# heathsc/bs_call

Measured on AMD Instinct MI355X. Metric: genome positions called/sec, higher is better.
Workload: dtype f64

## Files before the change

bs_call_amd/csrc/accumulate.hip:

```cpp
#include <hip/hip_runtime.h>
#include <stdint.h>

#include "accdev.h"
#include "devtables.h"

#define IN_DW 26
#define SLOT_DW (64 * IN_DW)
#define ACC_WAVES 4
#define SUM_DW 12

struct bsc_template_dev {
  uint32_t pos[2];
  uint32_t len[2];
  uint64_t off[2];
  uint8_t mapq[2];
  uint8_t orientation;
  uint8_t bs_strand;
  uint32_t flags;
};
#define TPL_WALK_KNOWN 1u
#define TPL_WALKED0 2u

__device__ static __forceinline__ uint32_t leftmost(uint32_t p0, uint32_t p1) {
  return p0 == 0 ? p1 : (p1 > 0 && p1 < p0 ? p1 : p0);
}

__device__ static __forceinline__ uint32_t template_error(const bsc_template_dev &tp, uint32_t left, uint32_t x,
                                                          uint64_t seq_bytes) {
  if (left < x) return BSC_TERR_LEFT;
  if ((tp.len[0] && tp.pos[0] < x) || (tp.len[1] && tp.pos[1] < x)) return BSC_TERR_LEFT;
  if (tp.orientation > 1) return BSC_TERR_ORI;
  if (tp.bs_strand > 2) return BSC_TERR_STRAND;
  if (tp.len[0] && (tp.off[0] > seq_bytes || tp.len[0] > seq_bytes - tp.off[0])) return BSC_TERR_RANGE0;
  if (tp.len[1] && (tp.off[1] > seq_bytes || tp.len[1] > seq_bytes - tp.off[1])) return BSC_TERR_RANGE1;
  if (tp.flags & ~(TPL_WALK_KNOWN | TPL_WALKED0)) return BSC_TERR_FLAGS;
  return 0;
}

__device__ static __forceinline__ uint32_t template_reads(const bsc_template_dev &tp, uint32_t x, uint32_t y, uint64_t seq_bytes,
                                                          bool walked0, bsc_read_desc d[2]) {
  acc_dead(d[0]);
  acc_dead(d[1]);
  const uint32_t terr = template_error(tp, leftmost(tp.pos[0], tp.pos[1]), x, seq_bytes);
  if (terr) return terr;
  uint32_t ori = tp.orientation & 1u;
#pragma unroll
  for (int k = 0; k < 2; k++) {
    const uint32_t rl = tp.len[k];
    if (rl != 0 && (k == 1 || walked0)) {
      const uint64_t pa = (uint64_t)tp.pos[k], pb = (uint64_t)tp.pos[k] + rl - 1u;
      if (pa <= y) {
        d[k].a = (uint32_t)pa;
        d[k].b = pb > y ? y : (uint32_t)pb;
        d[k].base = (int64_t)tp.off[k] - (int64_t)tp.pos[k];
        d[k].meta = ACC_META(ori, tp.mapq[k]);
        d[k].lut = tp.bs_strand == 0 ? LUT4(0, 1, 2, 3) : (tp.bs_strand == 1 ? LUT4(0, 5, 2, 7) : LUT4(4, 1, 6, 3));
      }
    }
    if (k == 0 && walked0) ori ^= 1u;
  }
  return 0;
}

__device__ static __forceinline__ void template_block(const bsc_chain_mblock *__restrict__ blk, uint32_t n_blk, uint32_t t, uint32_t &x,
                                                      uint32_t &y, uint32_t &bin0) {
  bin0 = 0;
  if (!blk) return;
  uint32_t lo = 0, hi = n_blk - 1u;
  while (lo < hi) {
    const uint32_t mid = (lo + hi) >> 1;
    if (t < blk[mid].tpl_end) hi = mid;
    else lo = mid + 1u;
  }
  x = blk[lo].x;
  y = blk[lo].x + (blk[lo].n - 1u);
  bin0 = blk[lo].bin0;
}

#ifndef BIN_WG
#define BIN_WG 256
#endif
#ifndef BIN_TPT
#define BIN_TPT 4
#endif
#define BIN_TPW (BIN_WG * BIN_TPT)
#ifndef BIN_WIN
#define BIN_WIN 1024
#endif

__device__ static __forceinline__ uint32_t wg_min_bin(uint32_t m, uint32_t *s_min) {
  if (threadIdx.x == 0) *s_min = 0xffffffffu;
  __syncthreads();
  for (int o = 32; o > 0; o >>= 1) {
    const uint32_t v = __shfl_xor(m, o);
    m = v < m ? v : m;
  }
  if ((threadIdx.x & 63u) == 0 && m != 0xffffffffu) atomicMin(s_min, m);
  __syncthreads();
  return *s_min;
}

extern "C" __global__ __launch_bounds__(BIN_WG) void bsc_bin_count_kernel(const bsc_template_dev *__restrict__ tpl, uint32_t nr,
                                                                          const uint8_t *__restrict__ seq, uint64_t seq_bytes,
                                                                          uint32_t x, uint32_t y, uint8_t *__restrict__ tflag,
                                                                          uint32_t *__restrict__ bin_cnt,
                                                                          unsigned long long *__restrict__ counters,
                                                                          const bsc_chain_mblock *__restrict__ blk, uint32_t n_blk) {
  __shared__ uint32_t s_cnt[BIN_WIN];
  __shared__ uint32_t s_min;
  for (unsigned i = threadIdx.x; i < BIN_WIN; i += BIN_WG) s_cnt[i] = 0;
  uint32_t bin[BIN_TPT][2], span_max = 0, bin_lo = 0xffffffffu;
  bsc_template_dev tps[BIN_TPT];
#pragma unroll
  for (int j = 0; j < BIN_TPT; j++) {
    const uint32_t t = blockIdx.x * BIN_TPW + (uint32_t)j * BIN_WG + threadIdx.x;
    if (t < nr) tps[j] = tpl[t];
  }
#pragma unroll
  for (int j = 0; j < BIN_TPT; j++) {
    const uint32_t t = blockIdx.x * BIN_TPW + (uint32_t)j * BIN_WG + threadIdx.x;
    bin[j][0] = bin[j][1] = 0xffffffffu;
    if (t < nr) {
      const bsc_template_dev tp = tps[j];
      uint32_t bin0;
      template_block(blk, n_blk, t, x, y, bin0);
      bool walked0 = false;
      if (tp.flags & TPL_WALK_KNOWN) walked0 = (tp.flags & TPL_WALKED0) != 0;
      else if (template_error(tp, leftmost(tp.pos[0], tp.pos[1]), x, seq_bytes) == 0) {
        const uint32_t rl = tp.len[0];
        const uint8_t *sp = seq + tp.off[0];
        for (uint32_t q_ = 0; q_ < rl; q_++) {
          const uint32_t q = (uint32_t)sp[q_] >> 2;
          if (q > 0 && q != 63u) {
            walked0 = true;
            break;
          }
        }
      }
      tflag[t] = walked0 ? 1 : 0;
      bsc_read_desc d[2];
      const uint32_t terr = template_reads(tp, x, y, seq_bytes, walked0, d);
      if (terr) atomicMin(&counters[BSC_CNT_ERR], ((unsigned long long)t << 8) | terr);
#pragma unroll
      for (int k = 0; k < 2; k++)
        if (d[k].b >= d[k].a) {
          bin[j][k] = bin0 + ((d[k].a - x) >> ACC_BIN_SHIFT);
          if (bin[j][k] < bin_lo) bin_lo = bin[j][k];
          if (d[k].b - d[k].a > span_max) span_max = d[k].b - d[k].a;
        }
    }
  }
  const uint32_t base = wg_min_bin(bin_lo, &s_min);
#pragma unroll
  for (int j = 0; j < BIN_TPT; j++)
#pragma unroll
    for (int k = 0; k < 2; k++)
      if (bin[j][k] != 0xffffffffu) {
        if (bin[j][k] - base < BIN_WIN) atomicAdd(&s_cnt[bin[j][k] - base], 1u);
        else atomicAdd(&bin_cnt[bin[j][k]], 1u);
      }
  __syncthreads();
  for (unsigned i = threadIdx.x; i < BIN_WIN; i += BIN_WG)
    if (s_cnt[i]) atomicAdd(&bin_cnt[base + i], s_cnt[i]);
  for (int o = 32; o > 0; o >>= 1) {
    const uint32_t v = __shfl_xor(span_max, o);
    span_max = v > span_max ? v : span_max;
  }
  if ((threadIdx.x & 63u) == 0 && span_max &&
      __hip_atomic_load(&counters[BSC_CNT_SPAN], __ATOMIC_RELAXED, __HIP_MEMORY_SCOPE_AGENT) < span_max)
    atomicMax(&counters[BSC_CNT_SPAN], (unsigned long long)span_max);
}

extern "C" __global__ __launch_bounds__(BIN_WG) void bsc_bin_scatter_kernel(const bsc_template_dev *__restrict__ tpl, uint32_t nr,
                                                                            uint64_t seq_bytes, uint32_t x, uint32_t y,
                                                                            const uint8_t *__restrict__ tflag,
                                                                            uint32_t *__restrict__ bin_cur,
                                                                            bsc_read_desc *__restrict__ rd,
                                                                            const bsc_chain_mblock *__restrict__ blk, uint32_t n_blk) {
  __shared__ uint32_t s_cnt[BIN_WIN];
  __shared__ uint32_t s_min;
  for (unsigned i = threadIdx.x; i < BIN_WIN; i += BIN_WG) s_cnt[i] = 0;
  uint32_t bin[BIN_TPT][2], rank[BIN_TPT][2], bin_lo = 0xffffffffu;
  bsc_read_desc d[BIN_TPT][2];
  bsc_template_dev tps[BIN_TPT];
  uint8_t tf[BIN_TPT];
#pragma unroll
  for (int j = 0; j < BIN_TPT; j++) {
    const uint32_t t = blockIdx.x * BIN_TPW + (uint32_t)j * BIN_WG + threadIdx.x;
    tf[j] = 0;
    if (t < nr) {
      tps[j] = tpl[t];
      tf[j] = tflag[t];
    }
  }
#pragma unroll
  for (int j = 0; j < BIN_TPT; j++) {
    const uint32_t t = blockIdx.x * BIN_TPW + (uint32_t)j * BIN_WG + threadIdx.x;
    bin[j][0] = bin[j][1] = 0xffffffffu;
    rank[j][0] = rank[j][1] = 0;
    acc_dead(d[j][0]);
    acc_dead(d[j][1]);
    if (t < nr) {
      uint32_t bin0;
      template_block(blk, n_blk, t, x, y, bin0);
      (void)template_reads(tps[j], x, y, seq_bytes, tf[j] != 0, d[j]);
#pragma unroll
      for (int k = 0; k < 2; k++)
        if (d[j][k].b >= d[j][k].a) {
          bin[j][k] = bin0 + ((d[j][k].a - x) >> ACC_BIN_SHIFT);
          if (bin[j][k] < bin_lo) bin_lo = bin[j][k];
        }
    }
  }
  const uint32_t base = wg_min_bin(bin_lo, &s_min);
#pragma unroll
  for (int j = 0; j < BIN_TPT; j++)
#pragma unroll
    for (int k = 0; k < 2; k++)
      if (bin[j][k] != 0xffffffffu && bin[j][k] - base < BIN_WIN) rank[j][k] = atomicAdd(&s_cnt[bin[j][k] - base], 1u);
  __syncthreads();
  for (unsigned i = threadIdx.x; i < BIN_WIN; i += BIN_WG)
    if (s_cnt[i]) s_cnt[i] = atomicAdd(&bin_cur[base + i], s_cnt[i]);
  __syncthreads();
#pragma unroll
  for (int j = 0; j < BIN_TPT; j++)
#pragma unroll
    for (int k = 0; k < 2; k++)
      if (bin[j][k] != 0xffffffffu) {
        const uint32_t slot = bin[j][k] - base < BIN_WIN ? s_cnt[bin[j][k] - base] + rank[j][k] : atomicAdd(&bin_cur[bin[j][k]], 1u);
        rd[slot] = d[j][k];
      }
}

template <bool SUMM>
__global__ __launch_bounds__(64 * ACC_WAVES) void bsc_accumulate_kernel_t(
    const bsc_read_desc *__restrict__ rd, const uint32_t *__restrict__ bin_off, uint32_t n_bins, const uint8_t *__restrict__ seq,
    uint32_t x, uint32_t y, uint32_t min_qual, uint32_t *__restrict__ cts, unsigned long long *__restrict__ counters,
    const bsc_chain_mblock *__restrict__ blk, uint32_t n_blk) {
  __shared__ __attribute__((aligned(16))) uint32_t lds_slot[ACC_WAVES][SLOT_DW];
  const unsigned lane = threadIdx.x & 63u;
  const unsigned wid = __builtin_amdgcn_readfirstlane(threadIdx.x >> 6);
  uint32_t *slot = lds_slot[wid];
  uint32_t *row = slot + lane * IN_DW;
  const uint32_t n_sites = y - x + 1;
  const uint32_t n_wt = blk ? n_bins : (n_sites + 63u) / 64u;
  const uint32_t q_span = min_qual < 63u ? 63u - min_qual : 0u;
  unsigned inexact = 0;
  acc_reads R;
  R.rd = rd;
  R.bin_off = bin_off;
  R.seq = seq;
  R.n_bins = n_bins;
  R.x = x;
  uint32_t n_live = bin_off[n_bins];
  const uint32_t span = (uint32_t)counters[BSC_CNT_SPAN];
  const uint32_t wt_step = gridDim.x * ACC_WAVES;
#ifndef ACC_XCD_CHUNK
#define ACC_XCD_CHUNK 16
#endif
#ifndef ACC_NO_XCD_SWIZZLE
  const uint32_t per8 = 8u * ACC_XCD_CHUNK, full8 = gridDim.x / per8 * per8;
  const uint32_t lb = blockIdx.x >> 3;
  const uint32_t vb = blockIdx.x < full8 ? (lb / ACC_XCD_CHUNK) * per8 + (blockIdx.x & 7u) * ACC_XCD_CHUNK + lb % ACC_XCD_CHUNK : blockIdx.x;
#else
  const uint32_t vb = blockIdx.x;
#endif
  uint32_t wt = vb * ACC_WAVES + wid;
  uint32_t t0 = 0, kv = 0xffffffffu;
  bsc_read_desc d;
  acc_dead(d);
  uint32_t wl = wt, wl_n = 0;
#define ACC_BLOCK_OF(w, wlocal)                                    \
  do {                                                             \
    uint32_t lo_ = 0, hi_ = n_blk - 1u;                            \
    while (lo_ < hi_) {                                            \
      const uint32_t mid_ = (lo_ + hi_) >> 1;                      \
      if ((w) < blk[mid_].bin_end) hi_ = mid_;                     \
      else lo_ = mid_ + 1u;                                        \
    }                                                              \
    x = blk[lo_].x;                                                \
    y = blk[lo_].x + (blk[lo_].n - 1u);                            \
    R.x = x;                                                       \
    R.bin_off = bin_off + blk[lo_].bin0;                           \
    n_live = bin_off[blk[lo_].bin_end];                            \
    (wlocal) = (w)-blk[lo_].bin0;                                  \
  } while (0)
  if (wt < n_wt) {
    if (blk) ACC_BLOCK_OF(wt, wl);
    t0 = acc_tile_start(R, (int64_t)wl * 64, span);
    acc_fetch(R, n_live, t0, lane, kv, d);
  }
  for (; wt < n_wt; wt += wt_step) {
    const uint32_t p0 = x + wl * 64u;
    const uint32_t p_last = y - p0 < 63u ? y : p0 + 63u;
    const uint32_t r_last = p_last - x;
    const bool valid = lane <= p_last - p0;
    const acc_reads Rc = R;
    const uint32_t n_live_c = n_live;
    const uint32_t wt1 = wt + wt_step;
    const bool have1 = wt1 < n_wt && wt1 > wt;
    uint32_t kv_n = 0xffffffffu, t0_n = 0;
    bsc_read_desc dn;
    acc_dead(dn);
    wl_n = wt1;
    if (have1) {
      if (blk) ACC_BLOCK_OF(wt1, wl_n);
      t0_n = acc_tile_start(R, (int64_t)wl_n * 64, span);
      acc_fetch(R, n_live, t0_n, lane, kv_n, dn);
    }
    {
      uint32_t w[IN_DW];
      bool packed;
      inexact |= acc_tile(Rc, n_live_c, lane, lane, row, p0, p_last, r_last, min_qual, q_span, t0, kv, d, w, &packed) ? 1u : 0u;
      if (SUMM) {
        if (__builtin_expect(!packed, 0)) {
          uint32_t cmax = 0;
#pragma unroll
          for (int j = 0; j < 8; j++) cmax = max(cmax, w[j] + w[8 + j]);
          if (__any(cmax > 0xffffu) && lane == 0) atomicMax(&counters[BSC_CNT_DEEP], 1ull);
        }
        uint32_t o[SUM_DW];
        {
#include "call_summary.inc"
#pragma unroll
          for (int j = 0; j < 8; j++) o[j] = ((w[j] + w[8 + j]) & 0xffffu) | (w[j] << 16);
          o[8] = qpack0;
          o[9] = qpack1;
          o[10] = ((uint32_t)aq & 0xffffu) | ((uint32_t)mq << 16);
          o[11] = covered ? n_reads : 0u;
        }
        uint32_t *srow = slot + lane * SUM_DW;
#pragma unroll
        for (int i = 0; i < SUM_DW / 2; i++) reinterpret_cast<uint2 *>(srow)[i] = make_uint2(o[2 * i], o[2 * i + 1]);
      } else {
#pragma unroll
        for (int i = 0; i < IN_DW / 2; i++) reinterpret_cast<uint2 *>(row)[i] = make_uint2(w[2 * i], w[2 * i + 1]);
      }
    }
    const uint32_t nvalid = p_last - p0 + 1u;
    constexpr unsigned ROW = SUMM ? SUM_DW : IN_DW;
    uint32_t *dst = cts + (uint64_t)wt * (64u * ROW);
#ifdef ACC_EXPERIMENT_NOSTORE
    if (wt == 0xffffffffu)
#endif
    if (nvalid == 64u) {
      typedef unsigned int u32x4 __attribute__((ext_vector_type(4)));
      const u32x4 *s4 = reinterpret_cast<const u32x4 *>(slot);
      u32x4 *d4 = reinterpret_cast<u32x4 *>(dst);
#ifdef ACC_PLAIN_STORES
#define ACC_ST(p, v) *(p) = (v)
#else
#define ACC_ST(p, v) __builtin_nontemporal_store((v), (p))
#endif
      constexpr int full = (int)(64u * ROW * 4u / 1024u);
#pragma unroll
      for (int v = 0; v < full; v++) ACC_ST(d4 + v * 64 + lane, s4[v * 64 + lane]);
      constexpr unsigned rem = (64u * ROW * 4u % 1024u) / 16u;
      if (rem && lane < rem) ACC_ST(d4 + full * 64 + lane, s4[full * 64 + lane]);
#undef ACC_ST
    } else if (valid || blk) {
      const uint32_t *orow = slot + lane * ROW;
#pragma unroll
      for (int i = 0; i < (int)ROW; i++) dst[lane * ROW + i] = valid ? orow[i] : 0u;
    }
    t0 = t0_n;
    kv = kv_n;
    d = dn;
    wl = wl_n;
  }
  if (__any(inexact)) {
    const unsigned long long m = __ballot(inexact);
    if (lane == 0) atomicAdd(&counters[BSC_CNT_INEXACT], (unsigned long long)__popcll(m));
  }
}

extern "C" __global__ __launch_bounds__(256) void bsc_ref_pad_kernel(const uint8_t *__restrict__ packed, const bsc_chain_mblock *__restrict__ blk,
                                                                     uint32_t n_blk, uint8_t *__restrict__ padded, uint32_t n_pos) {
  for (uint32_t p = blockIdx.x * 256u + threadIdx.x; p < n_pos; p += gridDim.x * 256u) {
    uint32_t lo = 0, hi = n_blk;
    while (hi - lo > 1u) {
      const uint32_t mid = (lo + hi) >> 1;
      if (blk[mid].pos_off <= p) lo = mid;
      else hi = mid;
    }
    const uint32_t i = p - blk[lo].pos_off;
    padded[p] = i < blk[lo].n ? packed[(uint64_t)blk[lo].ref_in + i] : (uint8_t)0;
  }
}

extern "C" int bsc_dev_launch_ref_pad(const void *packed, const void *d_blk, uint32_t n_blk, void *padded, uint32_t n_pos, int num_cus,
                                      void *stream) {
  if (!n_pos) return 0;
  unsigned g = (n_pos + 255u) / 256u;
  if (g > (unsigned)num_cus * 8u) g = (unsigned)num_cus * 8u;
  hipLaunchKernelGGL(bsc_ref_pad_kernel, dim3(g), dim3(256), 0, (hipStream_t)stream, (const uint8_t *)packed, (const bsc_chain_mblock *)d_blk,
                     n_blk, (uint8_t *)padded, n_pos);
  return (int)hipGetLastError();
}

extern "C" int bsc_dev_scan_u32(const void *in, void *out, uint32_t n, void *tmp, size_t tmp_bytes, void *stream);

extern "C" uint32_t bsc_dev_n_bins(uint32_t n_sites) { return ((n_sites - 1u) >> ACC_BIN_SHIFT) + 1u; }

static int launch_bin_reads(const void *tpl, uint32_t nr, const void *seq, uint64_t seq_bytes, uint32_t x, uint32_t y, uint32_t nb,
                            const bsc_chain_mblock *blk, uint32_t n_blk, void *tflag, void *bin_cnt, void *bin_off, void *bin_cur,
                            void *scan_tmp, size_t scan_tmp_bytes, void *rd, void *counters, void *stream) {
  hipStream_t s = (hipStream_t)stream;
  const size_t bytes = ((size_t)nb + 1u) * sizeof(uint32_t);
  if (!nr) return (int)hipMemsetAsync(bin_off, 0, bytes, s);
  hipError_t e = hipMemsetAsync(bin_cnt, 0, bytes, s);
  if (e != hipSuccess) return (int)e;
  const unsigned g = (nr + BIN_TPW - 1u) / BIN_TPW;
  hipLaunchKernelGGL(bsc_bin_count_kernel, dim3(g), dim3(BIN_WG), 0, s, (const bsc_template_dev *)tpl, nr, (const uint8_t *)seq,
                     seq_bytes, x, y, (uint8_t *)tflag, (uint32_t *)bin_cnt, (unsigned long long *)counters, blk, n_blk);
  if ((e = hipGetLastError()) != hipSuccess) return (int)e;
  int rc = bsc_dev_scan_u32(bin_cnt, bin_off, nb + 1u, scan_tmp, scan_tmp_bytes, stream);
  if (rc) return rc;
  if ((e = hipMemcpyAsync(bin_cur, bin_off, bytes, hipMemcpyDeviceToDevice, s)) != hipSuccess) return (int)e;
  hipLaunchKernelGGL(bsc_bin_scatter_kernel, dim3(g), dim3(BIN_WG), 0, s, (const bsc_template_dev *)tpl, nr, seq_bytes, x, y,
                     (const uint8_t *)tflag, (uint32_t *)bin_cur, (bsc_read_desc *)rd, blk, n_blk);
  return (int)hipGetLastError();
}

extern "C" int bsc_dev_launch_bin_reads(const void *tpl, uint32_t nr, const void *seq, uint64_t seq_bytes, uint32_t x, uint32_t y,
                                        void *tflag, void *bin_cnt, void *bin_off, void *bin_cur, void *scan_tmp,
                                        size_t scan_tmp_bytes, void *rd, void *counters, void *stream) {
  return launch_bin_reads(tpl, nr, seq, seq_bytes, x, y, bsc_dev_n_bins(y - x + 1), NULL, 0, tflag, bin_cnt, bin_off, bin_cur, scan_tmp,
                          scan_tmp_bytes, rd, counters, stream);
}

extern "C" int bsc_dev_launch_bin_reads_multi(const void *tpl, uint32_t nr, const void *seq, uint64_t seq_bytes, const void *d_blk,
                                              uint32_t n_blk, uint32_t n_bins, void *tflag, void *bin_cnt, void *bin_off, void *bin_cur,
                                              void *scan_tmp, size_t scan_tmp_bytes, void *rd, void *counters, void *stream) {
  return launch_bin_reads(tpl, nr, seq, seq_bytes, 0, 0, n_bins, (const bsc_chain_mblock *)d_blk, n_blk, tflag, bin_cnt, bin_off, bin_cur,
                          scan_tmp, scan_tmp_bytes, rd, counters, stream);
}

static int launch_accumulate(const void *rd, const void *bin_off, const void *seq, uint32_t x, uint32_t y, uint32_t n_wt, uint32_t min_qual,
                             void *cts, void *counters, const bsc_chain_mblock *blk, uint32_t n_blk, int num_cus, void *stream,
                             bool summary = false) {
  unsigned g = (n_wt + ACC_WAVES - 1) / ACC_WAVES;
  const unsigned cap = (unsigned)num_cus * 6u * 8u;
  if (g > cap) g = cap;
  if (summary)
    hipLaunchKernelGGL(bsc_accumulate_kernel_t<true>, dim3(g), dim3(64 * ACC_WAVES), 0, (hipStream_t)stream, (const bsc_read_desc *)rd,
                       (const uint32_t *)bin_off, n_wt, (const uint8_t *)seq, x, y, min_qual, (uint32_t *)cts,
                       (unsigned long long *)counters, blk, n_blk);
  else
    hipLaunchKernelGGL(bsc_accumulate_kernel_t<false>, dim3(g), dim3(64 * ACC_WAVES), 0, (hipStream_t)stream, (const bsc_read_desc *)rd,
                       (const uint32_t *)bin_off, n_wt, (const uint8_t *)seq, x, y, min_qual, (uint32_t *)cts,
                       (unsigned long long *)counters, blk, n_blk);
  return (int)hipGetLastError();
}

extern "C" int bsc_dev_launch_accumulate_summary(const void *rd, const void *bin_off, const void *seq, uint32_t x, uint32_t y,
                                                 uint32_t min_qual, void *cts, void *counters, int num_cus, void *stream) {
  return launch_accumulate(rd, bin_off, seq, x, y, bsc_dev_n_bins(y - x + 1), min_qual, cts, counters, NULL, 0, num_cus, stream, true);
}
extern "C" size_t bsc_dev_summary_bytes(void) { return SUM_DW * 4u; }

extern "C" int bsc_dev_launch_accumulate(const void *rd, const void *bin_off, const void *seq, uint32_t x, uint32_t y, uint32_t min_qual,
                                         void *cts, void *counters, int num_cus, void *stream) {
  return launch_accumulate(rd, bin_off, seq, x, y, bsc_dev_n_bins(y - x + 1), min_qual, cts, counters, NULL, 0, num_cus, stream);
}

extern "C" int bsc_dev_launch_accumulate_multi(const void *rd, const void *bin_off, const void *seq, const void *d_blk, uint32_t n_blk,
                                               uint32_t n_bins, uint32_t min_qual, void *cts, void *counters, int num_cus, void *stream) {
  return launch_accumulate(rd, bin_off, seq, 0, 0, n_bins, min_qual, cts, counters, (const bsc_chain_mblock *)d_blk, n_blk, num_cus, stream);
}
```

bs_call_amd/csrc/bscall_api.c:

```c
#ifndef __HIP_PLATFORM_AMD__
#define __HIP_PLATFORM_AMD__ 1
#endif
#include <hip/hip_runtime_api.h>
#include <math.h>
#include <pthread.h>
#include <stdarg.h>
#include <stdio.h>
#include <stdlib.h>
#include <string.h>

#include "../../include/bscall_amd.h"
#include "devtables.h"
#include "bsmath.h"
#include "bsmath_tables.h"
#include "synth.h"

int bsc_dev_launch_call(const void *cts, const void *ref, uint64_t n, void *out, uint32_t out_dw, void *skip,
                        const void *tb, void *het_list, void *counters, int num_cus, void *stream, void *ev_start,
                        void *ev_mid, void *ev_stop);
int bsc_dev_launch_accumulate(const void *rd, const void *bin_off, const void *seq, uint32_t x, uint32_t y, uint32_t min_qual, void *cts,
                              void *counters, int num_cus, void *stream);
int bsc_dev_launch_bin_reads(const void *tpl, uint32_t nr, const void *seq, uint64_t seq_bytes, uint32_t x, uint32_t y, void *tflag,
                             void *bin_cnt, void *bin_off, void *bin_cur, void *scan_tmp, size_t scan_tmp_bytes, void *rd,
                             void *counters, void *stream);
uint32_t bsc_dev_n_bins(uint32_t n_sites);
int bsc_dev_launch_site_stats(const void *core, const void *gtm, uint32_t gtm_stride, const void *dbsnp, uint32_t n,
                              const void *tb, const void *logp, const void *carry_in, void *carry_out, void *stats,
                              void *pairs, int num_cus, void *stream);
int bsc_dev_launch_gc_cov_gtm(const void *core, const void *gtm, uint32_t gtm_stride, uint32_t n, const void *gc_bins, uint32_t n_bins,
                              uint32_t start_pos, void *table, int num_cus, void *stream);
int bsc_dev_launch_meth_eval(void *pairs, const void *tb, const void *logp, void *stats, const void *ovf_list,
                             const void *counters, int num_cus, void *stream);
int bsc_dev_scan_tmp_bytes(uint32_t n, size_t *bytes);
int bsc_dev_launch_stream_probe(const void *cts, const void *ref, uint64_t n, void *out, void *skip, int num_cus,
                                void *stream);
int bsc_dev_launch_compact(const void *core, const void *gtm, uint32_t gtm_stride, const void *dbsnp, uint32_t n,
                           void *tile_cnt, void *tile_off, void *scan_tmp, size_t scan_tmp_bytes, void *out,
                           uint64_t out_cap, void *total, const void *emit, void *emit_ws, int num_cus, void *stream);
#define BSC_PAIR_BYTES (4ull * 512u * 512u * 8u)
#define BSC_OVF_CAP (1u << 20)
int bsc_dev_launch_vcf(const void *gtm, uint32_t stride, const void *skip, const void *ref, const void *dbsnp, uint32_t n,
                       uint32_t x, int all_positions, uint32_t reg_start, uint32_t reg_stop, const void *tb, void *g,
                       void *out, int num_cus, void *stream);
int bsc_dev_launch_chain(const bsc_chain_launch *L);
unsigned bsc_dev_chain_quantum(int num_cus);
unsigned bsc_dev_chain_window(int num_cus, unsigned limit);
int bsc_dev_launch_synth(uint64_t seed, uint64_t first_site, uint64_t n, uint32_t coverage, uint32_t flags, void *cts,
                         void *ref, int num_cus, void *stream);
size_t bsc_dev_chain_het_bytes(uint32_t n, int num_cus, int with_depth, int reads);
size_t bsc_dev_chain_scratch_bytes(int num_cus);
size_t bsc_dev_chain_multi_table_bytes(uint32_t n_blocks);
int bsc_dev_launch_chain_multi(const bsc_chain_launch *L, const bsc_chain_mblock *blk, uint32_t b_first, uint32_t b_last, void *tab_h,
                               void *tab_d, size_t *cursor);
int bsc_dev_launch_accumulate_summary(const void *rd, const void *bin_off, const void *seq, uint32_t x, uint32_t y, uint32_t min_qual, void *cts,
                                      void *counters, int num_cus, void *stream);
size_t bsc_dev_summary_bytes(void);
int bsc_dev_launch_accumulate_multi(const void *rd, const void *bin_off, const void *seq, const void *d_blk, uint32_t n_blk, uint32_t n_bins,
                                    uint32_t min_qual, void *cts, void *counters, int num_cus, void *stream);
int bsc_dev_scan_tmp_bytes_u64(uint32_t n, size_t *bytes);
size_t bsc_dev_prep_plan_bytes(void);
int bsc_dev_launch_prep(const void *raw, uint32_t nr, const void *seq, uint64_t seq_bytes, const void *misms, uint64_t n_misms,
                        const bsc_prep_params *par, void *ms_work, void *plan, void *out_len, void *out_off, void *scan_tmp,
                        size_t scan_tmp_bytes, void *tpl_out, void *seq_out, uint64_t seq_out_cap, void *cnt, int num_cus, void *stream,
                        const void *prof_ref, uint32_t prof_x, uint32_t prof_n_ref, uint32_t prof_cap, uint32_t prof_used0, void *prof_table,
                        void *max_pos1, void *used_scan, void *prof_mask);
int bsc_dev_launch_bcf(const void *recs, const void *core, const void *aux, const void *n_recs, uint64_t max_recs, int32_t rid,
                       const bsc_bcf_ids *ids, const void *name_pos, const void *name_off, const void *name_bytes, uint32_t n_names,
                       void *tile_bytes, void *tile_off, void *scan_tmp, size_t scan_tmp_bytes, void *out, uint64_t out_cap, void *totals,
                       int num_cus, void *stream, const void *emit_len);
int bsc_dev_launch_vcf_text(const void *recs, const void *core, const void *aux, const void *n_recs, uint64_t max_recs, const char *contig,
                            uint32_t contig_len, const void *name_pos, const void *name_off, const void *name_bytes, uint32_t n_names,
                            void *tile_bytes, void *tile_off, void *line_len, void *scan_tmp, size_t scan_tmp_bytes, void *out, uint64_t out_cap,
                            void *totals, int num_cus, void *stream);
int bsc_dev_launch_fmt_g(const void *v, uint64_t n, void *out16, int num_cus, void *stream);
int bsc_dev_launch_ref_pad(const void *packed, const void *d_blk, uint32_t n_blk, void *padded, uint32_t n_pos, int num_cus, void *stream);
int bsc_dev_launch_bin_reads_multi(const void *tpl, uint32_t nr, const void *seq, uint64_t seq_bytes, const void *d_blk, uint32_t n_blk,
                                   uint32_t n_bins, void *tflag, void *bin_cnt, void *bin_off, void *bin_cur, void *scan_tmp,
                                   size_t scan_tmp_bytes, void *rd, void *counters, void *stream);
int bsc_dev_launch_bgzf(const void *src, uint64_t n, uint32_t n_members, void *slots, void *sizes, void *offs, void *scratch, uint32_t grid,
                        void *stream);
int bsc_dev_launch_bgzf_gather(const void *slots, const void *offs, const void *sizes, uint32_t n_members, void *out, void *stream);
#define BSC_PREP_CNT_SLOTS 64u
#define BSC_PREP_CNT_ALL (8u + 8u * BSC_PREP_CNT_SLOTS)
#define BSC_LN10 (2.30258509299404568402)
#define BSC_HOST_CHUNK (4u << 20)
#define BSC_MAX_LAUNCH (1ull << 31)

struct bsc_context {
  bsc_params params;
  int device;
  int num_cus;
  hipStream_t stream;
  double q_prob[44][5];
  bsc_dev_tables host_tables;
  void *d_tables;
  unsigned long long *d_counters;
  uint64_t sites;
  void *d_cts, *d_ref, *d_out, *d_skip;
  size_t cap_cts, cap_ref, cap_out, cap_skip;
  void *d_het;
  size_t cap_het;
  uint64_t max_launch;
  void *d_ovf;
  void *d_gc_table;
  void *d_gc_own;
  size_t cap_gc_own;
  const void *d_gc_bins;
  uint32_t gc_n_bins, gc_start_pos;
  hipEvent_t ev_chain[2];
  int ev_chain_valid;
  void *d_tpl, *d_seq, *d_rd;
  size_t cap_tpl, cap_seq, cap_rd;
  void *d_tflag, *d_bcnt, *d_boff, *d_bcur, *d_bscan;
  size_t cap_tflag, cap_bcnt, cap_boff, cap_bcur, cap_bscan;
  void *d_vg, *d_vout, *d_vdb;
  size_t cap_vg, cap_vout, cap_vdb;
  void *d_tcnt, *d_toff, *d_scantmp, *d_recs;
  size_t cap_tcnt, cap_toff, cap_scantmp, cap_recs;
  void *d_sstats, *d_pairs;
  uint32_t *d_carry;
  double *d_logp;
  unsigned carry_slot;
  void *h_stage;
  size_t cap_stage;
  uint64_t pending_sz;
  uint32_t pending_stride;
  int pending_copied;
  const bsc_template *blk_tpl;
  const void *blk_d_tpl;
  uint32_t blk_x;
  unsigned long long *h_cnt;
  bsc_vcf_rec *rec_out;
  uint64_t rec_cap, rec_copied;
  uint32_t rec_sz;
  int rec_pending;
  double rec_share;
  void *d_btb, *d_bto, *d_bscn, *d_bnm, *d_bcf, *d_btot;
  size_t cap_btb, cap_bto, cap_bscn, cap_bnm, cap_bcf, cap_btot;
  void *d_vtl;
  size_t cap_vtl;
  struct {
    void *p[4];
    size_t cap[4];
  } bcf_pool;
  pthread_mutex_t pool_mu;
  int pool_mu_made;
  void *det_ptr[4];
  hipStream_t s_det;
  void *h_names;
  size_t cap_hnm;
  const bsc_bcf_names *names_up;
  uint32_t names_up_n;
  uint64_t names_up_bytes;
  struct {
    int valid, have_names, inexact;
    uint32_t sz, n_names;
    uint64_t name_bytes;
    int32_t rid;
    bsc_bcf_ids ids;
    const void *emit;
    bsc_bcf_names names;
    int text;
    char contig[256];
  } again;
  int no_h2d_turns;
  void *d_emit;
  size_t cap_emit;
  hipEvent_t ev_h2d;
  const void *emit_hint;
  uint8_t *bcf_out;
  int stage_timing;
  int no_emit_bytes;
  int bcf_blk, bcf_keep;
  uint64_t bcf_cap, bcf_copied, bcf_bytes;
  double bcf_share;
  const bsc_chain_mblock *mb_tab;
  uint32_t mb_n;
  void *d_mblk, *d_mtab;
  size_t cap_mblk, cap_mtab;
  void *d_pplan, *d_plen, *d_poff, *d_pms, *d_pscan, *d_pcnt, *d_raw, *d_rseq, *d_rms;
  size_t cap_pplan, cap_plen, cap_poff, cap_pms, cap_pscan, cap_pcnt, cap_raw, cap_rseq, cap_rms;
  unsigned long long *h_prep;
  size_t cap_hprep;
  void *d_pmask;
  size_t cap_pmask;
  void *d_pprof, *d_pmax, *d_pused;
  size_t cap_pprof, cap_pmax, cap_pused;
  void *d_refp;
  size_t cap_refp;
  const uint32_t *mb_toff;
  int dbg_fail_summary;
  int reads_fused;
  void *d_fscr;
  size_t cap_fscr;
  hipEvent_t ev_rchain[2];
  int ev_rchain_valid;
  hipEvent_t ev_raw[2];
  int ev_raw_valid;
  int ref_resident;
  hipEvent_t ev_acc[2];
  int ev_acc_valid;
  hipStream_t s_in, s_out;
  hipEvent_t ev_in[2], ev_k[2], ev_out[2];
  void *p_cts[2], *p_ref[2], *p_out[2], *p_skip[2];
  size_t p_cap_cts[2], p_cap_ref[2], p_cap_out[2], p_cap_skip[2];
  int pipe_ready;
  int profiling;
#define BSC_EV_RING 32
  hipEvent_t ev[BSC_EV_RING][3];
  uint64_t ev_count;
};

static __thread char bsc_errbuf[512];

static int bsc_fail(int code, const char *fmt, ...) {
  va_list ap;
  va_start(ap, fmt);
  vsnprintf(bsc_errbuf, sizeof bsc_errbuf, fmt, ap);
  va_end(ap);
  return code;
}

typedef struct {
  int prev;
} bsc_devguard;
static void bsc_devguard_exit(bsc_devguard *g) {
  if (g->prev >= 0) (void)hipSetDevice(g->prev);
}
#define BSC_GUARD(g) bsc_devguard g __attribute__((cleanup(bsc_devguard_exit), unused)) = {-1}
#define BSC_ENTER_GUARD(ctx, g)  \
  do {                                                                               \
    int cur_ = -1;                                                                   \
    if (hipGetDevice(&cur_) != hipSuccess || cur_ != (ctx)->device) {                \
      HIP_TRY(hipSetDevice((ctx)->device));                                          \
      (g).prev = cur_;                                                               \
    }                                                                                \
  } while (0)
#define BSC_ENTER(ctx) \
  BSC_GUARD(guard_);   \
  BSC_ENTER_GUARD(ctx, guard_)

int bsc_set_error(int code, const char *fmt, ...) {
  va_list ap;
  va_start(ap, fmt);
  vsnprintf(bsc_errbuf, sizeof bsc_errbuf, fmt, ap);
  va_end(ap);
  return code;
}

#define HIP_TRY(call)                                                                                        \
  do {                                                                                                       \
    hipError_t e_ = (call);                                                                                  \
    if (e_ != hipSuccess) return bsc_fail(BSC_ERR_HIP, "%s failed: %s (%s:%d)", #call, hipGetErrorString(e_), \
                                          __FILE__, __LINE__);                                               \
  } while (0)

int bsc_ctx_device(const bsc_context *ctx) { return ctx->device; }
void *bsc_ctx_stream(const bsc_context *ctx) { return (void *)ctx->stream; }

int bsc_abi_version(void) { return BSC_ABI_VERSION; }
const char *bsc_last_error(void) { return bsc_errbuf; }

void bsc_params_default(bsc_params *p) {
  p->under_conv = 0.01;
  p->over_conv = 0.05;
  p->ref_bias = 2.0;
  p->min_qual = 20;
  p->device = -1;
}

static int bsc_phred_of_om(double om) {
  const double lg = bsm_log_t(om, bsm_log_tab);
  const double v = (-10.0 * lg) / BSC_LN10;
  const int p = (int)v;
  return p > 255 ? 255 : p;
}
static int bsc_build_phred_table(bsc_dev_tables *t) {
  double T[260];
  for (int k = 1; k <= 255; k++) {
    uint64_t lo = bsm_bits(0x1p-1000), hi = bsm_bits(1.0);
    if (bsc_phred_of_om(bsm_from_bits(lo)) < k || bsc_phred_of_om(bsm_from_bits(hi)) >= k) return -1;
    while (hi - lo > 1) {
      const uint64_t mid = lo + (hi - lo) / 2;
      if (bsc_phred_of_om(bsm_from_bits(mid)) >= k) lo = mid;
      else hi = mid;
    }
    T[k] = bsm_from_bits(lo);
    if (k > 1 && !(T[k] < T[k - 1])) return -1;
  }
  for (int k = 256; k < 260; k++) T[k] = -1.0;
  for (int e = 0; e < 64; e++) {
    const double top = e == 0 ? 1.0 : bsm_from_bits(bsm_bits(ldexp(1.0, 1 - e)) - 1);
    const int b = bsc_phred_of_om(top);
    if (bsc_phred_of_om(ldexp(1.0, -e)) - b > 4) return -1;
    t->phred_base[e] = (unsigned char)b;
    for (int j = 0; j < 4; j++) t->phred_thr[e][j] = T[b + 1 + j];
  }
  return 0;
}

int bsc_phred_table(double *thr_64x4, unsigned char *base_64) {
  if (!thr_64x4 || !base_64) return bsc_fail(BSC_ERR_ARG, "bsc_phred_table: NULL argument");
  bsc_dev_tables *t = malloc(sizeof *t);
  if (!t) return bsc_fail(BSC_ERR_NOMEM, "bsc_phred_table: out of memory");
  const int rc = bsc_build_phred_table(t);
  if (!rc) {
    memcpy(thr_64x4, t->phred_thr, sizeof t->phred_thr);
    memcpy(base_64, t->phred_base, sizeof t->phred_base);
  }
  free(t);
  return rc ? bsc_fail(BSC_ERR_ARG, "bsc_phred_table: the QUAL staircase of this build's log is not monotone") : BSC_OK;
}

static void bsc_build_tables(bsc_context *ctx) {
  bsc_dev_tables *t = &ctx->host_tables;
  for (int q = 0; q <= 43; q++) {
    double e = exp(-.1 * (double)q * BSC_LN10);
    if (e > .5) e = .5;
    double k = e / (3.0 - 4.0 * e);
    ctx->q_prob[q][0] = e;
    ctx->q_prob[q][1] = t->k[q] = k;
    ctx->q_prob[q][2] = t->ln_k[q] = log(k);
    ctx->q_prob[q][3] = t->ln_k_half[q] = log(0.5 + k);
    ctx->q_prob[q][4] = t->ln_k_one[q] = log(1.0 + k);
  }
  t->lfact[0] = t->lfact[1] = 0.0;
  double l = 0.0;
  for (int i = 2; i < 256; i++) {
    l += log((double)i);
    t->lfact[i] = l;
  }
  memcpy(t->log_tab, bsm_log_tab, sizeof t->log_tab);
  memcpy(t->exp_tab, bsm_exp_tab, sizeof t->exp_tab);
  t->under_conv = ctx->params.under_conv;
  t->over_conv = ctx->params.over_conv;
  t->lrb = log(ctx->params.ref_bias);
  t->lrb1 = log(0.5 * (1.0 + ctx->params.ref_bias));
}

int bsc_create(const bsc_params *params, bsc_context **out) {
  if (!out) return bsc_fail(BSC_ERR_ARG, "bsc_create: out is NULL");
  *out = NULL;
  bsc_params p;
  if (params) p = *params;
  else bsc_params_default(&p);
  if (!(p.under_conv >= 0.0 && p.under_conv < 1.0) || !(p.over_conv >= 0.0 && p.over_conv < 1.0) || !(p.ref_bias > 0.0))
    return bsc_fail(BSC_ERR_ARG, "bsc_create: conversion rates must be in [0,1) and ref_bias > 0");
  if (!((1.0 - p.under_conv) - p.over_conv >= 0x1p-20))
    return bsc_fail(BSC_ERR_ARG, "bsc_create: under_conv + over_conv must be < 1 (by at least 2^-20)");
  if (p.min_qual < 1) p.min_qual = 1;
  if (p.min_qual > 43) p.min_qual = 43;
// ... 209 lines not shown
    return bsc_fail(BSC_ERR_ARG, "out_stride must be 200 (gt_meth[]) or 208 (gt_vcf[]), got %u", out_stride);
  return BSC_OK;
}

int bsc_call_sites_device(bsc_context *ctx, const void *d_cts, const void *d_ref, uint64_t n, void *d_out,
                          uint32_t out_stride, void *d_skip, void *stream) {
  if (!ctx) return bsc_fail(BSC_ERR_ARG, "bsc_call_sites_device: ctx is NULL");
  int rc = bsc_check_stride(out_stride);
  if (rc) return rc;
  if (n == 0) return BSC_OK;
  if (!d_cts || !d_ref || !d_out || !d_skip) return bsc_fail(BSC_ERR_ARG, "bsc_call_sites_device: NULL buffer");
  if (((uintptr_t)d_cts & 15u) || ((uintptr_t)d_out & 15u))
    return bsc_fail(BSC_ERR_ARG, "bsc_call_sites_device: d_cts and d_out must be 16-byte aligned");
  BSC_ENTER(ctx);
  hipStream_t s = (hipStream_t)stream;
  uint64_t done = 0;
  while (done < n) {
    uint64_t m = n - done;
    if (m > ctx->max_launch) m = ctx->max_launch;
    rc = bsc_reserve(&ctx->d_het, &ctx->cap_het, (size_t)((m + 63u) / 64u) * 8u);
    if (rc) return rc;
    int e = bsc_dev_launch_call((const char *)d_cts + done * 104u, (const char *)d_ref + done, m,
                                (char *)d_out + done * out_stride, out_stride / 4u, (char *)d_skip + done,
                                ctx->d_tables, ctx->d_het, ctx->d_counters, ctx->num_cus, s,
                                ctx->profiling ? ctx->ev[ctx->ev_count % BSC_EV_RING][0] : NULL,
                                ctx->profiling ? ctx->ev[ctx->ev_count % BSC_EV_RING][1] : NULL,
                                ctx->profiling ? ctx->ev[ctx->ev_count % BSC_EV_RING][2] : NULL);
    if (ctx->profiling) ctx->ev_count++;
    if (e) return bsc_fail(BSC_ERR_HIP, "kernel launch failed: %s", hipGetErrorString((hipError_t)e));
    done += m;
  }
  ctx->sites += n;
  return BSC_OK;
}

#define BSC_PIPE_CHUNK (1u << 20)

static int bsc_pipe_init(bsc_context *ctx) {
  if (ctx->pipe_ready) return BSC_OK;
  HIP_TRY(hipStreamCreateWithFlags(&ctx->s_in, hipStreamNonBlocking));
  HIP_TRY(hipStreamCreateWithFlags(&ctx->s_out, hipStreamNonBlocking));
  for (int b = 0; b < 2; b++) {
    HIP_TRY(hipEventCreateWithFlags(&ctx->ev_in[b], hipEventDisableTiming));
    HIP_TRY(hipEventCreateWithFlags(&ctx->ev_k[b], hipEventDisableTiming));
    HIP_TRY(hipEventCreateWithFlags(&ctx->ev_out[b], hipEventDisableTiming));
  }
  ctx->pipe_ready = 1;
  return BSC_OK;
}

int bsc_call_sites(bsc_context *ctx, const bsc_pileup *cts, const uint8_t *ref, uint64_t n, void *out,
                   uint32_t out_stride, uint8_t *skip) {
  if (!ctx) return bsc_fail(BSC_ERR_ARG, "bsc_call_sites: ctx is NULL");
  int rc = bsc_check_stride(out_stride);
  if (rc) return rc;
  if (n == 0) return BSC_OK;
  if (!cts || !ref || !out || !skip) return bsc_fail(BSC_ERR_ARG, "bsc_call_sites: NULL buffer");
  BSC_ENTER(ctx);
  if ((rc = bsc_pipe_init(ctx))) return rc;
  const uint64_t chunk = n < BSC_PIPE_CHUNK ? n : BSC_PIPE_CHUNK;
  const int nbuf = n > chunk ? 2 : 1;
  for (int b = 0; b < nbuf; b++) {
    if ((rc = bsc_reserve(&ctx->p_cts[b], &ctx->p_cap_cts[b], (size_t)chunk * 104u))) return rc;
    if ((rc = bsc_reserve(&ctx->p_ref[b], &ctx->p_cap_ref[b], (size_t)chunk))) return rc;
    if ((rc = bsc_reserve(&ctx->p_out[b], &ctx->p_cap_out[b], (size_t)chunk * out_stride))) return rc;
    if ((rc = bsc_reserve(&ctx->p_skip[b], &ctx->p_cap_skip[b], (size_t)chunk))) return rc;
  }
  uint64_t k = 0;
  for (uint64_t done = 0; done < n; done += chunk, k++) {
    const int b = (int)(k & 1);
    const uint64_t m = (n - done) < chunk ? (n - done) : chunk;
    if (k >= 2) HIP_TRY(hipStreamWaitEvent(ctx->s_in, ctx->ev_k[b], 0));
    HIP_TRY(hipMemcpyAsync(ctx->p_cts[b], cts + done, (size_t)m * 104u, hipMemcpyHostToDevice, ctx->s_in));
    HIP_TRY(hipMemcpyAsync(ctx->p_ref[b], ref + done, (size_t)m, hipMemcpyHostToDevice, ctx->s_in));
    HIP_TRY(hipEventRecord(ctx->ev_in[b], ctx->s_in));
    HIP_TRY(hipStreamWaitEvent(ctx->stream, ctx->ev_in[b], 0));
    if (k >= 2) HIP_TRY(hipStreamWaitEvent(ctx->stream, ctx->ev_out[b], 0));
    rc = bsc_call_sites_device(ctx, ctx->p_cts[b], ctx->p_ref[b], m, ctx->p_out[b], out_stride, ctx->p_skip[b], ctx->stream);
    if (rc) return rc;
    HIP_TRY(hipEventRecord(ctx->ev_k[b], ctx->stream));
    HIP_TRY(hipStreamWaitEvent(ctx->s_out, ctx->ev_k[b], 0));
    HIP_TRY(hipMemcpyAsync((char *)out + done * out_stride, ctx->p_out[b], (size_t)m * out_stride, hipMemcpyDeviceToHost,
                           ctx->s_out));
    HIP_TRY(hipMemcpyAsync(skip + done, ctx->p_skip[b], (size_t)m, hipMemcpyDeviceToHost, ctx->s_out));
    HIP_TRY(hipEventRecord(ctx->ev_out[b], ctx->s_out));
  }
  HIP_TRY(hipStreamSynchronize(ctx->s_out));
  HIP_TRY(hipStreamSynchronize(ctx->stream));
  return BSC_OK;
}

void *bsc_alloc_host(uint64_t bytes) {
  void *p = NULL;
  if (hipHostMalloc(&p, (size_t)bytes, hipHostMallocDefault) != hipSuccess) {
    bsc_fail(BSC_ERR_NOMEM, "bsc_alloc_host(%llu) failed", (unsigned long long)bytes);
    return NULL;
  }
  return p;
}

void bsc_free_host(void *p) {
  if (p) hipHostFree(p);
}

static uint32_t bsc_leftmost(const bsc_template *t) {
  uint32_t x1 = t->pos[0];
  if (x1 == 0) x1 = t->pos[1];
  else if (t->pos[1] > 0 && t->pos[1] < x1) x1 = t->pos[1];
  return x1;
}

static int bsc_stage_reserve(bsc_context *ctx, size_t need) {
  if (need <= ctx->cap_stage) return BSC_OK;
  if (ctx->h_stage) hipHostFree(ctx->h_stage);
  ctx->h_stage = NULL;
  ctx->cap_stage = 0;
  size_t sz = need + need / 4;
  if (hipHostMalloc(&ctx->h_stage, sz, hipHostMallocDefault) != hipSuccess)
    return bsc_fail(BSC_ERR_NOMEM, "hipHostMalloc(%zu) failed", sz);
  ctx->cap_stage = sz;
  return BSC_OK;
}

static int bsc_accumulate_queue2(bsc_context *ctx, const bsc_template *tpl, uint32_t nr, const uint8_t *seq,
                                 uint64_t seq_bytes, uint32_t x, uint32_t y, const uint8_t *ref, int stage);

static int bsc_accumulate_queue(bsc_context *ctx, const bsc_template *tpl, uint32_t nr, const uint8_t *seq,
                                uint64_t seq_bytes, uint32_t x, uint32_t y) {
  return bsc_accumulate_queue2(ctx, tpl, nr, seq, seq_bytes, x, y, NULL, 0);
}

static int bsc_accumulate_reserve(bsc_context *ctx, uint32_t nr, uint32_t x, uint32_t y, size_t *scan_bytes) {
  const uint64_t sz = (uint64_t)y - x + 1;
  if (sz > 0xffffffffull) return bsc_fail(BSC_ERR_ARG, "accumulate: block longer than 2^32 - 1 positions");
  const size_t nb1 = (size_t)bsc_dev_n_bins((uint32_t)sz) + 1u;
  int rc;
  *scan_bytes = 0;
  if (nr > 0x7fffffffu) return bsc_fail(BSC_ERR_ARG, "accumulate: more than 2^31 - 1 templates in one block");
  if (bsc_dev_scan_tmp_bytes((uint32_t)nb1, scan_bytes)) return bsc_fail(BSC_ERR_HIP, "accumulate: scan size query failed");
  if ((rc = bsc_reserve(&ctx->d_rd, &ctx->cap_rd, (size_t)(nr ? nr : 1) * 48u))) return rc;
  if ((rc = bsc_reserve(&ctx->d_tflag, &ctx->cap_tflag, (size_t)(nr ? nr : 1)))) return rc;
  if ((rc = bsc_reserve(&ctx->d_bcnt, &ctx->cap_bcnt, nb1 * 4u))) return rc;
  if ((rc = bsc_reserve(&ctx->d_boff, &ctx->cap_boff, nb1 * 4u))) return rc;
  if ((rc = bsc_reserve(&ctx->d_bcur, &ctx->cap_bcur, nb1 * 4u))) return rc;
  if ((rc = bsc_reserve(&ctx->d_bscan, &ctx->cap_bscan, *scan_bytes ? *scan_bytes : 1))) return rc;
  return BSC_OK;
}

static int bsc_reads_prepare(bsc_context *ctx, const void *d_tpl, uint32_t nr, const void *d_seq, uint64_t seq_bytes, uint32_t x,
                             uint32_t y, size_t scan_bytes, hipStream_t s) {
  HIP_TRY(hipMemsetAsync(ctx->d_counters + BSC_CNT_SPAN, 0, 2 * sizeof(unsigned long long), s));
  HIP_TRY(hipMemsetAsync(ctx->d_counters + BSC_CNT_ERR, 0xff, sizeof(unsigned long long), s));
  HIP_TRY(hipMemsetAsync(ctx->d_counters + BSC_CNT_DEEP, 0, sizeof(unsigned long long), s));
  int e = bsc_dev_launch_bin_reads(d_tpl, nr, d_seq, seq_bytes, x, y, ctx->d_tflag, ctx->d_bcnt, ctx->d_boff, ctx->d_bcur,
                                   ctx->d_bscan, scan_bytes, ctx->d_rd, ctx->d_counters, s);
  if (e) return bsc_fail(BSC_ERR_HIP, "read grouping launch failed: %s", hipGetErrorString((hipError_t)e));
  return BSC_OK;
}

static int bsc_accumulate_launch(bsc_context *ctx, const void *d_tpl, uint32_t nr, const void *d_seq, uint64_t seq_bytes,
                                 uint32_t x, uint32_t y, void *d_cts, size_t scan_bytes, hipStream_t s) {
  if (ctx->profiling) {
    if (!ctx->ev_acc[0])
      for (int i = 0; i < 2; i++) HIP_TRY(hipEventCreate(&ctx->ev_acc[i]));
    HIP_TRY(hipEventRecord(ctx->ev_acc[0], s));
  }
  int rc = bsc_reads_prepare(ctx, d_tpl, nr, d_seq, seq_bytes, x, y, scan_bytes, s);
  if (rc) return rc;
  int e = bsc_dev_launch_accumulate(ctx->d_rd, ctx->d_boff, d_seq, x, y, (uint32_t)ctx->params.min_qual, d_cts, ctx->d_counters,
                                    ctx->num_cus, s);
  if (e) return bsc_fail(BSC_ERR_HIP, "accumulate launch failed: %s", hipGetErrorString((hipError_t)e));
  if (ctx->profiling) {
    HIP_TRY(hipEventRecord(ctx->ev_acc[1], s));
    ctx->ev_acc_valid = 1;
  }
  return BSC_OK;
}

static int bsc_accumulate_queue2(bsc_context *ctx, const bsc_template *tpl, uint32_t nr, const uint8_t *seq,
                                 uint64_t seq_bytes, uint32_t x, uint32_t y, const uint8_t *ref, int stage) {
  if (y < x) return bsc_fail(BSC_ERR_ARG, "accumulate: y (%u) < x (%u) (reference asserts y >= x)", y, x);
  if (nr && (!tpl || !seq)) return bsc_fail(BSC_ERR_ARG, "accumulate: NULL template or read buffer");
  if (ctx->pending_sz || ctx->rec_pending)
    return bsc_fail(BSC_ERR_ARG, "a submitted block has not been fetched (bsc_block_fetch / bsc_block_records_fetch first)");
  BSC_ENTER(ctx);
  const uint64_t sz = (uint64_t)y - x + 1;
  const uint64_t n_wt = (sz + 63) / 64;
  int rc;
  size_t scan_bytes = 0;
  if ((rc = bsc_reserve(&ctx->d_cts, &ctx->cap_cts, (size_t)n_wt * 64u * 104u))) return rc;
  if ((rc = bsc_reserve(&ctx->d_tpl, &ctx->cap_tpl, (size_t)(nr ? nr : 1) * sizeof(bsc_template)))) return rc;
  if ((rc = bsc_reserve(&ctx->d_seq, &ctx->cap_seq, (size_t)(seq_bytes ? seq_bytes : 1)))) return rc;
  if ((rc = bsc_accumulate_reserve(ctx, nr, x, y, &scan_bytes))) return rc;
  if (stage) {
    const size_t b_tpl = (size_t)nr * sizeof(bsc_template), b_seq = (size_t)seq_bytes, b_ref = ref ? (size_t)sz : 0;
    const size_t o_seq = (b_tpl + 63u) & ~(size_t)63u, o_ref = (o_seq + b_seq + 63u) & ~(size_t)63u;
    if ((rc = bsc_stage_reserve(ctx, o_ref + b_ref + 64u))) return rc;
    char *st = ctx->h_stage;
    if (nr) {
      memcpy(st, tpl, b_tpl);
      memcpy(st + o_seq, seq, b_seq);
      tpl = (const bsc_template *)st;
      seq = (const uint8_t *)(st + o_seq);
    }
    if (ref) {
      memcpy(st + o_ref, ref, b_ref);
      if ((rc = bsc_reserve(&ctx->d_ref, &ctx->cap_ref, (size_t)sz))) return rc;
      HIP_TRY(hipMemcpyAsync(ctx->d_ref, st + o_ref, b_ref, hipMemcpyHostToDevice, ctx->stream));
    }
  }
  ctx->blk_tpl = tpl;
  ctx->blk_d_tpl = ctx->d_tpl;
  ctx->blk_x = x;
  ctx->mb_n = 0;
  if (nr) {
    HIP_TRY(hipMemcpyAsync(ctx->d_tpl, tpl, (size_t)nr * sizeof(bsc_template), hipMemcpyHostToDevice, ctx->stream));
    HIP_TRY(hipMemcpyAsync(ctx->d_seq, seq, (size_t)seq_bytes, hipMemcpyHostToDevice, ctx->stream));
  }
  return bsc_accumulate_launch(ctx, ctx->d_tpl, nr, ctx->d_seq, seq_bytes, x, y, ctx->d_cts, scan_bytes, ctx->stream);
}

static int bsc_verdict(bsc_context *ctx, const unsigned long long f[2], int *inexact);

static int bsc_block_check_on(bsc_context *ctx, hipStream_t s, int *inexact) {
  unsigned long long f[2];
  HIP_TRY(hipMemcpyAsync(f, ctx->d_counters + BSC_CNT_INEXACT, sizeof f, hipMemcpyDeviceToHost, s));
  HIP_TRY(hipStreamSynchronize(s));
  return bsc_verdict(ctx, f, inexact);
}

static int bsc_block_check(bsc_context *ctx, int *inexact) { return bsc_block_check_on(ctx, ctx->stream, inexact); }

static int bsc_verdict(bsc_context *ctx, const unsigned long long f[2], int *inexact) {
  if (f[1] != ~0ull) {
    const uint32_t i = (uint32_t)(f[1] >> 8);
    bsc_template dt;
    const bsc_template *t = &dt;
    if (ctx->blk_tpl) t = ctx->blk_tpl + i;
    else HIP_TRY(hipMemcpy(&dt, (const char *)ctx->blk_d_tpl + (size_t)i * sizeof(bsc_template), sizeof dt, hipMemcpyDeviceToHost));
    uint32_t blk_x = ctx->blk_x;
    for (uint32_t b = 0; b < ctx->mb_n; b++)
      if (i < ctx->mb_tab[b].tpl_end) {
        blk_x = ctx->mb_tab[b].x;
        break;
      }
    switch ((int)(f[1] & 0xffu)) {
      case BSC_TERR_LEFT:
        return bsc_fail(BSC_ERR_ARG, "accumulate: template %u starts at %u, left of the block start %u", i,
                        bsc_leftmost(t), blk_x);
      case BSC_TERR_ORI:
        return bsc_fail(BSC_ERR_ARG, "accumulate: template %u has orientation %u (reference asserts ori < 2)", i,
                        t->orientation);
      case BSC_TERR_STRAND: return bsc_fail(BSC_ERR_ARG, "accumulate: template %u has bs_strand %u", i, t->bs_strand);
      case BSC_TERR_FLAGS:
        return bsc_fail(BSC_ERR_ARG, "accumulate: template %u has flags 0x%x (only BSC_TPL_WALK_KNOWN | BSC_TPL_WALKED0 are defined: ABI %d)", i, t->flags,
                        BSC_ABI_VERSION);
      default:
        return bsc_fail(BSC_ERR_ARG, "accumulate: read %d of template %u lies outside the read buffer",
                        (int)(f[1] & 0xffu) - BSC_TERR_RANGE0, i);
    }
  }
  if (inexact) *inexact = f[0] != 0;
  return BSC_OK;
}

static int bsc_inexact_status(int inexact) {
  if (inexact) {
    bsc_fail(BSC_WARN_INEXACT, "accumulate: position(s) with a quality or MAPQ^2 sum >= 2^24: the reference's float "
             "sums depend on read order there");
    return BSC_WARN_INEXACT;
  }
  return BSC_OK;
}

int bsc_accumulate(bsc_context *ctx, const bsc_template *tpl, uint32_t nr, const uint8_t *seq, uint64_t seq_bytes,
                   uint32_t x, uint32_t y, bsc_pileup *out) {
  if (!ctx || !out) return bsc_fail(BSC_ERR_ARG, "bsc_accumulate: NULL argument");
  int rc = bsc_accumulate_queue(ctx, tpl, nr, seq, seq_bytes, x, y), inexact = 0;
  if (rc) return rc;
  if ((rc = bsc_block_check(ctx, &inexact))) return rc;
  const uint64_t sz = (uint64_t)y - x + 1;
  HIP_TRY(hipMemcpyAsync(out, ctx->d_cts, (size_t)sz * 104u, hipMemcpyDeviceToHost, ctx->stream));
  HIP_TRY(hipStreamSynchronize(ctx->stream));
  return bsc_inexact_status(inexact);
}

int bsc_accumulate_device(bsc_context *ctx, const void *d_tpl, uint32_t nr, const void *d_seq, uint64_t seq_bytes, uint32_t x,
                          uint32_t y, void *d_cts, void *stream) {
  if (!ctx || !d_cts) return bsc_fail(BSC_ERR_ARG, "bsc_accumulate_device: NULL argument");
  if (y < x) return bsc_fail(BSC_ERR_ARG, "accumulate: y (%u) < x (%u) (reference asserts y >= x)", y, x);
  if (nr && (!d_tpl || !d_seq)) return bsc_fail(BSC_ERR_ARG, "accumulate: NULL template or read buffer");
  if (((uintptr_t)d_cts & 15u) || ((uintptr_t)d_tpl & 7u))
    return bsc_fail(BSC_ERR_ARG, "bsc_accumulate_device: d_cts must be 16-byte and d_tpl 8-byte aligned");
  BSC_ENTER(ctx);
  size_t scan_bytes = 0;
  int rc = bsc_accumulate_reserve(ctx, nr, x, y, &scan_bytes);
  if (rc) return rc;
  ctx->blk_tpl = NULL;
  ctx->blk_d_tpl = d_tpl;
  ctx->blk_x = x;
  ctx->mb_n = 0;
  return bsc_accumulate_launch(ctx, d_tpl, nr, d_seq, seq_bytes, x, y, d_cts, scan_bytes, (hipStream_t)stream);
}

int bsc_block_status(bsc_context *ctx, void *stream) {
  if (!ctx) return bsc_fail(BSC_ERR_ARG, "bsc_block_status: ctx is NULL");
  BSC_ENTER(ctx);
  int inexact = 0;
// ... 489 lines not shown
    L.run_if = 2;
    e = bsc_dev_launch_chain(&L);
    if (e) return bsc_fail(BSC_ERR_HIP, "reads chain launch failed: %s", hipGetErrorString((hipError_t)e));
    L = L2;
    L.run_if = 1;
    L.ev_start = NULL;
  }
  if (!two_kernels || L.run_if) {
    L.rd = ctx->d_rd;
    L.bin_off = ctx->d_boff;
    L.seq = d_seq;
    L.f_scratch = ctx->d_fscr;
    L.n_bins = bsc_dev_n_bins(w.n);
    L.min_qual = (uint32_t)ctx->params.min_qual;
  }
  e = bsc_dev_launch_chain(&L);
  if (e) return bsc_fail(BSC_ERR_HIP, "reads chain launch failed: %s", hipGetErrorString((hipError_t)e));
  if (ctx->profiling) {
    HIP_TRY(hipEventRecord(ctx->ev_rchain[1], s));
    ctx->ev_rchain_valid = 1;
  }
  if (with_stats) ctx->carry_slot ^= 1u;
  ctx->sites += w.n;
  return BSC_OK;
}

int bsc_reads_chain_device(bsc_context *ctx, const void *d_tpl, uint32_t nr, const void *d_seq, uint64_t seq_bytes, uint32_t x,
                           uint32_t y, const void *d_ref, const void *d_dbsnp, const bsc_vcf_params *params, int with_stats,
                           void *d_core, void *d_aux, void *stream) {
  if (!ctx || !params || !d_ref || !d_core) return bsc_fail(BSC_ERR_ARG, "bsc_reads_chain_device: NULL argument");
  if (y < x) return bsc_fail(BSC_ERR_ARG, "bsc_reads_chain_device: y (%u) < x (%u) (reference asserts y >= x)", y, x);
  if (nr && (!d_tpl || !d_seq)) return bsc_fail(BSC_ERR_ARG, "bsc_reads_chain_device: NULL template or read buffer");
  if (((uintptr_t)d_core & 15u) || ((uintptr_t)d_aux & 15u) || ((uintptr_t)d_tpl & 7u))
    return bsc_fail(BSC_ERR_ARG, "bsc_reads_chain_device: d_core / d_aux must be 16-byte and d_tpl 8-byte aligned");
  BSC_ENTER(ctx);
  ctx->blk_tpl = NULL;
  ctx->blk_d_tpl = d_tpl;
  ctx->blk_x = x;
  ctx->mb_n = 0;
  return bsc_reads_chain_queue(ctx, d_tpl, nr, d_seq, seq_bytes, x, y, d_ref, d_dbsnp, params, with_stats, d_core, d_aux, NULL,
                               (hipStream_t)stream);
}

int bsc_reads_chain_len_device(bsc_context *ctx, const void *d_tpl, uint32_t nr, const void *d_seq, uint64_t seq_bytes, uint32_t x, uint32_t y,
                               const void *d_ref, const void *d_dbsnp, const bsc_vcf_params *params, int with_stats, void *d_core, void *d_aux,
                               void *d_len, void *stream) {
  if (!ctx || !params || !d_ref || !d_core || !d_len) return bsc_fail(BSC_ERR_ARG, "bsc_reads_chain_len_device: NULL argument");
  if (y < x) return bsc_fail(BSC_ERR_ARG, "bsc_reads_chain_len_device: y (%u) < x (%u)", y, x);
  if (nr && (!d_tpl || !d_seq)) return bsc_fail(BSC_ERR_ARG, "bsc_reads_chain_len_device: NULL template or read buffer");
  if (((uintptr_t)d_core & 15u) || ((uintptr_t)d_aux & 15u) || ((uintptr_t)d_tpl & 7u))
    return bsc_fail(BSC_ERR_ARG, "bsc_reads_chain_len_device: d_core / d_aux must be 16-byte and d_tpl 8-byte aligned");
  BSC_ENTER(ctx);
  ctx->blk_tpl = NULL;
  ctx->blk_d_tpl = d_tpl;
  ctx->blk_x = x;
  ctx->mb_n = 0;
  HIP_TRY(hipMemsetAsync(d_len, 0, (size_t)y - x + 1u, (hipStream_t)stream));
  return bsc_reads_chain_queue(ctx, d_tpl, nr, d_seq, seq_bytes, x, y, d_ref, d_dbsnp, params, with_stats, d_core, d_aux, d_len, (hipStream_t)stream);
}

int bsc_last_reads_chain_ms(bsc_context *ctx, float *ms) {
  if (!ctx || !ms) return bsc_fail(BSC_ERR_ARG, "bsc_last_reads_chain_ms: NULL argument");
  if (!ctx->profiling || !ctx->ev_rchain_valid) return bsc_fail(BSC_ERR_ARG, "bsc_last_reads_chain_ms: no profiled launch yet");
  BSC_ENTER(ctx);
  HIP_TRY(hipEventSynchronize(ctx->ev_rchain[1]));
  HIP_TRY(hipEventElapsedTime(ms, ctx->ev_rchain[0], ctx->ev_rchain[1]));
  return BSC_OK;
}

int bsc_last_raw_block_ms(bsc_context *ctx, float *ms) {
  if (!ctx || !ms) return bsc_fail(BSC_ERR_ARG, "bsc_last_raw_block_ms: NULL argument");
  if (!ctx->profiling || !ctx->ev_raw_valid) return bsc_fail(BSC_ERR_ARG, "bsc_last_raw_block_ms: no profiled raw block yet");
  BSC_ENTER(ctx);
  HIP_TRY(hipEventSynchronize(ctx->ev_raw[1]));
  HIP_TRY(hipEventElapsedTime(ms, ctx->ev_raw[0], ctx->ev_raw[1]));
  return BSC_OK;
}

uint32_t bsc_chain_window_quantum(const bsc_context *ctx) { return ctx ? bsc_dev_chain_quantum(ctx->num_cus) : 0u; }
uint32_t bsc_chain_window_size(const bsc_context *ctx, uint32_t limit) { return ctx ? bsc_dev_chain_window(ctx->num_cus, limit) : 0u; }

int bsc_last_chain_ms(bsc_context *ctx, float *ms) {
  if (!ctx || !ms) return bsc_fail(BSC_ERR_ARG, "bsc_last_chain_ms: NULL argument");
  if (!ctx->profiling || !ctx->ev_chain_valid) return bsc_fail(BSC_ERR_ARG, "bsc_last_chain_ms: no profiled launch yet");
  BSC_ENTER(ctx);
  HIP_TRY(hipEventSynchronize(ctx->ev_chain[1]));
  HIP_TRY(hipEventElapsedTime(ms, ctx->ev_chain[0], ctx->ev_chain[1]));
  return BSC_OK;
}

static int bsc_prep_device_error(bsc_context *ctx, unsigned long long word, const void *d_raw, const void *d_seq, const void *d_misms,
                                 const bsc_prep_params *par) {
  (void)ctx;
  const uint32_t ti = (uint32_t)(word >> 8), code = (uint32_t)(word & 0xffu);
  if (code == 9u) return bsc_fail(BSC_ERR_ARG, "bsc_prepare_templates: seq_out too small (template %u)", ti);
  if (code == 10u) return bsc_fail(BSC_ERR_ARG, "bsc_prepare_templates: template %u: read position beyond the profile", ti);
  if (code == 11u) return bsc_fail(BSC_ERR_ARG, "bsc_prepare_templates: template %u lies outside the profile's reference", ti);
  bsc_raw_template t;
  HIP_TRY(hipMemcpy(&t, (const char *)d_raw + (size_t)ti * sizeof t, sizeof t, hipMemcpyDeviceToHost));
  if (code == 1u) return bsc_fail(BSC_ERR_ARG, "bsc_prepare_templates: template %u has orientation %u", ti, t.orientation);
  if (code == 2u || code == 3u) return bsc_fail(BSC_ERR_ARG, "bsc_prepare_templates: read %d of template %u lies outside the read buffer", (int)code - 2, ti);
  if (code == 4u || code == 5u)
    return bsc_fail(BSC_ERR_ARG, "bsc_prepare_templates: mismatch list %d of template %u lies outside the list buffer", (int)code - 4, ti);
  const size_t nb = (size_t)t.len[0] + t.len[1], nmm = (size_t)t.n_misms[0] + t.n_misms[1];
  uint8_t *rb = malloc(nb + 1);
  bsc_misms *mb = malloc((nmm + 1) * sizeof *mb);
  uint8_t *so = NULL;
  size_t so_cap = nb + 16;
  if (!rb || !mb) {
    free(rb);
    free(mb);
    return bsc_fail(BSC_ERR_NOMEM, "bsc_prepare_templates_device: out of memory");
  }
  bsc_raw_template l = t;
  size_t ob = 0, om = 0;
  for (int k = 0; k < 2; k++) {
    if (t.len[k]) (void)hipMemcpy(rb + ob, (const char *)d_seq + t.off[k], t.len[k], hipMemcpyDeviceToHost);
    if (t.n_misms[k])
      (void)hipMemcpy(mb + om, (const char *)d_misms + (size_t)t.misms_off[k] * sizeof *mb, (size_t)t.n_misms[k] * sizeof *mb, hipMemcpyDeviceToHost);
    l.off[k] = ob;
    l.misms_off[k] = om;
    ob += t.len[k];
    om += t.n_misms[k];
  }
  for (size_t z = 0; z < nmm; z++)
    if (mb[z].type == BSC_MISMS_INS && mb[z].size <= nb) so_cap += mb[z].size;
  so = malloc(so_cap);
  if (!so) {
    free(rb);
    free(mb);
    return bsc_fail(BSC_ERR_NOMEM, "bsc_prepare_templates_device: out of memory");
  }
  bsc_template o;
  uint64_t used = 0;
  const int rc = bsc_prepare_templates(&l, 1, rb, nb, mb, nmm, par, &o, so, so_cap, &used, NULL);
  free(rb);
  free(mb);
  free(so);
  if (rc >= 0 || strstr(bsc_errbuf, "seq_out too small"))
    return bsc_fail(BSC_ERR_ARG, "bsc_prepare_templates_device: template %u fails check %u on the device, none on the host", ti, code);
  char msg[sizeof bsc_errbuf];
  snprintf(msg, sizeof msg, "%s", bsc_errbuf);
  char *at = strstr(msg, "template 0 ");
  if (at) {
    char tail[sizeof bsc_errbuf];
    snprintf(tail, sizeof tail, "%s", at + 11);
    *at = 0;
    return bsc_fail(rc, "%stemplate %u %s", msg, ti, tail);
  }
  return bsc_fail(rc, "%s (template %u)", msg, ti);
}

static int bsc_prep_queue(bsc_context *ctx, const void *d_raw, uint32_t nr, const void *d_seq, uint64_t seq_bytes, const void *d_misms, uint64_t n_misms,
                          const bsc_prep_params *par, void *d_tpl_out, void *d_seq_out, uint64_t seq_out_cap, const bsc_read_profile *pf, hipStream_t s) {
  int rc;
  size_t scan_bytes = 0;
  const uint32_t n2 = 2u * nr + 1u;
  if (bsc_dev_scan_tmp_bytes_u64(n2, &scan_bytes)) return bsc_fail(BSC_ERR_HIP, "bsc_prepare_templates_device: scan size query failed");
  if ((rc = bsc_reserve(&ctx->d_pplan, &ctx->cap_pplan, (size_t)(nr ? nr : 1) * 2u * bsc_dev_prep_plan_bytes()))) return rc;
  if ((rc = bsc_reserve(&ctx->d_plen, &ctx->cap_plen, (size_t)n2 * 8u))) return rc;
  if ((rc = bsc_reserve(&ctx->d_poff, &ctx->cap_poff, (size_t)n2 * 8u))) return rc;
  if ((rc = bsc_reserve(&ctx->d_pms, &ctx->cap_pms, (size_t)(n_misms ? n_misms : 1) * sizeof(bsc_misms)))) return rc;
  if ((rc = bsc_reserve(&ctx->d_pscan, &ctx->cap_pscan, scan_bytes ? scan_bytes : 1))) return rc;
  if ((rc = bsc_reserve(&ctx->d_pcnt, &ctx->cap_pcnt, BSC_PREP_CNT_ALL * sizeof(unsigned long long)))) return rc;
  const size_t prof_bytes = pf && nr ? (size_t)pf->cap * 4u * sizeof(unsigned long long) : 0;
  const size_t h_need = (BSC_PREP_CNT_ALL + 2u) * sizeof(unsigned long long) + prof_bytes;
  if (h_need > ctx->cap_hprep) {
    if (ctx->h_prep) hipHostFree(ctx->h_prep);
    ctx->h_prep = NULL;
    ctx->cap_hprep = 0;
    if (hipHostMalloc((void **)&ctx->h_prep, h_need, hipHostMallocDefault) != hipSuccess)
      return bsc_fail(BSC_ERR_NOMEM, "bsc_prepare_templates_device: hipHostMalloc(%zu) failed", h_need);
    ctx->cap_hprep = h_need;
  }
  if (prof_bytes) {
    if ((rc = bsc_reserve(&ctx->d_pprof, &ctx->cap_pprof, prof_bytes))) return rc;
    if ((rc = bsc_reserve(&ctx->d_pmax, &ctx->cap_pmax, (size_t)nr * 4u))) return rc;
    if ((rc = bsc_reserve(&ctx->d_pused, &ctx->cap_pused, (size_t)nr * 4u))) return rc;
    if ((rc = bsc_reserve(&ctx->d_pmask, &ctx->cap_pmask, (size_t)pf->n_ref + 28u))) return rc;
    HIP_TRY(hipMemsetAsync(ctx->d_pprof, 0, prof_bytes, s));
  }
  HIP_TRY(hipMemsetAsync(ctx->d_pcnt, 0, BSC_PREP_CNT_ALL * sizeof(unsigned long long), s));
  HIP_TRY(hipMemsetAsync(ctx->d_pcnt, 0xff, sizeof(unsigned long long), s));
  int e = bsc_dev_launch_prep(d_raw, nr, d_seq, seq_bytes, d_misms, n_misms, par, ctx->d_pms, ctx->d_pplan, ctx->d_plen, ctx->d_poff,
                              ctx->d_pscan, scan_bytes, d_tpl_out, d_seq_out, seq_out_cap, ctx->d_pcnt, ctx->num_cus, s,
                              prof_bytes ? pf->ref : NULL, pf ? pf->x : 0u, pf ? pf->n_ref : 0u, pf ? pf->cap : 0u, pf ? pf->used : 0u,
                              ctx->d_pprof, ctx->d_pmax, ctx->d_pused, ctx->d_pmask);
  if (e) {
    (void)hipStreamSynchronize(s);
    return bsc_fail(BSC_ERR_HIP, "read pre-processing launch failed: %s", hipGetErrorString((hipError_t)e));
  }
  unsigned long long *h = ctx->h_prep;
  h[BSC_PREP_CNT_ALL + 1u] = 0;
  HIP_TRY(hipMemcpyAsync(h, ctx->d_pcnt, BSC_PREP_CNT_ALL * sizeof(unsigned long long), hipMemcpyDeviceToHost, s));
  HIP_TRY(hipMemcpyAsync(h + BSC_PREP_CNT_ALL, (const char *)ctx->d_poff + (size_t)(nr ? 2u * nr : 0u) * 8u, sizeof(unsigned long long), hipMemcpyDeviceToHost, s));
  if (prof_bytes) {
    HIP_TRY(hipMemcpyAsync(h + BSC_PREP_CNT_ALL + 2u, ctx->d_pprof, prof_bytes, hipMemcpyDeviceToHost, s));
    HIP_TRY(hipMemcpyAsync(h + BSC_PREP_CNT_ALL + 1u, (const char *)ctx->d_pused + (size_t)(nr - 1u) * 4u, 4, hipMemcpyDeviceToHost, s));
  }
  return BSC_OK;
}

static int bsc_prep_finish(bsc_context *ctx, const void *d_raw, uint32_t nr, const void *d_seq, const void *d_misms, const bsc_prep_params *par,
                           uint64_t *seq_out_used, bsc_prep_stats *stats, bsc_read_profile *pf) {
  const unsigned long long *hs = ctx->h_prep;
  unsigned long long h[8];
  memcpy(h, hs, sizeof h);
  for (unsigned k = 0; k < BSC_PREP_CNT_SLOTS; k++) {
    h[1] += hs[8u + 8u * k];
    h[2] += hs[8u + 8u * k + 1u];
  }
  if (h[0] != ~0ull) return bsc_prep_device_error(ctx, h[0], d_raw, d_seq, d_misms, par);
  if (pf && nr) {
    const uint32_t used_last = (uint32_t)hs[BSC_PREP_CNT_ALL + 1u];
    const unsigned long long *delta = hs + BSC_PREP_CNT_ALL + 2u;
    if (used_last > pf->used) {
      memset(pf->counts + (size_t)pf->used * 4u, 0, (size_t)(pf->cap - pf->used) * 4u * sizeof(uint64_t));
      pf->used = used_last;
    }
    for (size_t i = 0; i < (size_t)pf->cap * 4u; i++) pf->counts[i] += delta[i];
  }
  if (seq_out_used) *seq_out_used = hs[BSC_PREP_CNT_ALL];
  if (stats) {
    stats->base_clip = h[1];
    stats->base_overlap = h[2];
    stats->base_none = h[3];
    stats->base_trim = h[4];
    stats->base_lowqual = h[5];
    stats->reads = h[6];
    stats->read_bases = h[7];
  }
  return BSC_OK;
}

static int bsc_prep_args_check(bsc_context *ctx, const void *d_raw, uint32_t nr, const void *d_seq, uint64_t seq_bytes, const void *d_misms, uint64_t n_misms,
                               const bsc_prep_params *par, void *d_tpl_out, void *d_seq_out, uint64_t seq_out_cap, const bsc_read_profile *pf) {
  if (pf && (!pf->ref || !pf->counts || pf->used > pf->cap || !pf->cap)) return bsc_fail(BSC_ERR_ARG, "bsc_prepare_templates_device: bad read profile");
  if (!ctx || !par || (nr && (!d_raw || !d_tpl_out))) return bsc_fail(BSC_ERR_ARG, "bsc_prepare_templates_device: NULL argument");
  if ((seq_bytes && !d_seq) || (n_misms && !d_misms) || (seq_out_cap && !d_seq_out))
    return bsc_fail(BSC_ERR_ARG, "bsc_prepare_templates_device: NULL buffer");
  if (nr > 0x7fffffffu) return bsc_fail(BSC_ERR_ARG, "bsc_prepare_templates_device: more than 2^31 - 1 templates in one call");
  if (((uintptr_t)d_raw & 7u) || ((uintptr_t)d_tpl_out & 7u) || ((uintptr_t)d_misms & 3u))
    return bsc_fail(BSC_ERR_ARG, "bsc_prepare_templates_device: d_raw / d_tpl_out must be 8-byte, d_misms 4-byte aligned");
  return BSC_OK;
}

int bsc_prepare_templates_device(bsc_context *ctx, const void *d_raw, uint32_t nr, const void *d_seq, uint64_t seq_bytes, const void *d_misms,
                                 uint64_t n_misms, const bsc_prep_params *par, void *d_tpl_out, void *d_seq_out, uint64_t seq_out_cap,
                                 uint64_t *seq_out_used, bsc_prep_stats *stats, bsc_read_profile *pf, void *stream) {
  if (!seq_out_used) return bsc_fail(BSC_ERR_ARG, "bsc_prepare_templates_device: NULL argument");
  int rc = bsc_prep_args_check(ctx, d_raw, nr, d_seq, seq_bytes, d_misms, n_misms, par, d_tpl_out, d_seq_out, seq_out_cap, pf);
  if (rc) return rc;
  *seq_out_used = 0;
  if (stats) memset(stats, 0, sizeof *stats);
  BSC_ENTER(ctx);
  hipStream_t s = (hipStream_t)stream;
  if ((rc = bsc_prep_queue(ctx, d_raw, nr, d_seq, seq_bytes, d_misms, n_misms, par, d_tpl_out, d_seq_out, seq_out_cap, pf, s))) return rc;
  const hipError_t se = hipStreamSynchronize(s);
  if (se != hipSuccess) return bsc_fail(BSC_ERR_HIP, "bsc_prepare_templates_device: %s", hipGetErrorString(se));
  return bsc_prep_finish(ctx, d_raw, nr, d_seq, d_misms, par, seq_out_used, stats, pf);
}

int bsc_vcf_compact_device(bsc_context *ctx, const void *d_core, const void *d_gtm, uint32_t gtm_stride,
                           const void *d_dbsnp, uint32_t n, void *d_out, uint64_t out_cap, void *d_count, void *stream) {
  if (!ctx || !d_count) return bsc_fail(BSC_ERR_ARG, "bsc_vcf_compact_device: NULL argument");
  int rc = gtm_stride ? bsc_check_stride(gtm_stride) : BSC_OK;
  if (rc) return rc;
  BSC_ENTER(ctx);
  if (n == 0) {
    HIP_TRY(hipMemsetAsync(d_count, 0, sizeof(unsigned long long), (hipStream_t)stream));
    return BSC_OK;
  }
  if (!d_core || !d_gtm || (!d_out && out_cap)) return bsc_fail(BSC_ERR_ARG, "bsc_vcf_compact_device: NULL buffer");
  if (((uintptr_t)d_core & 15u) || ((uintptr_t)d_gtm & 7u) || ((uintptr_t)d_out & 15u))
    return bsc_fail(BSC_ERR_ARG, "bsc_vcf_compact_device: d_core / d_out must be 16-byte and d_gtm 8-byte aligned");
  const uint32_t n_tiles = (n + 63u) / 64u;
  size_t scan_bytes = 0;
  if (bsc_dev_scan_tmp_bytes(n_tiles, &scan_bytes)) return bsc_fail(BSC_ERR_HIP, "compact: scan size query failed");
  if ((rc = bsc_reserve(&ctx->d_tcnt, &ctx->cap_tcnt, (size_t)n_tiles * 4u))) return rc;
  if ((rc = bsc_reserve(&ctx->d_toff, &ctx->cap_toff, (size_t)n_tiles * 4u))) return rc;
  if ((rc = bsc_reserve(&ctx->d_scantmp, &ctx->cap_scantmp, scan_bytes ? scan_bytes : 1))) return rc;
  const void *emit = gtm_stride == 0 ? ctx->emit_hint : NULL;
  void *emit_ws = NULL;
  if (gtm_stride == 0 && !emit && !ctx->no_emit_bytes) {
    if ((rc = bsc_reserve(&ctx->d_emit, &ctx->cap_emit, (size_t)n + 64u))) return rc;
    emit_ws = ctx->d_emit;
  }
  int e = bsc_dev_launch_compact(d_core, d_gtm, gtm_stride, d_dbsnp, n, ctx->d_tcnt, ctx->d_toff, ctx->d_scantmp, scan_bytes,
                                 d_out, out_cap, d_count, emit, emit_ws, ctx->num_cus, stream);
  if (e) return bsc_fail(BSC_ERR_HIP, "compact launch failed: %s", hipGetErrorString((hipError_t)e));
  return BSC_OK;
}

static int bsc_names_check(const char *who, const bsc_bcf_names *names, uint32_t *n_names, uint64_t *name_bytes) {
  *n_names = 0;
  *name_bytes = 0;
  if (!names || !names->n) return BSC_OK;
  if (!names->pos || !names->off || (!names->bytes && names->off[names->n])) return bsc_fail(BSC_ERR_ARG, "%s: a names table with NULL arrays", who);
  for (uint32_t i = 0; i < names->n; i++) {
    if (names->off[i] > names->off[i + 1] || (i && names->pos[i] <= names->pos[i - 1]))
      return bsc_fail(BSC_ERR_ARG, "%s: names table entry %u: positions must ascend, offsets must not descend", who, i);
  }
  *n_names = names->n;
  *name_bytes = names->off[names->n];
  return BSC_OK;
}

static int bsc_names_upload(bsc_context *ctx, const char *who, const bsc_bcf_names *names, hipStream_t s) {
  ctx->names_up = NULL;
  uint32_t n = 0;
  uint64_t nb = 0;
  int rc;
  if ((rc = bsc_names_check(who, names, &n, &nb))) return rc;
  if (!n) return BSC_OK;
  const size_t o_off = (size_t)n * 4u, o_by = o_off + ((size_t)n + 1u) * 4u, total = o_by + (size_t)nb;
  if (total + 1u > ctx->cap_hnm) {
    if (ctx->h_names) hipHostFree(ctx->h_names);
    ctx->h_names = NULL;
    ctx->cap_hnm = 0;
    const size_t sz = total + total / 4 + 4096u;
    if (hipHostMalloc(&ctx->h_names, sz, hipHostMallocDefault) != hipSuccess) return bsc_fail(BSC_ERR_NOMEM, "%s: hipHostMalloc(%zu) failed", who, sz);
    ctx->cap_hnm = sz;
  }
  if ((rc = bsc_reserve(&ctx->d_bnm, &ctx->cap_bnm, total + 1u))) return rc;
  char *h = (char *)ctx->h_names;
  memcpy(h, names->pos, (size_t)n * 4u);
  memcpy(h + o_off, names->off, ((size_t)n + 1u) * 4u);
  if (nb) memcpy(h + o_by, names->bytes, (size_t)nb);
  HIP_TRY(hipMemcpyAsync(ctx->d_bnm, h, total, hipMemcpyHostToDevice, s));
  ctx->names_up = names;
  ctx->names_up_n = n;
  ctx->names_up_bytes = nb;
  return BSC_OK;
}

static int bsc_stream_args_check(const bsc_context *ctx, const char *who, const void *d_recs, const void *d_core, const void *d_aux, const void *d_n_recs,
                                 uint64_t max_recs, const void *d_out, uint64_t out_cap, const void *d_totals) {
  if (!ctx || !d_totals || (out_cap && !d_out)) return bsc_fail(BSC_ERR_ARG, "%s: NULL argument", who);
  if (d_recs ? !d_n_recs : (max_recs && (!d_core || !d_aux))) return bsc_fail(BSC_ERR_ARG, "%s: NULL argument", who);
  if (((uintptr_t)d_recs & 15u) || ((uintptr_t)d_core & 15u) || ((uintptr_t)d_aux & 15u) || ((uintptr_t)d_n_recs & 7u) || ((uintptr_t)d_totals & 7u))
    return bsc_fail(BSC_ERR_ARG, "%s: the records must be 16-byte, the count and the totals 8-byte aligned", who);
  if ((uintptr_t)d_out & 15u)
    return bsc_fail(BSC_ERR_ARG, "%s: d_out must be 16-byte aligned (append blocks at multiples of 16, or encode into a buffer of its own)", who);
  if (max_recs > 0x1fffffffc0ull) return bsc_fail(BSC_ERR_ARG, "%s: more than 2^37 records", who);
  return BSC_OK;
}

typedef struct {
  bsc_devguard guard;
  uint32_t n_tiles;
  size_t scan_bytes;
  const void *d_pos, *d_off, *d_nb;
  uint32_t n_names;
} bsc_stream_plan;
static void bsc_stream_plan_exit(bsc_stream_plan *p) { bsc_devguard_exit(&p->guard); }
#define BSC_STREAM_PLAN(p) bsc_stream_plan p __attribute__((cleanup(bsc_stream_plan_exit))) = {.guard = {-1}}

static int bsc_stream_encode_begin(bsc_context *ctx, const char *who, const void *d_recs, const void *d_core, const void *d_aux, const void *d_n_recs,
                                   uint64_t max_recs, const bsc_bcf_names *names, void *d_out, uint64_t out_cap, void *d_totals, void *stream,
                                   bsc_stream_plan *plan) {
  int rc;
  if ((rc = bsc_stream_args_check(ctx, who, d_recs, d_core, d_aux, d_n_recs, max_recs, d_out, out_cap, d_totals))) return rc;
  uint32_t n_names = 0;
  uint64_t name_bytes = 0;
  const int names_up = names && ctx->names_up == names;
  if (names_up) {
    n_names = ctx->names_up_n;
    name_bytes = ctx->names_up_bytes;
  } else if ((rc = bsc_names_check(who, names, &n_names, &name_bytes)))
    return rc;
  BSC_ENTER_GUARD(ctx, plan->guard);
  hipStream_t s = (hipStream_t)stream;
  const uint32_t n_tiles = (uint32_t)((max_recs + 63u) / 64u);
  size_t scan_bytes = 0;
  if (bsc_dev_scan_tmp_bytes_u64(n_tiles + 1u, &scan_bytes)) return bsc_fail(BSC_ERR_HIP, "%s: scan size query failed", who);
  if ((rc = bsc_reserve(&ctx->d_btb, &ctx->cap_btb, ((size_t)n_tiles + 1u) * 8u))) return rc;
  if ((rc = bsc_reserve(&ctx->d_bto, &ctx->cap_bto, ((size_t)n_tiles + 1u) * 8u))) return rc;
  if ((rc = bsc_reserve(&ctx->d_bscn, &ctx->cap_bscn, scan_bytes ? scan_bytes : 1))) return rc;
  plan->d_pos = plan->d_off = plan->d_nb = NULL;
  if (n_names) {
    const size_t o_off = (size_t)n_names * 4u, o_by = o_off + ((size_t)n_names + 1u) * 4u;
    if (!names_up) {
      if ((rc = bsc_reserve(&ctx->d_bnm, &ctx->cap_bnm, o_by + (size_t)name_bytes + 1u))) return rc;
      HIP_TRY(hipMemcpyAsync(ctx->d_bnm, names->pos, (size_t)n_names * 4u, hipMemcpyHostToDevice, s));
      HIP_TRY(hipMemcpyAsync((char *)ctx->d_bnm + o_off, names->off, ((size_t)n_names + 1u) * 4u, hipMemcpyHostToDevice, s));
      if (name_bytes) HIP_TRY(hipMemcpyAsync((char *)ctx->d_bnm + o_by, names->bytes, (size_t)name_bytes, hipMemcpyHostToDevice, s));
    }
    plan->d_pos = ctx->d_bnm;
    plan->d_off = (char *)ctx->d_bnm + o_off;
    plan->d_nb = (char *)ctx->d_bnm + o_by;
  }
  HIP_TRY(hipMemsetAsync(d_totals, 0, 3 * sizeof(unsigned long long), s));
  plan->n_tiles = n_tiles;
  plan->scan_bytes = scan_bytes;
  plan->n_names = n_names;
  return BSC_OK;
}

static int bsc_bcf_encode(bsc_context *ctx, const char *who, const void *d_recs, const void *d_core, const void *d_aux, const void *d_n_recs,
                          uint64_t max_recs, int32_t rid, const bsc_bcf_ids *ids, const bsc_bcf_names *names, void *d_out, uint64_t out_cap,
                          void *d_totals, void *stream) {
  if (!ids) return bsc_fail(BSC_ERR_ARG, "%s: NULL argument", who);
  BSC_STREAM_PLAN(plan);
  int rc;
  if ((rc = bsc_stream_encode_begin(ctx, who, d_recs, d_core, d_aux, d_n_recs, max_recs, names, d_out, out_cap, d_totals, stream, &plan))) return rc;
  const int e = bsc_dev_launch_bcf(d_recs, d_core, d_aux, d_n_recs, max_recs, rid, ids, plan.d_pos, plan.d_off, plan.d_nb, plan.n_names, ctx->d_btb,
                                   ctx->d_bto, ctx->d_bscn, plan.scan_bytes, d_out, out_cap, d_totals, ctx->num_cus, stream, d_recs ? NULL : ctx->emit_hint);
  if (e) return bsc_fail(BSC_ERR_HIP, "BCF encoder launch failed: %s", hipGetErrorString((hipError_t)e));
  return BSC_OK;
}
// ... 59 lines not shown
}

int bsc_fmt_g(const float *v, uint64_t n, uint8_t *out16) {
  if (n && (!v || !out16)) return bsc_fail(BSC_ERR_ARG, "bsc_fmt_g: NULL argument");
  for (uint64_t i = 0; i < n; i++) {
    char buf[32];
    const int l = snprintf(buf, sizeof buf, "%g", (double)v[i]);
    if (l < 0 || l > 15) return bsc_fail(BSC_ERR_RANGE, "bsc_fmt_g: a value printed in %d characters", l);
    memset(out16 + 16u * i, 0, 16);
    memcpy(out16 + 16u * i, buf, (size_t)l);
    out16[16u * i + 15u] = (uint8_t)l;
  }
  return BSC_OK;
}

int bsc_fmt_g_device(bsc_context *ctx, const void *d_v, uint64_t n, void *d_out16, void *stream) {
  if (!ctx || (n && (!d_v || !d_out16))) return bsc_fail(BSC_ERR_ARG, "bsc_fmt_g_device: NULL argument");
  if (((uintptr_t)d_v & 3u) || ((uintptr_t)d_out16 & 15u)) return bsc_fail(BSC_ERR_ARG, "bsc_fmt_g_device: the values must be 4-byte, the slots 16-byte aligned");
  BSC_ENTER(ctx);
  const int e = bsc_dev_launch_fmt_g(d_v, n, d_out16, ctx->num_cus, stream);
  if (e) return bsc_fail(BSC_ERR_HIP, "bsc_fmt_g_device: launch failed: %s", hipGetErrorString((hipError_t)e));
  return BSC_OK;
}

static void bsc_bcf_pool_take(bsc_context *ctx, size_t need);
typedef struct {
  int32_t rid;
  const bsc_bcf_ids *ids;
  const bsc_bcf_names *names;
  uint8_t *out;
  uint64_t out_cap;
  int text;
  const char *contig;
} bsc_bcf_req;

static pthread_mutex_t bsc_h2d_lock = PTHREAD_MUTEX_INITIALIZER;
static hipEvent_t bsc_h2d_last = NULL;
static int bsc_h2d_last_dev = -1;
static const bsc_context *bsc_h2d_last_ctx = NULL;

static void bsc_h2d_turn_begin(bsc_context *ctx, hipStream_t s) {
  if (ctx->no_h2d_turns) return;
  pthread_mutex_lock(&bsc_h2d_lock);
  if (bsc_h2d_last && bsc_h2d_last_ctx != ctx && bsc_h2d_last_dev == ctx->device) (void)hipStreamWaitEvent(s, bsc_h2d_last, 0);
  pthread_mutex_unlock(&bsc_h2d_lock);
}

static void bsc_h2d_turn_end(bsc_context *ctx, hipStream_t s) {
  if (ctx->no_h2d_turns) return;
  if (!ctx->ev_h2d && hipEventCreateWithFlags(&ctx->ev_h2d, hipEventDisableTiming) != hipSuccess) {
    ctx->ev_h2d = NULL;
    (void)hipGetLastError();
    return;
  }
  if (hipEventRecord(ctx->ev_h2d, s) != hipSuccess) return;
  pthread_mutex_lock(&bsc_h2d_lock);
  bsc_h2d_last = ctx->ev_h2d;
  bsc_h2d_last_dev = ctx->device;
  bsc_h2d_last_ctx = ctx;
  pthread_mutex_unlock(&bsc_h2d_lock);
}

static void bsc_h2d_turn_forget(bsc_context *ctx) {
  pthread_mutex_lock(&bsc_h2d_lock);
  if (bsc_h2d_last_ctx == ctx) {
    bsc_h2d_last = NULL;
    bsc_h2d_last_ctx = NULL;
    bsc_h2d_last_dev = -1;
  }
  pthread_mutex_unlock(&bsc_h2d_lock);
  if (ctx->ev_h2d) (void)hipEventDestroy(ctx->ev_h2d);
  ctx->ev_h2d = NULL;
}

static int bsc_records_queue(bsc_context *ctx, const bsc_template *tpl, uint32_t nr, const uint8_t *seq, uint64_t seq_bytes, uint32_t x,
                             uint32_t y, const uint8_t *ref, const uint8_t *dbsnp, const bsc_vcf_params *params, int with_stats,
                             bsc_vcf_rec *out, uint64_t out_cap, int stage, const bsc_bcf_req *bcf) {
  const int resident = stage == 2;
  if (resident) {
    stage = 0;
    tpl = NULL;
  }
  if (y < x) return bsc_fail(BSC_ERR_ARG, "accumulate: y (%u) < x (%u) (reference asserts y >= x)", y, x);
  if (nr && !resident && (!tpl || !seq)) return bsc_fail(BSC_ERR_ARG, "accumulate: NULL template or read buffer");
  if (ctx->pending_sz || ctx->rec_pending)
    return bsc_fail(BSC_ERR_ARG, "a submitted block has not been fetched (bsc_block_fetch / bsc_block_records_fetch first)");
  const uint64_t sz64 = (uint64_t)y - x + 1;
  if (sz64 > 0x0fffffffull) return bsc_fail(BSC_ERR_ARG, "bsc_block_records: block longer than 2^28 - 1 positions");
  const uint32_t sz = (uint32_t)sz64;
  BSC_ENTER(ctx);
  int rc;
  if (bcf) {
    out = NULL;
    out_cap = 0;
    bsc_bcf_pool_take(ctx, (size_t)(bcf->out_cap ? bcf->out_cap : 1));
    if ((rc = bsc_reserve(&ctx->d_bcf, &ctx->cap_bcf, (size_t)(bcf->out_cap ? bcf->out_cap : 1)))) return rc;
    if ((rc = bsc_reserve(&ctx->d_btot, &ctx->cap_btot, 3 * sizeof(unsigned long long)))) return rc;
  }
  if (!resident) {
    if ((rc = bsc_reserve(&ctx->d_tpl, &ctx->cap_tpl, (size_t)(nr ? nr : 1) * sizeof(bsc_template)))) return rc;
    if ((rc = bsc_reserve(&ctx->d_seq, &ctx->cap_seq, (size_t)(seq_bytes ? seq_bytes : 1)))) return rc;
  }
  if ((rc = bsc_reserve(&ctx->d_ref, &ctx->cap_ref, (size_t)sz + 2))) return rc;
  ctx->again.valid = 0;
  if ((rc = bsc_reserve(&ctx->d_out, &ctx->cap_out, (size_t)sz * 64u))) return rc;
  if ((rc = bsc_reserve(&ctx->d_vout, &ctx->cap_vout, (size_t)sz * sizeof(bsc_vcf_core)))) return rc;
  if ((rc = bsc_reserve(&ctx->d_recs, &ctx->cap_recs, (size_t)(out_cap ? out_cap : 1) * sizeof(bsc_vcf_rec)))) return rc;
  if (dbsnp && (rc = bsc_reserve(&ctx->d_vdb, &ctx->cap_vdb, (size_t)sz))) return rc;
  if (!ctx->h_cnt && hipHostMalloc((void **)&ctx->h_cnt, 8 * sizeof(unsigned long long), hipHostMallocDefault) != hipSuccess)
    return bsc_fail(BSC_ERR_NOMEM, "bsc_block_records: pinned counter block");
  if (stage) {
    const size_t b_tpl = resident ? 0 : (size_t)nr * sizeof(bsc_template), b_seq = resident ? 0 : (size_t)seq_bytes, b_ref = (size_t)sz + 2,
                 b_db = dbsnp ? (size_t)sz : 0;
    const size_t o_seq = (b_tpl + 63u) & ~(size_t)63u, o_ref = (o_seq + b_seq + 63u) & ~(size_t)63u, o_db = (o_ref + b_ref + 63u) & ~(size_t)63u;
    if ((rc = bsc_stage_reserve(ctx, o_db + b_db + 64u))) return rc;
    char *st = ctx->h_stage;
    if (nr && !resident) {
      memcpy(st, tpl, b_tpl);
      memcpy(st + o_seq, seq, b_seq);
      tpl = (const bsc_template *)st;
      seq = (const uint8_t *)(st + o_seq);
    }
    memcpy(st + o_ref, ref, b_ref);
    ref = (const uint8_t *)(st + o_ref);
    if (dbsnp) {
      memcpy(st + o_db, dbsnp, b_db);
      dbsnp = (const uint8_t *)(st + o_db);
    }
  }
  hipStream_t s = ctx->stream;
  ctx->blk_tpl = tpl;
  ctx->blk_d_tpl = ctx->d_tpl;
  ctx->blk_x = x;
  ctx->mb_n = 0;
  const int turns = bcf != NULL && !resident;
  if (turns) bsc_h2d_turn_begin(ctx, s);
  if (nr && !resident) {
    HIP_TRY(hipMemcpyAsync(ctx->d_tpl, tpl, (size_t)nr * sizeof(bsc_template), hipMemcpyHostToDevice, s));
    HIP_TRY(hipMemcpyAsync(ctx->d_seq, seq, (size_t)seq_bytes, hipMemcpyHostToDevice, s));
  }
  if (!(resident && ctx->ref_resident)) HIP_TRY(hipMemcpyAsync(ctx->d_ref, ref, (size_t)sz + 2, hipMemcpyHostToDevice, s));
  if (dbsnp) HIP_TRY(hipMemcpyAsync(ctx->d_vdb, dbsnp, (size_t)sz, hipMemcpyHostToDevice, s));
  if (bcf && (rc = bsc_names_upload(ctx, "bsc_block_bcf", bcf->names, s))) return rc;
  const bsc_bcf_names *const names_ready = ctx->names_up;
  ctx->names_up = NULL;
  if (turns) bsc_h2d_turn_end(ctx, s);
  void *d_db = dbsnp ? ctx->d_vdb : NULL;
  void *d_emit = NULL;
  if (!ctx->no_emit_bytes) {
    if ((rc = bsc_reserve(&ctx->d_emit, &ctx->cap_emit, (size_t)sz + 64u))) return rc;
    HIP_TRY(hipMemsetAsync(ctx->d_emit, 0, (size_t)sz + 64u, s));
    d_emit = ctx->d_emit;
  }
  if ((rc = bsc_reads_chain_queue(ctx, ctx->d_tpl, nr, ctx->d_seq, seq_bytes, x, y, ctx->d_ref, d_db, params, with_stats, ctx->d_vout,
                                  ctx->d_out, d_emit, s)))
    return rc;
  unsigned long long *d_total = ctx->d_counters + BSC_CNT_RECORDS;
  ctx->emit_hint = d_emit;
  rc = bcf ? BSC_OK : bsc_vcf_compact_device(ctx, ctx->d_vout, ctx->d_out, 0, d_db, sz, ctx->d_recs, out_cap, d_total, s);
  ctx->emit_hint = NULL;
  if (rc) return rc;
  HIP_TRY(hipMemcpyAsync(ctx->h_cnt, ctx->d_counters + BSC_CNT_INEXACT, 3 * sizeof(unsigned long long), hipMemcpyDeviceToHost, s));
  ctx->rec_out = out;
  ctx->rec_cap = out_cap;
  ctx->rec_sz = sz;
  ctx->bcf_out = NULL;
  if (bcf) {
    ctx->emit_hint = d_emit;
    ctx->again.sz = sz;
    ctx->again.rid = bcf->rid;
    ctx->again.text = bcf->text;
    if (bcf->text) {
      strncpy(ctx->again.contig, bcf->contig, sizeof ctx->again.contig - 1);
      ctx->again.contig[sizeof ctx->again.contig - 1] = 0;
    } else
      ctx->again.ids = *bcf->ids;
    ctx->again.emit = d_emit;
    ctx->again.have_names = names_ready != NULL;
    ctx->again.n_names = ctx->names_up_n;
    ctx->again.name_bytes = ctx->names_up_bytes;
    ctx->names_up = names_ready;
    rc = bcf->text ? bsc_vcf_text_sites_device(ctx, ctx->d_vout, ctx->d_out, sz, bcf->contig, bcf->names, ctx->d_bcf, bcf->out_cap, ctx->d_btot, s)
                   : bsc_bcf_sites_device(ctx, ctx->d_vout, ctx->d_out, sz, bcf->rid, bcf->ids, bcf->names, ctx->d_bcf, bcf->out_cap, ctx->d_btot, s);
    ctx->emit_hint = NULL;
    ctx->names_up = NULL;
    if (rc) return rc;
    HIP_TRY(hipMemcpyAsync(ctx->h_cnt + 4, ctx->d_btot, 3 * sizeof(unsigned long long), hipMemcpyDeviceToHost, s));
    uint64_t guess = ctx->bcf_share > 0.0 ? (uint64_t)((double)sz * ctx->bcf_share) + 65536u : 0u;
    if (guess > bcf->out_cap) guess = bcf->out_cap;
    if (!bcf->out) guess = 0;
    if (guess) HIP_TRY(hipMemcpyAsync(bcf->out, ctx->d_bcf, (size_t)guess, hipMemcpyDeviceToHost, s));
    ctx->bcf_blk = 1;
    ctx->bcf_keep = bcf->out == NULL;
    ctx->bcf_out = bcf->out;
    ctx->bcf_cap = bcf->out_cap;
    ctx->bcf_copied = guess;
    ctx->rec_copied = 0;
    return BSC_OK;
  }
  uint64_t guess = (uint64_t)((double)sz * ctx->rec_share) + 4096u;
  if (guess > out_cap) guess = out_cap;
  if (guess > sz) guess = sz;
  if (guess) HIP_TRY(hipMemcpyAsync(out, ctx->d_recs, (size_t)guess * sizeof(bsc_vcf_rec), hipMemcpyDeviceToHost, s));
  ctx->rec_copied = guess;
  return BSC_OK;
}

static int bsc_bcf_finish(bsc_context *ctx, uint8_t *out, int inexact) {
  const unsigned long long bytes = ctx->h_cnt[4], bad = ctx->h_cnt[5];
  ctx->bcf_bytes = bytes;
  ctx->bcf_copied = ctx->bcf_copied < bytes ? ctx->bcf_copied : bytes;
  const char *const who = ctx->again.text ? "bsc_block_vcf" : "bsc_block_bcf";
  if (bad) return bsc_fail(BSC_ERR_ARG, "%s: %llu records with a genotype beyond 9 or more than 6 likelihoods", who, bad);
  if (bytes > ctx->bcf_cap) {
    ctx->again.valid = 1;
    ctx->again.inexact = inexact;
    return bsc_fail(BSC_ERR_ARG, "%s: the block's stream has %llu bytes, out_cap is %llu", who, bytes, (unsigned long long)ctx->bcf_cap);
  }
  if (ctx->bcf_keep) return bsc_inexact_status(inexact);
  if (bytes > ctx->bcf_copied) {
    HIP_TRY(hipMemcpyAsync(out + ctx->bcf_copied, (const char *)ctx->d_bcf + ctx->bcf_copied, (size_t)(bytes - ctx->bcf_copied), hipMemcpyDeviceToHost,
                           ctx->stream));
    HIP_TRY(hipStreamSynchronize(ctx->stream));
  }
  if (ctx->rec_sz >= 4096u) ctx->bcf_share = (double)bytes / (double)ctx->rec_sz * 1.02;
  return bsc_inexact_status(inexact);
}

int bsc_block_bcf_again(bsc_context *ctx, uint8_t *out, uint64_t out_cap, uint64_t *n_bytes, uint64_t *n_records) {
  if (!ctx || !n_bytes || !n_records || !out_cap) return bsc_fail(BSC_ERR_ARG, "bsc_block_bcf_again: NULL argument");
  *n_bytes = *n_records = 0;
  if (!ctx->again.valid || ctx->rec_pending || ctx->pending_sz)
    return bsc_fail(BSC_ERR_ARG, "bsc_block_bcf_again: the last call on this context was not a BCF block refused for its out_cap");
  BSC_ENTER(ctx);
  hipStream_t s = ctx->stream;
  int rc;
  if ((rc = bsc_reserve(&ctx->d_bcf, &ctx->cap_bcf, (size_t)out_cap))) return rc;
  ctx->again.names.n = ctx->again.n_names;
  ctx->names_up = ctx->again.have_names ? &ctx->again.names : NULL;
  ctx->names_up_n = ctx->again.n_names;
  ctx->names_up_bytes = ctx->again.name_bytes;
  ctx->emit_hint = ctx->again.emit;
  rc = ctx->again.text
           ? bsc_vcf_text_sites_device(ctx, ctx->d_vout, ctx->d_out, ctx->again.sz, ctx->again.contig, ctx->names_up, ctx->d_bcf, out_cap, ctx->d_btot, s)
           : bsc_bcf_sites_device(ctx, ctx->d_vout, ctx->d_out, ctx->again.sz, ctx->again.rid, &ctx->again.ids, ctx->names_up, ctx->d_bcf, out_cap, ctx->d_btot, s);
  ctx->emit_hint = NULL;
  ctx->names_up = NULL;
  if (rc) return rc;
  HIP_TRY(hipMemcpyAsync(ctx->h_cnt + 4, ctx->d_btot, 3 * sizeof(unsigned long long), hipMemcpyDeviceToHost, s));
  HIP_TRY(hipStreamSynchronize(s));
  const unsigned long long bytes = ctx->h_cnt[4];
  *n_bytes = ctx->bcf_bytes = bytes;
  *n_records = ctx->h_cnt[6];
  if (bytes > out_cap)
    return bsc_fail(BSC_ERR_ARG, "%s: the block's stream has %llu bytes, out_cap is %llu", ctx->again.text ? "bsc_block_vcf" : "bsc_block_bcf", bytes,
                    (unsigned long long)out_cap);
  if (out && bytes) {
    HIP_TRY(hipMemcpyAsync(out, ctx->d_bcf, (size_t)bytes, hipMemcpyDeviceToHost, s));
    HIP_TRY(hipStreamSynchronize(s));
  }
  ctx->bcf_keep = out == NULL;
  ctx->again.valid = 0;
  return bsc_inexact_status(ctx->again.inexact);
}

static int bsc_records_finish(bsc_context *ctx, uint64_t *n_out) {
  *n_out = 0;
  uint8_t *const bcf_out = ctx->bcf_out;
  const int is_bcf = ctx->bcf_blk;
  ctx->bcf_out = NULL;
  ctx->bcf_blk = 0;
  HIP_TRY(hipStreamSynchronize(ctx->stream));
  int inexact = 0;
  int rc = bsc_verdict(ctx, ctx->h_cnt, &inexact);
  if (rc) return rc;
  const unsigned long long total = is_bcf ? ctx->h_cnt[6] : ctx->h_cnt[2];
  *n_out = total;
  if (is_bcf) return bsc_bcf_finish(ctx, bcf_out, inexact);
  if (total > ctx->rec_cap)
    return bsc_fail(BSC_ERR_ARG, "bsc_block_records: the block has %llu records, out_cap is %llu", total,
                    (unsigned long long)ctx->rec_cap);
  if (total > ctx->rec_copied) {
    HIP_TRY(hipMemcpyAsync((char *)ctx->rec_out + (size_t)ctx->rec_copied * sizeof(bsc_vcf_rec),
                           (const char *)ctx->d_recs + (size_t)ctx->rec_copied * sizeof(bsc_vcf_rec),
                           (size_t)(total - ctx->rec_copied) * sizeof(bsc_vcf_rec), hipMemcpyDeviceToHost, ctx->stream));
    HIP_TRY(hipStreamSynchronize(ctx->stream));
  }
  if (ctx->rec_sz >= 4096u) {
    const double share = (double)total / (double)ctx->rec_sz * 1.02;
    ctx->rec_share = share > 1.0 ? 1.0 : share;
  }
  return bsc_inexact_status(inexact);
}

static int bsc_block_records_(bsc_context *ctx, const bsc_template *tpl, uint32_t nr, const uint8_t *seq, uint64_t seq_bytes,
                              uint32_t x, uint32_t y, const uint8_t *ref, const uint8_t *dbsnp, const bsc_vcf_params *params,
                              int with_stats, bsc_vcf_rec *out, uint64_t out_cap, uint64_t *n_out, const bsc_bcf_req *bcf) {
  if (!ctx || !ref || !params || !n_out || (!out && out_cap)) return bsc_fail(BSC_ERR_ARG, "bsc_block_records: NULL argument");
  *n_out = 0;
  if (ctx->rec_pending) return bsc_fail(BSC_ERR_ARG, "bsc_block_records: a submitted block has not been fetched");
  int rc = bsc_records_queue(ctx, tpl, nr, seq, seq_bytes, x, y, ref, dbsnp, params, with_stats, out, out_cap, 0, bcf);
  if (rc) {
    (void)hipStreamSynchronize(ctx->stream);
    return rc;
  }
  BSC_ENTER(ctx);
  return bsc_records_finish(ctx, n_out);
}

int bsc_block_records(bsc_context *ctx, const bsc_template *tpl, uint32_t nr, const uint8_t *seq, uint64_t seq_bytes,
                      uint32_t x, uint32_t y, const uint8_t *ref, const uint8_t *dbsnp, const bsc_vcf_params *params,
                      int with_stats, bsc_vcf_rec *out, uint64_t out_cap, uint64_t *n_out) {
  return bsc_block_records_(ctx, tpl, nr, seq, seq_bytes, x, y, ref, dbsnp, params, with_stats, out, out_cap, n_out, NULL);
}

static int bsc_bcf_req_check(const char *who, const bsc_bcf_ids *ids, uint8_t *out, uint64_t out_cap, uint64_t *n_bytes, uint64_t *n_records) {
  if (!ids || !n_bytes || !n_records || (!out && out_cap)) return bsc_fail(BSC_ERR_ARG, "%s: NULL argument", who);
  *n_bytes = 0;
  *n_records = 0;
  return BSC_OK;
}

int bsc_block_bcf(bsc_context *ctx, const bsc_template *tpl, uint32_t nr, const uint8_t *seq, uint64_t seq_bytes, uint32_t x, uint32_t y,
                  const uint8_t *ref, const uint8_t *dbsnp, const bsc_vcf_params *params, int with_stats, int32_t rid, const bsc_bcf_ids *ids,
                  const bsc_bcf_names *names, uint8_t *out, uint64_t out_cap, uint64_t *n_bytes, uint64_t *n_records) {
  int rc = bsc_bcf_req_check("bsc_block_bcf", ids, out, out_cap, n_bytes, n_records);
  if (rc) return rc;
  const bsc_bcf_req req = {rid, ids, names, out, out_cap};
  if (ctx) ctx->bcf_bytes = 0;
  rc = bsc_block_records_(ctx, tpl, nr, seq, seq_bytes, x, y, ref, dbsnp, params, with_stats, NULL, 0, n_records, &req);
  if (ctx) *n_bytes = ctx->bcf_bytes;
  return rc;
}

static double bsc_now_s(void) {
  struct timespec t;
  clock_gettime(CLOCK_MONOTONIC, &t);
  return (double)t.tv_sec + 1e-9 * (double)t.tv_nsec;
}
static int bsc_block_records_rawdev_(bsc_context *ctx, const void *d_raw, uint32_t nr, const void *d_rseq, uint64_t seq_bytes, const void *d_rms,
                                     uint64_t n_misms, uint64_t cap, const bsc_prep_params *prep, uint32_t x, uint32_t y, const uint8_t *ref,
                                     const uint8_t *dbsnp, const bsc_vcf_params *params, int with_stats, bsc_vcf_rec *out, uint64_t out_cap,
                                     uint64_t *n_out, bsc_prep_stats *prep_stats, bsc_read_profile *profile, const bsc_bcf_req *bcf) {
  int rc;
  const int timing = ctx->stage_timing;
  double t0 = timing ? bsc_now_s() : 0.0, t1;
  if ((rc = bsc_reserve(&ctx->d_tpl, &ctx->cap_tpl, (size_t)nr * sizeof(bsc_template)))) return rc;
  if ((rc = bsc_reserve(&ctx->d_seq, &ctx->cap_seq, (size_t)cap))) return rc;
  hipStream_t s = ctx->stream;
  bsc_read_profile dp;
  ctx->ref_resident = 0;
  if (profile) {
    const uint64_t n_ref = (uint64_t)y - x + 3;
    if ((rc = bsc_reserve(&ctx->d_ref, &ctx->cap_ref, (size_t)n_ref))) return rc;
    HIP_TRY(hipMemcpyAsync(ctx->d_ref, ref, (size_t)n_ref, hipMemcpyHostToDevice, s));
    ctx->ref_resident = 1;
    dp = *profile;
    dp.ref = ctx->d_ref;
    dp.x = x;
    dp.n_ref = (uint32_t)n_ref;
  }
  if (ctx->profiling) {
    if (!ctx->ev_raw[0])
      for (int i = 0; i < 2; i++) HIP_TRY(hipEventCreate(&ctx->ev_raw[i]));
    HIP_TRY(hipEventRecord(ctx->ev_raw[0], s));
    ctx->ev_raw_valid = 0;
  }
  if (timing) {
    t1 = bsc_now_s();
    fprintf(stderr, "bsc stage: reserve + reference upload queued %.1f us\n", (t1 - t0) * 1e6);
    t0 = t1;
  }
  if ((rc = bsc_prep_args_check(ctx, d_raw, nr, d_rseq, seq_bytes, d_rms, n_misms, prep, ctx->d_tpl, ctx->d_seq, cap, profile ? &dp : NULL))) return rc;
  if (prep_stats) memset(prep_stats, 0, sizeof *prep_stats);
  if ((rc = bsc_prep_queue(ctx, d_raw, nr, d_rseq, seq_bytes, d_rms, n_misms, prep, ctx->d_tpl, ctx->d_seq, cap, profile ? &dp : NULL, s))) {
    (void)hipStreamSynchronize(s);
    return rc;
  }
  if (timing) {
    t1 = bsc_now_s();
    fprintf(stderr, "bsc stage: pre-processing queued %.1f us\n", (t1 - t0) * 1e6);
    t0 = t1;
  }
  rc = bsc_records_queue(ctx, NULL, nr, NULL, cap, x, y, ref, dbsnp, params, with_stats, out, out_cap, 2, bcf);
  ctx->ref_resident = 0;
  if (rc) {
    (void)hipStreamSynchronize(ctx->stream);
    return rc;
  }
  if (ctx->profiling && hipEventRecord(ctx->ev_raw[1], s) == hipSuccess) ctx->ev_raw_valid = 1;
  if (timing) {
    t1 = bsc_now_s();
    fprintf(stderr, "bsc stage: bsc_records_queue (reserves, uploads, launches) %.1f us\n", (t1 - t0) * 1e6);
    t0 = t1;
  }
  const hipError_t se = hipStreamSynchronize(s);
  if (se != hipSuccess) return bsc_fail(BSC_ERR_HIP, "bsc_block_records_raw: %s", hipGetErrorString(se));
  if (timing) {
    t1 = bsc_now_s();
    fprintf(stderr, "bsc stage: the wait %.1f us\n", (t1 - t0) * 1e6);
    t0 = t1;
  }
  rc = bsc_prep_finish(ctx, d_raw, nr, d_rseq, d_rms, prep, NULL, prep_stats, profile ? &dp : NULL);
  if (profile) profile->used = dp.used;
  if (rc) {
    ctx->bcf_out = NULL;
    ctx->bcf_blk = 0;
    return rc;
  }
  rc = bsc_records_finish(ctx, n_out);
  if (timing) {
    t1 = bsc_now_s();
    fprintf(stderr, "bsc stage: bsc_records_finish %.1f us\n", (t1 - t0) * 1e6);
  }
  return rc;
}

static int bsc_block_records_raw_(bsc_context *ctx, const bsc_raw_template *raw, uint32_t nr, const uint8_t *seq, uint64_t seq_bytes,
                                  const bsc_misms *misms, uint64_t n_misms, const bsc_prep_params *prep, uint32_t x, uint32_t y, const uint8_t *ref,
                                  const uint8_t *dbsnp, const bsc_vcf_params *params, int with_stats, bsc_vcf_rec *out, uint64_t out_cap,
                                  uint64_t *n_out, bsc_prep_stats *prep_stats, bsc_read_profile *profile, const bsc_bcf_req *bcf) {
  if (!ctx || !ref || !params || !prep || !n_out || (!out && out_cap)) return bsc_fail(BSC_ERR_ARG, "bsc_block_records_raw: NULL argument");
  if (y < x) return bsc_fail(BSC_ERR_ARG, "bsc_block_records_raw: y (%u) < x (%u)", y, x);
  *n_out = 0;
  if (prep_stats) memset(prep_stats, 0, sizeof *prep_stats);
  if (ctx->rec_pending || ctx->pending_sz) return bsc_fail(BSC_ERR_ARG, "bsc_block_records_raw: a submitted block has not been fetched");
  if (nr && (!raw || (seq_bytes && !seq) || (n_misms && !misms))) return bsc_fail(BSC_ERR_ARG, "bsc_block_records_raw: NULL input buffer");
  if (!nr) return bsc_block_records_(ctx, NULL, 0, NULL, 0, x, y, ref, dbsnp, params, with_stats, out, out_cap, n_out, bcf);
  if (y - x > 0x0ffffffeu) return bsc_fail(BSC_ERR_ARG, "bsc_block_records_raw: block longer than 2^28 - 1 positions");
  BSC_ENTER(ctx);
  uint64_t cap = seq_bytes + 16;
  for (uint64_t z = 0; z < n_misms; z++)
    if (misms[z].type == BSC_MISMS_INS && misms[z].size <= seq_bytes) cap += misms[z].size;
  int rc;
  if ((rc = bsc_reserve(&ctx->d_raw, &ctx->cap_raw, (size_t)nr * sizeof *raw))) return rc;
  if ((rc = bsc_reserve(&ctx->d_rseq, &ctx->cap_rseq, (size_t)(seq_bytes ? seq_bytes : 1)))) return rc;
  if ((rc = bsc_reserve(&ctx->d_rms, &ctx->cap_rms, (size_t)(n_misms ? n_misms : 1) * sizeof *misms))) return rc;
  hipStream_t s = ctx->stream;
  HIP_TRY(hipMemcpyAsync(ctx->d_raw, raw, (size_t)nr * sizeof *raw, hipMemcpyHostToDevice, s));
  if (seq_bytes) HIP_TRY(hipMemcpyAsync(ctx->d_rseq, seq, (size_t)seq_bytes, hipMemcpyHostToDevice, s));
  if (n_misms) HIP_TRY(hipMemcpyAsync(ctx->d_rms, misms, (size_t)n_misms * sizeof *misms, hipMemcpyHostToDevice, s));
  return bsc_block_records_rawdev_(ctx, ctx->d_raw, nr, ctx->d_rseq, seq_bytes, ctx->d_rms, n_misms, cap, prep, x, y, ref, dbsnp, params, with_stats, out,
                                   out_cap, n_out, prep_stats, profile, bcf);
}

static int bsc_block_rawdev_check(bsc_context *ctx, const void *d_raw, uint32_t nr, const void *d_seq, uint64_t seq_bytes, const void *d_misms,
                                  uint64_t n_misms, const bsc_prep_params *prep, uint32_t x, uint32_t y, const uint8_t *ref, const bsc_vcf_params *params,
                                  uint64_t *n_out, const void *out, uint64_t out_cap) {
  if (!ctx || !ref || !params || !prep || !n_out || (!out && out_cap)) return bsc_fail(BSC_ERR_ARG, "bsc_block_records_rawdev: NULL argument");
  if (y < x) return bsc_fail(BSC_ERR_ARG, "bsc_block_records_rawdev: y (%u) < x (%u)", y, x);
  if (ctx->rec_pending || ctx->pending_sz) return bsc_fail(BSC_ERR_ARG, "bsc_block_records_rawdev: a submitted block has not been fetched");
  if (nr && (!d_raw || (seq_bytes && !d_seq) || (n_misms && !d_misms))) return bsc_fail(BSC_ERR_ARG, "bsc_block_records_rawdev: NULL input buffer");
  if (nr && y - x > 0x0ffffffeu) return bsc_fail(BSC_ERR_ARG, "bsc_block_records_rawdev: block longer than 2^28 - 1 positions");
  return BSC_OK;
}

int bsc_block_records_rawdev(bsc_context *ctx, const void *d_raw, uint32_t nr, const void *d_seq, uint64_t seq_bytes, const void *d_misms, uint64_t n_misms,
                             uint64_t ins_pad, const bsc_prep_params *prep, uint32_t x, uint32_t y, const uint8_t *ref, const uint8_t *dbsnp,
                             const bsc_vcf_params *params, int with_stats, bsc_vcf_rec *out, uint64_t out_cap, uint64_t *n_out, bsc_prep_stats *prep_stats,
                             bsc_read_profile *profile) {
  int rc = bsc_block_rawdev_check(ctx, d_raw, nr, d_seq, seq_bytes, d_misms, n_misms, prep, x, y, ref, params, n_out, out, out_cap);
  if (rc) return rc;
  *n_out = 0;
  if (prep_stats) memset(prep_stats, 0, sizeof *prep_stats);
  if (!nr) return bsc_block_records_(ctx, NULL, 0, NULL, 0, x, y, ref, dbsnp, params, with_stats, out, out_cap, n_out, NULL);
  BSC_ENTER(ctx);
  return bsc_block_records_rawdev_(ctx, d_raw, nr, d_seq, seq_bytes, d_misms, n_misms, seq_bytes + ins_pad + 16, prep, x, y, ref, dbsnp, params, with_stats,
                                   out, out_cap, n_out, prep_stats, profile, NULL);
}

int bsc_block_bcf_rawdev(bsc_context *ctx, const void *d_raw, uint32_t nr, const void *d_seq, uint64_t seq_bytes, const void *d_misms, uint64_t n_misms,
                         uint64_t ins_pad, const bsc_prep_params *prep, uint32_t x, uint32_t y, const uint8_t *ref, const uint8_t *dbsnp,
                         const bsc_vcf_params *params, int with_stats, int32_t rid, const bsc_bcf_ids *ids, const bsc_bcf_names *names, uint8_t *out,
                         uint64_t out_cap, uint64_t *n_bytes, uint64_t *n_records, bsc_prep_stats *prep_stats, bsc_read_profile *profile) {
  int rc = bsc_bcf_req_check("bsc_block_bcf_rawdev", ids, out, out_cap, n_bytes, n_records);
  if (rc) return rc;
  if ((rc = bsc_block_rawdev_check(ctx, d_raw, nr, d_seq, seq_bytes, d_misms, n_misms, prep, x, y, ref, params, n_records, NULL, 0))) return rc;
  if (prep_stats) memset(prep_stats, 0, sizeof *prep_stats);
  const bsc_bcf_req req = {rid, ids, names, out, out_cap};
  ctx->bcf_bytes = 0;
  if (!nr) rc = bsc_block_records_(ctx, NULL, 0, NULL, 0, x, y, ref, dbsnp, params, with_stats, NULL, 0, n_records, &req);
  else {
    BSC_ENTER(ctx);
    rc = bsc_block_records_rawdev_(ctx, d_raw, nr, d_seq, seq_bytes, d_misms, n_misms, seq_bytes + ins_pad + 16, prep, x, y, ref, dbsnp, params, with_stats,
                                   NULL, 0, n_records, prep_stats, profile, &req);
  }
  *n_bytes = ctx->bcf_bytes;
  return rc;
}

int bsc_block_records_raw(bsc_context *ctx, const bsc_raw_template *raw, uint32_t nr, const uint8_t *seq, uint64_t seq_bytes,
                          const bsc_misms *misms, uint64_t n_misms, const bsc_prep_params *prep, uint32_t x, uint32_t y, const uint8_t *ref,
                          const uint8_t *dbsnp, const bsc_vcf_params *params, int with_stats, bsc_vcf_rec *out, uint64_t out_cap,
                          uint64_t *n_out, bsc_prep_stats *prep_stats, bsc_read_profile *profile) {
  return bsc_block_records_raw_(ctx, raw, nr, seq, seq_bytes, misms, n_misms, prep, x, y, ref, dbsnp, params, with_stats, out, out_cap, n_out, prep_stats,
                                profile, NULL);
}

int bsc_block_bcf_raw(bsc_context *ctx, const bsc_raw_template *raw, uint32_t nr, const uint8_t *seq, uint64_t seq_bytes, const bsc_misms *misms,
                      uint64_t n_misms, const bsc_prep_params *prep, uint32_t x, uint32_t y, const uint8_t *ref, const uint8_t *dbsnp,
                      const bsc_vcf_params *params, int with_stats, int32_t rid, const bsc_bcf_ids *ids, const bsc_bcf_names *names, uint8_t *out,
                      uint64_t out_cap, uint64_t *n_bytes, uint64_t *n_records, bsc_prep_stats *prep_stats, bsc_read_profile *profile) {
  int rc = bsc_bcf_req_check("bsc_block_bcf_raw", ids, out, out_cap, n_bytes, n_records);
  if (rc) return rc;
  const bsc_bcf_req req = {rid, ids, names, out, out_cap};
  if (ctx) ctx->bcf_bytes = 0;
  rc = bsc_block_records_raw_(ctx, raw, nr, seq, seq_bytes, misms, n_misms, prep, x, y, ref, dbsnp, params, with_stats, NULL, 0, n_records, prep_stats,
                              profile, &req);
  if (ctx) *n_bytes = ctx->bcf_bytes;
  return rc;
}

int bsc_block_bcf_rawdev_keep(bsc_context *ctx, const void *d_raw, uint32_t nr, const void *d_seq, uint64_t seq_bytes, const void *d_misms, uint64_t n_misms,
                              uint64_t ins_pad, const bsc_prep_params *prep, uint32_t x, uint32_t y, const uint8_t *ref, const uint8_t *dbsnp,
                              const bsc_vcf_params *params, int with_stats, int32_t rid, const bsc_bcf_ids *ids, const bsc_bcf_names *names, uint64_t dev_cap,
                              uint64_t *n_bytes, uint64_t *n_records, bsc_prep_stats *prep_stats, bsc_read_profile *profile) {
  if (!ids || !n_bytes || !n_records) return bsc_fail(BSC_ERR_ARG, "bsc_block_bcf_rawdev_keep: NULL argument");
  *n_bytes = 0;
  *n_records = 0;
  int rc;
  if ((rc = bsc_block_rawdev_check(ctx, d_raw, nr, d_seq, seq_bytes, d_misms, n_misms, prep, x, y, ref, params, n_records, NULL, 0))) return rc;
  if (prep_stats) memset(prep_stats, 0, sizeof *prep_stats);
  const bsc_bcf_req req = {rid, ids, names, NULL, dev_cap};
  ctx->bcf_bytes = 0;
  if (!nr) rc = bsc_block_records_(ctx, NULL, 0, NULL, 0, x, y, ref, dbsnp, params, with_stats, NULL, 0, n_records, &req);
  else {
    BSC_ENTER(ctx);
    rc = bsc_block_records_rawdev_(ctx, d_raw, nr, d_seq, seq_bytes, d_misms, n_misms, seq_bytes + ins_pad + 16, prep, x, y, ref, dbsnp, params, with_stats,
                                   NULL, 0, n_records, prep_stats, profile, &req);
  }
  *n_bytes = ctx->bcf_bytes;
  return rc;
}

int bsc_block_vcf_rawdev_keep(bsc_context *ctx, const void *d_raw, uint32_t nr, const void *d_seq, uint64_t seq_bytes, const void *d_misms, uint64_t n_misms,
                              uint64_t ins_pad, const bsc_prep_params *prep, uint32_t x, uint32_t y, const uint8_t *ref, const uint8_t *dbsnp,
                              const bsc_vcf_params *params, int with_stats, const char *contig, const bsc_bcf_names *names, uint64_t dev_cap,
// ... 948 lines not shown
```

bs_call_amd/csrc/prepdev.hip:

```cpp
#include <hip/hip_runtime.h>
#include <stdint.h>

#include "../../include/bscall_amd.h"

#define FLT_QUAL 63u

struct bsc_prep_plan {
  uint64_t src;
  uint64_t ms;
  uint32_t rl0;
  uint32_t w0, wl;
  uint32_t nm;
  uint32_t mark_l, mark_r;
  uint32_t out_len;
  uint32_t present;
  uint32_t trim_l, trim_r;
};

struct bsc_prep_desc {
  uint64_t srcw;
  uint32_t pk;
  int32_t pc;
};
#define PD_PRESENT 1u
#define PD_EDITED 2u
#define PD_SLOW 8u

#define PREP_CNT_WORDS 8u
#define PREP_CNT_SLOTS 64u
#define PE_ORI 1u
#define PE_READ 2u
#define PE_LIST 4u
#define PE_SOFT_POS 6u
#define PE_SOFT_ILL 7u
#define PE_INDEL 8u
#define PE_CAP 9u
#define PE_PROF_CAP 10u
#define PE_PROF_RANGE 11u

struct prep_rd {
  uint32_t w0, wl;
};
__device__ static __forceinline__ void d_left_trim(prep_rd &r, uint32_t l) {
  if (l > 0) {
    if (l >= r.wl) r.wl = 0;
    else {
      r.w0 += l;
      r.wl -= l;
    }
  }
}
__device__ static __forceinline__ void d_right_trim(prep_rd &r, uint32_t l) {
  if (l > 0) {
    if (l >= r.wl) r.wl = 0;
    else r.wl -= l;
  }
}

__device__ static __forceinline__ uint32_t d_qual(const uint8_t *sp, uint32_t i, uint32_t rl0, uint32_t mark_l, uint32_t mark_r) {
  return (i < mark_l || i >= rl0 - mark_r) ? FLT_QUAL : (uint32_t)sp[i] >> 2;
}

__device__ static __forceinline__ uint32_t d_ld32(const uint8_t *p);
__device__ static uint32_t d_mean_qual(const uint8_t *sp, const prep_rd &r, uint32_t rl0, uint32_t mark_l, uint32_t mark_r) {
  const uint32_t lo = r.w0 > mark_l ? r.w0 : mark_l;
  const uint32_t e0 = r.w0 + r.wl, e1 = rl0 - mark_r;
  const uint32_t hi = e0 < e1 ? e0 : e1;
  uint32_t tot = 0, n = 0, i = lo;
#define MQ_DWORD(w_)                                                                                                                   \
  {                                                                                                                                    \
    const uint32_t q = ((w_) >> 2) & 0x3f3f3f3fu;                                                                                      \
    const uint32_t nz = ((q ^ 0x3f3f3f3fu) + 0x7f7f7f7fu) & 0x80808080u;  \
    n += (uint32_t)__popc(nz);                                                                                                         \
    tot = __builtin_amdgcn_sad_u8(q & ((nz >> 7) * 0xffu), 0u, tot);                                       \
  }
  for (; i + 16u <= hi; i += 16u) {
    uint4 v;
    __builtin_memcpy(&v, sp + i, 16);
    MQ_DWORD(v.x) MQ_DWORD(v.y) MQ_DWORD(v.z) MQ_DWORD(v.w)
  }
  for (; i + 4u <= hi; i += 4u) MQ_DWORD(d_ld32(sp + i))
#undef MQ_DWORD
  for (; i < hi; i++) {
    const uint32_t q = (uint32_t)sp[i] >> 2;
    if (q != FLT_QUAL) {
      tot += q;
      n++;
    }
  }
  return n > 0 ? tot / n : 0;
}

__global__ __launch_bounds__(256) void bsc_prep_plan_kernel(const bsc_raw_template *__restrict__ raw, uint32_t nr, const uint8_t *__restrict__ seq,
                                                            uint64_t seq_bytes, const bsc_misms *__restrict__ misms_in, uint64_t n_misms_in,
                                                            bsc_prep_params par, bsc_misms *__restrict__ ms_work,
                                                            bsc_prep_plan *__restrict__ plan, bsc_prep_desc *__restrict__ desc,
                                                            unsigned long long *__restrict__ out_len,
                                                            bsc_template *__restrict__ tpl_out, unsigned long long *__restrict__ cnt,
                                                            uint32_t *__restrict__ max_pos1) {
  const uint32_t ti = blockIdx.x * 256u + threadIdx.x;
  unsigned long long n_clip = 0, n_overlap = 0;
  uint32_t err = 0;
  if (ti < nr) {
    const bsc_raw_template t = raw[ti];
    bsc_prep_plan P[2];
    prep_rd rd[2];
    uint32_t nm[2];
    bsc_misms *ms[2];
    bool edited[2] = {false, false};
    uint32_t pos[2] = {t.pos[0], t.pos[1]};
    if (t.orientation > 1) err = PE_ORI;
#pragma unroll
    for (int k = 0; k < 2 && !err; k++) {
      if (t.len[k] && (t.off[k] > seq_bytes || t.len[k] > seq_bytes - t.off[k])) err = PE_READ + (uint32_t)k;
      else if (t.n_misms[k] && (t.misms_off[k] > n_misms_in || t.n_misms[k] > n_misms_in - t.misms_off[k])) err = PE_LIST + (uint32_t)k;
    }
    if (!err) {
      const int msk = t.orientation == 0 ? 0 : 1;
#pragma unroll
      for (int k = 0; k < 2; k++) {
        const int side = k ^ msk;
        const uint32_t rl = t.len[k];
        const int32_t lt = side ? par.left_trim[1] : par.left_trim[0], rt = side ? par.right_trim[1] : par.right_trim[0];
        P[k].src = t.off[k];
        P[k].ms = t.misms_off[k];
        P[k].rl0 = rl;
        P[k].mark_l = lt > 0 ? ((uint32_t)lt < rl ? (uint32_t)lt : rl) : 0u;
        P[k].mark_r = rt > 0 ? ((uint32_t)rt < rl ? (uint32_t)rt : rl) : 0u;
        P[k].present = rl != 0;
        P[k].trim_l = P[k].trim_r = 0;
        rd[k].w0 = 0;
        rd[k].wl = rl;
        nm[k] = t.n_misms[k];
        ms[k] = ms_work + t.misms_off[k];
        for (uint32_t z = 0; z < nm[k]; z++) ms[k][z] = misms_in[t.misms_off[k] + z];
      }
#pragma unroll
      for (int k = 0; k < 2 && !err; k++) {
        const uint32_t rl = rd[k].wl;
        if (rl == 0) continue;
        int nclip = 0;
        uint32_t adj = 0;
        const uint32_t n0 = nm[k];
        for (uint32_t z = 0; z < n0; z++) {
          bsc_misms *m = ms[k] + z;
          if (m->type == BSC_MISMS_SOFT) {
            if (z && z != n0 - 1) { err = PE_SOFT_POS; break; }
            nclip++;
            if (!m->position) {
              if (m->size >= rl) { err = PE_SOFT_ILL; break; }
              adj = m->size;
              n_clip += adj;
              P[k].trim_l = adj;
              d_left_trim(rd[k], adj);
            } else {
              if (m->position + m->size != rl) { err = PE_SOFT_ILL; break; }
              d_right_trim(rd[k], m->size);
              P[k].trim_r = m->size;
              n_clip += m->size;
            }
          } else if (nclip) {
            m->position -= adj;
            ms[k][z - (uint32_t)nclip] = *m;
          }
        }
        if (nclip) nm[k] -= (uint32_t)nclip;
      }
    }
    if (!err) {
      const uint32_t rdl[2] = {rd[0].wl, rd[1].wl};
      if (rdl[0] > 0 && rdl[1] > 0) {
        int rev;
        int32_t overlap;
        if (pos[0] <= pos[1]) {
          overlap = (int32_t)(t.reference_span[0] - pos[1] + pos[0]);
          rev = 0;
        } else {
          overlap = (int32_t)(t.reference_span[1] + pos[1] - pos[0]);
          rev = 1;
        }
        if (pos[0] + t.reference_span[0] >= pos[1]) {
          int tr;
          if (t.reference_span[0] > t.reference_span[1]) tr = 1;
          else if (t.reference_span[0] < t.reference_span[1]) tr = 0;
          else
            tr = d_mean_qual(seq + P[0].src, rd[0], P[0].rl0, P[0].mark_l, P[0].mark_r) <=
                         d_mean_qual(seq + P[1].src, rd[1], P[1].rl0, P[1].mark_l, P[1].mark_r)
                     ? 0
                     : 1;
          const int right = (rev && tr) || !(rev || tr);
          if (!right) {
            if (tr) pos[1] += (uint32_t)overlap;
            else pos[0] += (uint32_t)overlap;
          }
          bsc_misms *mm = tr ? ms[1] : ms[0];
          prep_rd rdt = tr ? rd[1] : rd[0];
          const uint32_t rdl_t = tr ? rdl[1] : rdl[0], span_t = tr ? t.reference_span[1] : t.reference_span[0];
          uint32_t num = tr ? nm[1] : nm[0];
          if (!num) {
            if (right) d_right_trim(rdt, (uint32_t)overlap);
            else d_left_trim(rdt, (uint32_t)overlap);
          } else {
            int trimmed = 0;
            if (right) {
              const uint32_t xx = span_t - (uint32_t)overlap;
              int64_t adj = 0;
              for (uint32_t z = 0; z < num; z++) {
                bsc_misms *m = mm + z;
                if ((int64_t)m->position + adj >= (int64_t)xx) {
                  const int64_t trim = (int64_t)rdl_t - xx + adj;
                  d_right_trim(rdt, (uint32_t)trim);
                  num = z;
                  trimmed = 1;
                  break;
                }
                if (m->type == BSC_MISMS_INS) {
                  if ((int64_t)m->position + adj + m->size >= (int64_t)xx) {
                    const int64_t trim = (int64_t)rdl_t - m->position;
                    m->size = (uint32_t)((int64_t)xx - ((int64_t)m->position + adj));
                    d_right_trim(rdt, (uint32_t)trim);
                    num = z + 1;
                    trimmed = 1;
                  }
                  adj += m->size;
                } else if (m->type == BSC_MISMS_DEL) adj -= m->size;
              }
              if (!trimmed) d_right_trim(rdt, (uint32_t)overlap);
            } else {
              const uint32_t xx = (uint32_t)overlap;
              int64_t adj = 0;
              uint32_t z;
              for (z = 0; z < num; z++) {
                bsc_misms *m = mm + z;
                if ((int64_t)m->position + adj >= (int64_t)xx) {
                  const uint32_t trim = (uint32_t)((int64_t)overlap - adj);
                  d_left_trim(rdt, trim);
                  trimmed = 1;
                  if (z) {
                    for (uint32_t z1 = z; z1 < num; z1++) {
                      mm[z1].position -= trim;
                      const bsc_misms a = mm[z1], b = mm[z1 - z];
                      mm[z1 - z] = a;
                      mm[z1] = b;
                    }
                    num -= z;
                  } else {
                    for (uint32_t z1 = 0; z1 < num; z1++) mm[z1].position -= trim;
                  }
                  break;
                }
                if (m->type == BSC_MISMS_INS) {
                  if ((int64_t)m->position + adj + m->size >= (int64_t)xx) {
                    m->size = (uint32_t)((int64_t)m->position + m->size + adj - xx);
                    const uint32_t trim = m->position;
                    d_left_trim(rdt, trim);
                    trimmed = 1;
                    const uint32_t z2 = m->size ? z : z + 1;
                    for (uint32_t z1 = z2; z1 < num; z1++) {
                      mm[z1].position -= trim;
                      if (z2) {
                        const bsc_misms a = mm[z1], b = mm[z1 - z2];
                        mm[z1 - z2] = a;
                        mm[z1] = b;
                      }
                    }
                    num -= z2;
                    break;
                  }
                  adj += m->size;
                } else if (m->type == BSC_MISMS_DEL) adj -= m->size;
              }
              if (!trimmed) {
                d_left_trim(rdt, (uint32_t)((int64_t)overlap - adj));
                num = 0;
              }
            }
          }
          if (tr) {
            nm[1] = num;
            rd[1] = rdt;
          } else {
            nm[0] = num;
            rd[0] = rdt;
          }
          n_overlap += (rdl[0] - rd[0].wl) + (rdl[1] - rd[1].wl);
          const uint32_t cut = tr ? rdl[1] - rd[1].wl : rdl[0] - rd[0].wl;
          if (right) {
            if (tr) P[1].trim_r += cut;
            else P[0].trim_r += cut;
          } else {
            if (tr) P[1].trim_l += cut;
            else P[0].trim_l += cut;
          }
        }
      }
#pragma unroll
      for (int k = 0; k < 2 && !err; k++) {
        const uint32_t rl = rd[k].wl;
        uint32_t adj = 0;
        for (uint32_t z = 0; z < nm[k]; z++) {
          bsc_misms *m = ms[k] + z;
          const uint32_t ix1 = m->position + adj;
          edited[k] |= m->type == BSC_MISMS_INS || m->type == BSC_MISMS_DEL;
          if (m->type == BSC_MISMS_INS) {
            if (ix1 > rl + adj) { err = PE_INDEL; break; }
            adj += m->size;
          } else if (m->type == BSC_MISMS_DEL) {
            if ((uint64_t)ix1 + m->size > (uint64_t)rl + adj) { err = PE_INDEL; break; }
            adj -= m->size;
          }
          m->position = ix1;
        }
        P[k].w0 = rd[k].w0;
        P[k].wl = rl;
        P[k].nm = nm[k];
        P[k].out_len = rl + adj;
      }
    }
    if (err) {
#pragma unroll
      for (int k = 0; k < 2; k++) {
        P[k].src = P[k].ms = 0;
        P[k].rl0 = P[k].w0 = P[k].wl = P[k].nm = P[k].mark_l = P[k].mark_r = P[k].out_len = P[k].present = P[k].trim_l = P[k].trim_r = 0;
      }
      atomicMin(&cnt[0], ((unsigned long long)ti << 8) | err);
      n_clip = n_overlap = 0;
    }
#pragma unroll
    for (int k = 0; k < 2; k++) {
      bsc_prep_desc d;
      const uint32_t ol = P[k].out_len;
      d.srcw = P[k].src + P[k].w0;
      const uint32_t ml = P[k].mark_l > P[k].w0 ? (P[k].mark_l - P[k].w0 < ol ? P[k].mark_l - P[k].w0 : ol) : 0u;
      const uint32_t keep = P[k].rl0 - P[k].mark_r;
      const uint32_t hr = keep > P[k].w0 ? (keep - P[k].w0 < ol ? keep - P[k].w0 : ol) : 0u;
      const bool ed = edited[k] && !err;
      const bool slow = ol != 0 && (ed || hr < ol || ol < 4u || ol >= 0xfffffu || ml >= 256u);
      d.pk = (ol < 0xfffffu ? ol : 0xfffffu) | ((ml & 0xffu) << 20) |
             (((P[k].present ? PD_PRESENT : 0u) | (ed ? PD_EDITED : 0u) | (slow ? PD_SLOW : 0u)) << 28);
      d.pc = k ? (int32_t)(P[k].wl + P[k].trim_r) - 1 : (int32_t)P[k].trim_l;
      desc[2u * ti + (uint32_t)k] = d;
      if (slow) plan[2u * ti + (uint32_t)k] = P[k];
    }
    if (max_pos1) {
      int32_t max_pos = 0;
#pragma unroll
      for (int k = 0; k < 2; k++)
        if (P[k].present) {
          const int32_t mpos = k ? (int32_t)(P[k].wl + P[k].trim_r) - 1 : (int32_t)(P[k].trim_l + P[k].wl);
          if (mpos > max_pos) max_pos = mpos;
        }
      max_pos1[ti] = err ? 0u : (uint32_t)max_pos + 1u;
    }
    out_len[2u * ti] = P[0].out_len;
    out_len[2u * ti + 1u] = P[1].out_len;
    bsc_template o;
    o.pos[0] = pos[0];
    o.pos[1] = pos[1];
    o.len[0] = P[0].out_len;
    o.len[1] = P[1].out_len;
    o.off[0] = o.off[1] = 0;
    o.mapq[0] = t.mapq[0];
    o.mapq[1] = t.mapq[1];
    o.orientation = t.orientation;
    o.bs_strand = t.bs_strand;
    o.flags = 0;
    tpl_out[ti] = o;
  }
  for (int o = 32; o > 0; o >>= 1) {
    n_clip += __shfl_xor(n_clip, o);
    n_overlap += __shfl_xor(n_overlap, o);
  }
  if ((threadIdx.x & 63u) == 0) {
    unsigned long long *slot = cnt + PREP_CNT_WORDS + (blockIdx.x & (PREP_CNT_SLOTS - 1u)) * 8u;
    if (n_clip) atomicAdd(&slot[0], n_clip);
    if (n_overlap) atomicAdd(&slot[1], n_overlap);
  }
}

__device__ static __forceinline__ uint32_t d_marked(const uint8_t *sp, uint32_t i, uint32_t rl0, uint32_t mark_l, uint32_t mark_r) {
  const bool in_r = i >= rl0 - mark_r;
  const uint32_t b = sp[(in_r && 2u * i > rl0 - 1u) ? rl0 - 1u - i : i];
  return (i < mark_l || in_r) ? (b & 3u) | (FLT_QUAL << 2) : (uint32_t)sp[i];
}

struct bsc_prep_prof {
  const uint8_t *ref;
  uint32_t x, n_ref, cap, used0;
  const uint32_t *used_scan;
  unsigned long long *table;
};
__device__ static const uint8_t PROF_REF[64] = {
    0, 0, 0, 0, 0, 0, 0, 0, 0, 0, 0, 8, 0, 0, 0, 0, 0, 4, 4, 0, 4, 0, 0, 0, 0, 0, 0, 8, 0, 0, 0, 0,
    0, 0, 0, 8, 0, 0, 0, 0, 0, 0, 0, 0, 0, 0, 0, 0, 0, 0, 0, 0, 0, 0, 0, 0, 0, 0, 0, 0, 0, 0, 0, 0};
__device__ static __forceinline__ uint32_t d_profile_base(uint32_t bs_strand, uint32_t c) {
  const uint32_t q = c >> 2;
  if (q < 20u  || q >= FLT_QUAL || bs_strand > 2u) return 0u;
  return ((bs_strand == 0 ? 0x7A6Bu : (bs_strand == 1 ? 0x5A4Bu : 0x7869u)) >> (4u * (c & 3u))) & 15u;
}

#define PREP_WAVES 4
#define PREP_BATCH 4u
#define PROF_LDS 512u

__device__ static __forceinline__ void d_prof_base(const bsc_prep_prof &F, uint32_t *s_prof, uint32_t strand, uint32_t used_t, int64_t v,
                                                   int32_t orig, uint32_t byte) {
  const uint32_t xx = d_profile_base(strand, byte);
  if (xx && v + 1 < (int64_t)F.n_ref) {
    const uint32_t ra = v >= 1 ? F.ref[v - 1] : 0u, rb = v >= 0 ? F.ref[v] : 0u, rc = F.ref[v + 1];
    const uint32_t m_before = PROF_REF[((ra << 3) | rb) & 63u], m_after = PROF_REF[((rb << 3) | rc) & 63u];
    if ((((xx & m_after) | ((xx & m_before) >> 1)) >> 2) & 1u) {
      const uint32_t ix = (uint32_t)(orig + 1);
      if (ix < used_t && ix < F.cap) {
        if (ix < PROF_LDS) atomicAdd(&s_prof[(xx & 3u) * PROF_LDS + ix], 1u);
        else atomicAdd(&F.table[(uint64_t)ix * 4u + (xx & 3u)], 1ull);
      }
    }
  }
}

__device__ static __forceinline__ uint32_t d_bcast(uint32_t v, uint32_t l) { return (uint32_t)__builtin_amdgcn_readlane((int)v, (int)l); }
__device__ static __forceinline__ unsigned long long d_bcast64(unsigned long long v, uint32_t l) {
  return (unsigned long long)d_bcast((uint32_t)v, l) | ((unsigned long long)d_bcast((uint32_t)(v >> 32), l) << 32);
}
__device__ static __forceinline__ uint32_t d_ld32(const uint8_t *p) {
  uint32_t v;
  __builtin_memcpy(&v, p, 4);
  return v;
}
__device__ static __forceinline__ void d_st32(uint8_t *p, uint32_t v) { __builtin_memcpy(p, &v, 4); }

struct prep_slow_ret {
  uint32_t c63, cge;
  uint32_t walked;
};

__device__ static __forceinline__ uint32_t prep_slow_src(const bsc_prep_plan &P, const bsc_misms *__restrict__ ms, bool edited, uint32_t j, bool &pad) {
  uint32_t s = j;
  pad = false;
  if (edited) {
    for (uint32_t z = P.nm; z-- > 0;) {
      const bsc_misms m = ms[z];
      if (m.type == BSC_MISMS_INS) {
        if (s >= m.position) {
          if (s - m.position < m.size) {
            pad = true;
            break;
          }
          s -= m.size;
        }
      } else if (m.type == BSC_MISMS_DEL) {
        if (s >= m.position) s += m.size;
      }
    }
  }
  return s;
}

__device__ __noinline__ static prep_slow_ret prep_slow_read(const bsc_prep_plan *__restrict__ plan_r, uint32_t flags, uint8_t *__restrict__ dp,
                                                            const uint8_t *__restrict__ seq, const bsc_misms *__restrict__ ms_work, uint32_t mq) {
  const unsigned lane = threadIdx.x & 63u;
  prep_slow_ret r = {0u, 0u, 0u};
  const bsc_prep_plan P = *plan_r;
  const uint8_t *const sp = seq + P.src;
  const bool edited = (flags & PD_EDITED) != 0;
  if (edited) {
    for (uint32_t s0 = 0; s0 < P.wl; s0 += 64u) {
      const uint32_t s = s0 + lane;
      if (s < P.wl) {
        const uint32_t q = d_marked(sp, P.w0 + s, P.rl0, P.mark_l, P.mark_r) >> 2;
        r.c63 += q == FLT_QUAL;
        r.cge += q >= mq;
      }
    }
  }
  const bsc_misms *const ms = ms_work + P.ms;
  bool walked = false;
  for (uint32_t j0 = 0; j0 < P.out_len; j0 += 64u) {
    const uint32_t j = j0 + lane;
    if (j < P.out_len) {
      bool pad;
      const uint32_t s = prep_slow_src(P, ms, edited, j, pad);
      const uint32_t byte = pad ? 0u : d_marked(sp, P.w0 + s, P.rl0, P.mark_l, P.mark_r);
      const uint32_t q = byte >> 2;
      if (!edited) {
        r.c63 += q == FLT_QUAL;
        r.cge += q >= mq;
      }
      walked |= q != 0 && q != FLT_QUAL;
      dp[j] = (uint8_t)byte;
    }
  }
  r.walked = __any(walked) ? 1u : 0u;
  return r;
}

__global__ __launch_bounds__(64 * PREP_WAVES) void bsc_prep_copy_kernel(const bsc_prep_plan *__restrict__ plan,
                                                                        const bsc_prep_desc *__restrict__ desc, uint32_t nr,
                                                                        const uint8_t *__restrict__ seq, const bsc_misms *__restrict__ ms_work,
                                                                        const unsigned long long *__restrict__ out_off, int32_t min_qual,
                                                                        bsc_template *__restrict__ tpl_out, uint8_t *__restrict__ seq_out,
                                                                        uint64_t seq_out_cap, unsigned long long *__restrict__ cnt) {
  const unsigned lane = threadIdx.x & 63u, lane4 = lane * 4u;
  const uint32_t wave = (uint32_t)__builtin_amdgcn_readfirstlane((int)(blockIdx.x * PREP_WAVES + (threadIdx.x >> 6)));
  const uint32_t n_waves = gridDim.x * PREP_WAVES;
  const uint32_t mq = min_qual < 0 ? 0u : (min_qual > 64 ? 64u : (uint32_t)min_qual), mq4 = mq * 0x01010101u;
  unsigned long long l_total = 0, l_bases = 0;
  uint32_t c63 = 0, cge = 0, l_reads = 0;
  const uint32_t n_reads2 = 2u * nr, n_groups = (n_reads2 + 63u) / 64u;
  for (uint32_t g = wave; g < n_groups; g += n_waves) {
    const uint32_t g0 = g * 64u, n = n_reads2 - g0 < 64u ? n_reads2 - g0 : 64u;
    const uint32_t ri = g0 + (lane < n ? lane : 0u), my_ti = ri >> 1, my_k = ri & 1u;
    bsc_prep_desc L = desc[ri];
    const unsigned long long l_off = out_off[ri];
    if (lane >= n) L.pk = 0;
    if (lane < n) {
      const uint32_t fl = L.pk >> 28;
      uint32_t ol = L.pk & 0xfffffu, wl = ol;
      if (fl & PD_SLOW) {
        ol = plan[ri].out_len;
        wl = plan[ri].wl;
      }
      tpl_out[my_ti].off[my_k] = l_off;
      if (l_off > seq_out_cap || seq_out_cap - l_off < ol) {
        atomicMin(&cnt[0], ((unsigned long long)my_ti << 8) | PE_CAP);
        L.pk &= 0xf0000000u;
      }
      l_total += (fl & PD_EDITED) ? wl : ol;
      if (fl & PD_PRESENT) {
        l_reads++;
        l_bases += wl;
      }
    }
    enum : uint32_t { KIND_LEAN = 1u, KIND_FAST = 2u, KIND_SLOW = 3u };
    const uint32_t my_len = L.pk & 0xfffffu, my_ml = (L.pk >> 20) & 0xffu;
    const uint32_t my_kind = my_len == 0 ? 0u : ((L.pk >> 28) & PD_SLOW ? KIND_SLOW : ((my_len <= 256u && my_ml == 0) ? KIND_LEAN : KIND_FAST));
    const uint32_t l_ctl = (L.pk & 0x0fffffffu) | (my_kind << 28) | (((L.pk >> 28) & PD_EDITED) ? 1u << 30 : 0u);
    const bool my_fetch = my_kind == KIND_LEAN || my_kind == KIND_FAST;
    const unsigned long long l_src = my_fetch ? (unsigned long long)(seq + L.srcw) - (unsigned long long)desc : 0ull;
    unsigned long long walked_mask = 0;
    const unsigned long long obase = d_bcast64(l_off, 0);
    const unsigned long long m_w0 = __ballot(my_kind == KIND_LEAN && my_len >= 16u && my_len <= 128u);
    const unsigned long long sbase = m_w0 ? d_bcast64(L.srcw, (uint32_t)__builtin_ctzll(m_w0)) : 0ull;
    const unsigned long long orel = l_off - obase, srel = L.srcw - sbase;
    const bool my_wide = my_kind == KIND_LEAN && my_len >= 16u && my_len <= 128u && orel < (1ull << 24) && srel < (1ull << 31);
    const uint32_t w_a = my_wide ? my_len | ((uint32_t)orel << 8) : 0u, w_s = my_wide ? (uint32_t)srel : 0u;
    const uint32_t l16 = (lane & 7u) * 16u, sub = lane & 56u;
    const uint8_t *const sp_w = seq + sbase;
    uint8_t *const dp_w = seq_out + obase;
    uint32_t walk_bits = 0;
    constexpr uint32_t RW = 2u;
    auto fetch8 = [&](uint32_t i0, uint4(&vv)[RW]) {
#pragma unroll
      for (uint32_t i = 0; i < RW; i++) {
        const int src = (int)(sub | ((i0 + i) & 7u));
        const uint32_t len = (uint32_t)__shfl((int)w_a, src) & 0xffu, so = (uint32_t)__shfl((int)w_s, src);
        const uint32_t last = len ? len - 16u : 0u;
        __builtin_memcpy(&vv[i], sp_w + (so + (l16 < last ? l16 : last)), 16);
      }
    };
    auto process8 = [&](const uint32_t i0, const uint4(&v)[RW]) {
#pragma unroll
      for (uint32_t i = 0; i < RW; i++) {
        const uint32_t l = i0 + i;
        const int src = (int)(sub | l);
        const uint32_t a_ = (uint32_t)__shfl((int)w_a, src), len = a_ & 0xffu;
        const bool act = l16 < len;
        const uint32_t o = l16 < len - 16u ? l16 : len - 16u, dup = act ? l16 - o : 16u;
        const uint32_t w4[4] = {v[i].x, v[i].y, v[i].z, v[i].w};
        uint32_t any = 0;
#pragma unroll
        for (uint32_t d = 0; d < 4u; d++) {
          const uint32_t ge = (((0x83828180u + 0x04040404u * d) - dup * 0x01010101u) >> 7) & 0x01010101u;
          const uint32_t wc = w4[d] & (ge * 0xffu);
          const uint32_t qh = ((wc >> 2) & 0x3f3f3f3fu) | 0x80808080u;
          const uint32_t q1 = qh + 0x01010101u;
          c63 += (uint32_t)__popc(q1 & 0x40404040u);
          cge += (uint32_t)__popc((qh - mq4) & 0x80808080u);
          any |= q1 & 0x3e3e3e3eu;
        }
        if (any) walk_bits |= 1u << l;
        if (act) __builtin_memcpy(dp_w + ((a_ >> 8) + o), &v[i], 16);
      }
    };
    auto one = [&](const uint32_t l) {
      const uint32_t k = l & 1u;
      const uint32_t ctl = d_bcast(l_ctl, l), kind = (ctl >> 28) & 3u, len = ctl & 0xfffffu;
      uint8_t *const dp = seq_out + d_bcast64(l_off, l);
      if (kind == KIND_SLOW) {
        const prep_slow_ret r = prep_slow_read(plan + g0 + l, (ctl >> 30) & 1u ? PD_EDITED : 0u, dp, seq, ms_work, mq);
        c63 += r.c63;
        cge += r.cge;
        if (k == 0 && r.walked) walked_mask |= 1ull << l;
        return;
      }
      const uint32_t ml = (ctl >> 20) & 0xffu;
      bool walked = false;
      for (uint32_t base = 0; base < len; base += 256u) {
        const uint32_t nominal = base + lane4;
        const bool act = nominal < len;
        const uint32_t o = nominal < len - 4u ? nominal : len - 4u;
        uint32_t w = act ? d_ld32((const uint8_t *)desc + d_bcast64(l_src, l) + o) : 0u;
        if (ml + 3u > base) {
          const uint32_t nmk = act && ml > o ? (ml - o < 4u ? ml - o : 4u) : 0u;
          const uint32_t mm = nmk >= 4u ? 0xffffffffu : (1u << (8u * nmk)) - 1u;
          w = (w & ~mm) | (((w & 0x03030303u) | 0xfcfcfcfcu) & mm);
        }
        const uint32_t wc = act ? w >> (8u * (nominal - o)) : 0u;
        const uint32_t qh = ((wc >> 2) & 0x3f3f3f3fu) | 0x80808080u;
        const uint32_t q1 = qh + 0x01010101u;
        c63 += (uint32_t)__popc(q1 & 0x40404040u);
        cge += (uint32_t)__popc((qh - mq4) & 0x80808080u);
        if (k == 0) walked |= __any((q1 & 0x3e3e3e3eu) != 0u) != 0;
        if (act) d_st32(dp + o, w);
      }
      if (k == 0 && walked) walked_mask |= 1ull << l;
    };
    if (__ballot(my_wide)) {
      uint4 va[RW], vb[RW];
      fetch8(0, va);
#pragma unroll
      for (uint32_t i0 = 0; i0 < 8u; i0 += 2u * RW) {
        fetch8(i0 + RW, vb);
        process8(i0, va);
        fetch8(i0 + 2u * RW, va);
        process8(i0 + RW, vb);
      }
      walk_bits |= (uint32_t)__shfl_xor((int)walk_bits, 1);
      walk_bits |= (uint32_t)__shfl_xor((int)walk_bits, 2);
      walk_bits |= (uint32_t)__shfl_xor((int)walk_bits, 4);
      walked_mask |= __ballot((walk_bits >> (lane & 7u)) & 1u);
    }
    for (unsigned long long rest = __ballot(my_kind != 0u && !my_wide); rest; rest &= rest - 1ull) one((uint32_t)__builtin_ctzll(rest));
    if (lane < n && my_k == 0) tpl_out[my_ti].flags = BSC_TPL_WALK_KNOWN | (((walked_mask >> lane) & 1ull) ? BSC_TPL_WALKED0 : 0u);
  }
  unsigned long long w[5] = {l_total, c63, cge, l_reads, l_bases};
  for (int i = 0; i < 5; i++)
    for (int o = 32; o > 0; o >>= 1) w[i] += __shfl_xor(w[i], o);
  if (mq == 0) w[2] = w[0];
  if (lane == 0) {
    const unsigned long long low = w[0] - w[2] - (mq > FLT_QUAL ? w[1] : 0ull), none = w[0] - w[1] - low;
    if (none) atomicAdd(&cnt[3], none);
    if (w[1]) atomicAdd(&cnt[4], w[1]);
    if (low) atomicAdd(&cnt[5], low);
    if (w[3]) atomicAdd(&cnt[6], w[3]);
    if (w[4]) atomicAdd(&cnt[7], w[4]);
  }
}

__global__ __launch_bounds__(256) void bsc_prep_refmask_kernel(const uint8_t *__restrict__ ref, uint32_t n_ref, uint8_t *__restrict__ mask) {
  const uint64_t i = ((uint64_t)blockIdx.x * 256u + threadIdx.x) * 4u;
  if (i >= (uint64_t)n_ref + 24u) return;
  uint32_t m = 0;
  if (i >= 12u && i - 8u + 7u <= n_ref) {
    const uint64_t v = i - 8u;
    const uint32_t lo = d_ld32(ref + v - 1u) & 0x07070707u, hi = d_ld32(ref + v + 3u) & 0x07070707u;
    const uint32_t r_at = __builtin_amdgcn_alignbyte(hi, lo, 1u), r_next = __builtin_amdgcn_alignbyte(hi, lo, 2u);
#define PROF_NE(x, c) ((((x) ^ ((c) * 0x01010101u)) + 0x7f7f7f7fu) & 0x80808080u)
    const uint32_t over_c = ~PROF_NE(r_at, 2u) & PROF_NE(r_next, 0u) & PROF_NE(r_next, 3u) & 0x80808080u;
    const uint32_t over_g = ~PROF_NE(r_at, 3u) & PROF_NE(lo, 0u) & PROF_NE(lo, 2u) & 0x80808080u;
#undef PROF_NE
    m = (over_c >> 5) | (over_g >> 4);
  } else {
    for (uint32_t t = 0; t < 4u; t++) {
      const uint64_t it = i + t;
      if (it >= 8u && it - 8u + 1u < n_ref) {
        const uint64_t v = it - 8u;
        const uint32_t ra = v >= 1 ? ref[v - 1] : 0u, rb = ref[v], rc = ref[v + 1];
        m |= ((PROF_REF[((rb << 3) | rc) & 63u] & 4u) | (PROF_REF[((ra << 3) | rb) & 63u] & 8u)) << (8u * t);
      }
    }
  }
  __builtin_memcpy(mask + i, &m, 4);
}

__global__ __launch_bounds__(64 * PREP_WAVES) void bsc_prep_profile_kernel(const bsc_prep_plan *__restrict__ plan, const bsc_prep_desc *__restrict__ desc,
                                                                           uint32_t nr, const bsc_misms *__restrict__ ms_work,
                                                                           const unsigned long long *__restrict__ out_off,
                                                                           const bsc_template *__restrict__ tpl_out, const uint8_t *__restrict__ seq_out,
                                                                           uint64_t seq_out_cap, unsigned long long *__restrict__ cnt,
                                                                           const uint8_t *__restrict__ mask, const bsc_prep_prof F) {
  __shared__ uint32_t s_prof[PROF_LDS * 4u];
  for (unsigned i = threadIdx.x; i < PROF_LDS * 4u; i += 64 * PREP_WAVES) s_prof[i] = 0;
  __syncthreads();
  const unsigned lane = threadIdx.x & 63u;
  const uint32_t wave = (uint32_t)__builtin_amdgcn_readfirstlane((int)(blockIdx.x * PREP_WAVES + (threadIdx.x >> 6)));
  const uint32_t n_waves = gridDim.x * PREP_WAVES;
  const uint32_t n_reads2 = 2u * nr, n_groups = (n_reads2 + 63u) / 64u;
  uint32_t acc[4][2] = {{0u, 0u}, {0u, 0u}, {0u, 0u}, {0u, 0u}};
  uint32_t acc_n = 0;
  bool acc_quarter = true;
  auto flush = [&]() {
    const uint32_t p0 = 8u * (acc_quarter ? (lane & 15u) : (lane & 31u));
#pragma unroll
    for (uint32_t b = 0; b < 4u; b++) {
      const uint32_t col = (0x63u >> (2u * b)) & 3u;
#pragma unroll
      for (uint32_t t = 0; t < 8u; t++) {
        const uint32_t c = (acc[b][t >> 2] >> (8u * (t & 3u))) & 0xffu;
        if (c) atomicAdd(&s_prof[col * PROF_LDS + p0 + t + 1u], c);
      }
      acc[b][0] = acc[b][1] = 0u;
    }
    acc_n = 0;
  };
  for (uint32_t g = wave; g < n_groups; g += n_waves) {
    const uint32_t g0 = g * 64u, n = n_reads2 - g0 < 64u ? n_reads2 - g0 : 64u;
    const uint32_t ri = g0 + (lane < n ? lane : 0u), my_ti = ri >> 1, my_k = ri & 1u;
    const bsc_prep_desc L = desc[ri];
    const unsigned long long l_off = out_off[ri];
    const uint32_t us_prev = my_ti ? F.used_scan[my_ti - 1u] : 0u, us_mine = F.used_scan[my_ti];
    const uint32_t t_strand = tpl_out[my_ti].bs_strand, t_pos = tpl_out[my_ti].pos[my_k];
    uint32_t c1 = 0, kind = 0, l_used = 0, l_strand = 0, l_ol = 0, top = 0;
    if (lane < n) {
      const uint32_t fl = L.pk >> 28;
      uint32_t ol = L.pk & 0xfffffu;
      if (fl & PD_SLOW) ol = plan[ri].out_len;
      const bool fits = !(l_off > seq_out_cap || seq_out_cap - l_off < ol);
      if ((fl & PD_PRESENT) && ol != 0 && fits) {
        const uint32_t before = my_ti ? (us_prev > F.used0 ? us_prev : F.used0) : F.used0;
        l_used = us_mine > before ? us_mine : before;
        if (l_used > before && (unsigned long long)l_used + 1ull > F.cap) atomicMin(&cnt[0], ((unsigned long long)my_ti << 8) | PE_PROF_CAP);
        l_strand = t_strand;
        const uint32_t pos = t_pos;
        l_ol = ol;
        const bool in_ref = pos >= F.x && (uint64_t)pos - F.x + ol + 1u <= F.n_ref;
        if (!in_ref) atomicMin(&cnt[0], ((unsigned long long)my_ti << 8) | PE_PROF_RANGE);
        if (in_ref && l_strand <= 2u) {
          const uint32_t lim = l_used < F.cap ? l_used : F.cap;
          const int32_t pc = L.pc;
          top = my_k ? (uint32_t)(pc < 0 ? 0 : pc) : (uint32_t)pc + ol - 1u;
          const bool regs = !(fl & PD_SLOW) && l_strand != 0u && ol <= 256u && pc >= 0 && pc < 512 && top < 256u && top + 1u < lim && l_off >= 8u &&
                            seq_out_cap - l_off - ol >= 8u;
          kind = regs ? 1u : 2u;
          c1 = pos > F.x ? pos - F.x + 1u : 0u;
        }
      }
    }
    unsigned long long m_regs = __ballot(kind == 1u);
    if (m_regs) {
      const uint32_t first = (uint32_t)__builtin_ctzll(m_regs);
      const unsigned long long obase = d_bcast64(l_off, first);
      const unsigned long long orel = l_off - obase;
      if (kind == 1u && orel >= (1ull << 15)) kind = 2u;
      const uint32_t A1 = kind == 1u ? (c1 + 7u) | (l_strand == 2u ? 1u << 29 : 0u) | (1u << 31) : 0u;
      const uint32_t A2 = kind == 1u ? (l_ol - 1u) | ((uint32_t)L.pc << 8) | ((uint32_t)orel << 17) : 0u;
      const bool quarter = __ballot(kind == 1u && top >= 128u) == 0ull;
      if (quarter != acc_quarter) {
        flush();
        acc_quarter = quarter;
      }
      const uint8_t *const sb = seq_out + obase - 8u;
      const uint32_t h = quarter ? (lane & 15u) : (lane & 31u);
      const int32_t p0 = (int32_t)(8u * h);
      const uint32_t hsel = quarter ? (lane & 48u) : (lane & 32u), rounds = quarter ? 16u : 32u;
      constexpr uint32_t B = 2u;
      struct rnd {
        uint32_t a1;
        unsigned long long w, mw;
        int32_t jc, len8;
      };
      auto ask = [&](uint32_t i, rnd &r) {
        const int src = (int)(hsel | (i & (rounds - 1u)));
        r.a1 = (uint32_t)__shfl((int)A1, src);
        const uint32_t a2 = (uint32_t)__shfl((int)A2, src);
        const int32_t len = (int32_t)(a2 & 0xffu) + 1;
        r.len8 = 8 - len;
        const int32_t pc = (int32_t)((a2 >> 8) & 0x1ffu);
        const int32_t j0 = (i & 1u) ? pc - p0 - 7 : p0 - pc;
        const bool some = (int32_t)r.a1 < 0 && (uint32_t)(j0 + 7) < (uint32_t)(len + 7);
        r.jc = some ? j0 : 0;
        __builtin_memcpy(&r.w, sb + ((a2 >> 17) + (uint32_t)(r.jc + 8)), 8);
        __builtin_memcpy(&r.mw, mask + (some ? (r.a1 & 0x1fffffffu) + (uint32_t)j0 : 0u), 8);
      };
      auto count = [&](uint32_t i, const rnd &r) {
        const int32_t lo = r.jc < 0 ? -r.jc : 0, hi = r.jc + r.len8 > 0 ? r.jc + r.len8 : 0;
        unsigned long long w8 = r.w & (~0ull << (8 * lo)) & (~0ull >> (8 * hi));
        unsigned long long m8 = r.mw;
        if (i & 1u) {
          w8 = __builtin_bswap64(w8);
          m8 = __builtin_bswap64(m8);
        }
        const uint32_t sx = (r.a1 >> 29) & 1u ? 0xffffffffu : 0u;
#pragma unroll
        for (int d = 0; d < 2; d++) {
          const uint32_t w = (uint32_t)(w8 >> (32 * d)), mw = (uint32_t)(m8 >> (32 * d));
          const uint32_t odd = w << 7;
          const uint32_t qf = ((w >> 2) & 0x3f3f3f3fu) | 0x80808080u;
          const uint32_t q_ok = (qf - 20u * 0x01010101u) & ~((qf + 0x01010101u) << 1) & 0x80808080u;
          const uint32_t hb = (((odd & (mw << 5)) | (~odd & (mw << 4))) & q_ok) >> 7;
          const uint32_t wb = w ^ sx;
          const uint32_t t1 = hb & (wb >> 1), t0 = hb ^ t1, t3 = t1 & wb, t2 = t0 & wb;
          acc[3][d] += t3;
          acc[2][d] += t1 ^ t3;
          acc[1][d] += t2;
          acc[0][d] += t0 ^ t2;
        }
      };
      rnd ra[B], rb[B];
#pragma unroll
      for (uint32_t u = 0; u < B; u++) ask(u, ra[u]);
      for (uint32_t i0 = 0; i0 < rounds; i0 += 2u * B) {
        if (acc_n + 2u * B > 255u) flush();
#pragma unroll
        for (uint32_t u = 0; u < B; u++) ask(i0 + B + u, rb[u]);
#pragma unroll
        for (uint32_t u = 0; u < B; u++) count(u, ra[u]);
#pragma unroll
        for (uint32_t u = 0; u < B; u++) ask(i0 + 2u * B + u, ra[u]);
#pragma unroll
        for (uint32_t u = 0; u < B; u++) count(B + u, rb[u]);
        acc_n += 2u * B;
      }
    }
    unsigned long long m_long = __ballot(kind == 2u);
    while (m_long) {
      const uint32_t l = (uint32_t)__builtin_ctzll(m_long);
      m_long &= m_long - 1ull;
      const uint32_t ol = d_bcast(l_ol, l), k = l & 1u, strand = d_bcast(l_strand, l), used_t = d_bcast(l_used, l);
      const int32_t pc = (int32_t)d_bcast((uint32_t)L.pc, l);
      const int64_t v0 = (int64_t)d_bcast(c1, l) - 1;
      const uint8_t *const dp = seq_out + d_bcast64(l_off, l);
      const bool slow = (d_bcast(L.pk, l) >> 28) & PD_SLOW;
      bsc_prep_plan P;
      bool edited = false;
      if (slow) {
        P = plan[g0 + l];
        edited = (d_bcast(L.pk, l) >> 28) & PD_EDITED;
      }
      for (uint32_t jb = 0; jb < ol; jb += 64u) {
        const uint32_t j = jb + lane;
        if (j < ol) {
          bool pad = false;
          const uint32_t s = slow ? prep_slow_src(P, ms_work + P.ms, edited, j, pad) : j;
          if (!pad) d_prof_base(F, s_prof, strand, used_t, v0 + j, k ? pc - (int32_t)s : pc + (int32_t)s, dp[j]);
        }
      }
    }
  }
  flush();
  __syncthreads();
  for (unsigned i = threadIdx.x; i < PROF_LDS * 4u; i += 64 * PREP_WAVES)
    if (s_prof[i] && i % PROF_LDS < F.cap) atomicAdd(&F.table[(uint64_t)(i % PROF_LDS) * 4u + i / PROF_LDS], (unsigned long long)s_prof[i]);
}

extern "C" int bsc_dev_scan_u64(const void *in, void *out, uint32_t n, void *tmp, size_t tmp_bytes, void *stream);

extern "C" size_t bsc_dev_prep_plan_bytes(void) { return sizeof(bsc_prep_plan) + sizeof(bsc_prep_desc); }

extern "C" int bsc_dev_scan_max_u32(const void *in, void *out, uint32_t n, void *tmp, size_t tmp_bytes, void *stream);

extern "C" int bsc_dev_launch_prep(const void *raw, uint32_t nr, const void *seq, uint64_t seq_bytes, const void *misms, uint64_t n_misms,
                                   const bsc_prep_params *par, void *ms_work, void *plan, void *out_len, void *out_off, void *scan_tmp,
                                   size_t scan_tmp_bytes, void *tpl_out, void *seq_out, uint64_t seq_out_cap, void *cnt, int num_cus,
                                   void *stream, const void *prof_ref, uint32_t prof_x, uint32_t prof_n_ref, uint32_t prof_cap,
                                   uint32_t prof_used0, void *prof_table, void *max_pos1, void *used_scan, void *prof_mask) {
  hipStream_t s = (hipStream_t)stream;
  bsc_prep_desc *const desc = (bsc_prep_desc *)((bsc_prep_plan *)plan + 2ull * nr);
  if (!nr) return (int)hipMemsetAsync(out_off, 0, sizeof(unsigned long long), s);
  hipError_t e = hipMemsetAsync((unsigned long long *)out_len + 2ull * nr, 0, sizeof(unsigned long long), s);
  if (e != hipSuccess) return (int)e;
  hipLaunchKernelGGL(bsc_prep_plan_kernel, dim3((nr + 255u) / 256u), dim3(256), 0, s, (const bsc_raw_template *)raw, nr, (const uint8_t *)seq,
                     seq_bytes, (const bsc_misms *)misms, n_misms, *par, (bsc_misms *)ms_work, (bsc_prep_plan *)plan, desc,
                     (unsigned long long *)out_len, (bsc_template *)tpl_out, (unsigned long long *)cnt, prof_ref ? (uint32_t *)max_pos1 : nullptr);
  if ((e = hipGetLastError()) != hipSuccess) return (int)e;
  int rc = bsc_dev_scan_u64(out_len, out_off, 2u * nr + 1u, scan_tmp, scan_tmp_bytes, stream);
  if (rc) return rc;
  bsc_prep_prof F = {nullptr, 0u, 0u, 0u, 0u, nullptr, nullptr};
  if (prof_ref) {
    if ((rc = bsc_dev_scan_max_u32(max_pos1, used_scan, nr, scan_tmp, scan_tmp_bytes, stream))) return rc;
    F.ref = (const uint8_t *)prof_ref;
    F.x = prof_x;
    F.n_ref = prof_n_ref;
    F.cap = prof_cap;
    F.used0 = prof_used0;
    F.used_scan = (const uint32_t *)used_scan;
    F.table = (unsigned long long *)prof_table;
  }
  unsigned g = ((nr + 31u) / 32u + PREP_WAVES - 1u) / PREP_WAVES;
  static int per_cu[2] = {0, 0};
  for (int pv = 0; pv < (prof_ref ? 2 : 1); pv++)
    if (!per_cu[pv]) {
      int nb = 0;
      const hipError_t eo = pv ? hipOccupancyMaxActiveBlocksPerMultiprocessor(&nb, bsc_prep_profile_kernel, 64 * PREP_WAVES, 0)
                               : hipOccupancyMaxActiveBlocksPerMultiprocessor(&nb, bsc_prep_copy_kernel, 64 * PREP_WAVES, 0);
      per_cu[pv] = (eo == hipSuccess && nb > 0) ? nb : 4;
      (void)hipGetLastError();
    }
  unsigned gc = g, gp = g;
  if (gc > (unsigned)num_cus * (unsigned)per_cu[0]) gc = (unsigned)num_cus * (unsigned)per_cu[0];
  hipLaunchKernelGGL(bsc_prep_copy_kernel, dim3(gc), dim3(64 * PREP_WAVES), 0, s, (const bsc_prep_plan *)plan, (const bsc_prep_desc *)desc, nr,
                     (const uint8_t *)seq, (const bsc_misms *)ms_work, (const unsigned long long *)out_off, par->min_qual, (bsc_template *)tpl_out,
                     (uint8_t *)seq_out, seq_out_cap, (unsigned long long *)cnt);
  if ((e = hipGetLastError()) != hipSuccess) return (int)e;
  if (prof_ref) {
    hipLaunchKernelGGL(bsc_prep_refmask_kernel, dim3((unsigned)(((uint64_t)prof_n_ref + 24u + 1023u) / 1024u)), dim3(256), 0, s, (const uint8_t *)prof_ref,
                       prof_n_ref, (uint8_t *)prof_mask);
    if ((e = hipGetLastError()) != hipSuccess) return (int)e;
    if (gp > (unsigned)num_cus * (unsigned)per_cu[1]) gp = (unsigned)num_cus * (unsigned)per_cu[1];
    hipLaunchKernelGGL(bsc_prep_profile_kernel, dim3(gp), dim3(64 * PREP_WAVES), 0, s, (const bsc_prep_plan *)plan, (const bsc_prep_desc *)desc, nr,
                       (const bsc_misms *)ms_work, (const unsigned long long *)out_off, (const bsc_template *)tpl_out, (const uint8_t *)seq_out,
                       seq_out_cap, (unsigned long long *)cnt, (const uint8_t *)prof_mask, F);
  }
  return (int)hipGetLastError();
}
```

Before: 18.00 billion.

## Reference unedited reads in place instead of copying them to output buffer

When preprocessing from a device-resident raw sequence buffer, reads that need no edits (not slow, no mismatches) get zero output length. Their template offset then points back into the original input sequence instead of a copy in the compacted output. The copy, profile and binning kernels become templated on in-place mode and accept a second bounds window for offsets relative to the side buffer. This removes the byte copy and output-buffer traffic for most reads. In exchange it adds address arithmetic across two buffers and extra branching in the hot profile and accumulate paths.

```diff
diff --git a/bs_call_amd/csrc/accumulate.hip b/bs_call_amd/csrc/accumulate.hip
--- a/bs_call_amd/csrc/accumulate.hip
+++ b/bs_call_amd/csrc/accumulate.hip
@@ -25,19 +25,28 @@
   return p0 == 0 ? p1 : (p1 > 0 && p1 < p0 ? p1 : p0);
 }
 
+struct acc_seq_bounds {
+  uint64_t bytes, side_off, side_bytes;
+};
+__device__ static __forceinline__ bool read_in_bounds(const acc_seq_bounds &sb, uint64_t off, uint32_t len) {
+  if (off <= sb.bytes && len <= sb.bytes - off) return true;
+  const uint64_t rel = off - sb.side_off;
+  return rel <= sb.side_bytes && len <= sb.side_bytes - rel;
+}
+
 __device__ static __forceinline__ uint32_t template_error(const bsc_template_dev &tp, uint32_t left, uint32_t x,
-                                                          uint64_t seq_bytes) {
+                                                          const acc_seq_bounds &seq_bytes) {
   if (left < x) return BSC_TERR_LEFT;
   if ((tp.len[0] && tp.pos[0] < x) || (tp.len[1] && tp.pos[1] < x)) return BSC_TERR_LEFT;
   if (tp.orientation > 1) return BSC_TERR_ORI;
   if (tp.bs_strand > 2) return BSC_TERR_STRAND;
-  if (tp.len[0] && (tp.off[0] > seq_bytes || tp.len[0] > seq_bytes - tp.off[0])) return BSC_TERR_RANGE0;
-  if (tp.len[1] && (tp.off[1] > seq_bytes || tp.len[1] > seq_bytes - tp.off[1])) return BSC_TERR_RANGE1;
+  if (tp.len[0] && !read_in_bounds(seq_bytes, tp.off[0], tp.len[0])) return BSC_TERR_RANGE0;
+  if (tp.len[1] && !read_in_bounds(seq_bytes, tp.off[1], tp.len[1])) return BSC_TERR_RANGE1;
   if (tp.flags & ~(TPL_WALK_KNOWN | TPL_WALKED0)) return BSC_TERR_FLAGS;
   return 0;
 }
 
-__device__ static __forceinline__ uint32_t template_reads(const bsc_template_dev &tp, uint32_t x, uint32_t y, uint64_t seq_bytes,
+__device__ static __forceinline__ uint32_t template_reads(const bsc_template_dev &tp, uint32_t x, uint32_t y, const acc_seq_bounds &seq_bytes,
                                                           bool walked0, bsc_read_desc d[2]) {
   acc_dead(d[0]);
   acc_dead(d[1]);
@@ -101,7 +110,7 @@
 }
 
 extern "C" __global__ __launch_bounds__(BIN_WG) void bsc_bin_count_kernel(const bsc_template_dev *__restrict__ tpl, uint32_t nr,
-                                                                          const uint8_t *__restrict__ seq, uint64_t seq_bytes,
+                                                                          const uint8_t *__restrict__ seq, const acc_seq_bounds seq_bytes,
                                                                           uint32_t x, uint32_t y, uint8_t *__restrict__ tflag,
                                                                           uint32_t *__restrict__ bin_cnt,
                                                                           unsigned long long *__restrict__ counters,
@@ -172,7 +181,7 @@
 }
 
 extern "C" __global__ __launch_bounds__(BIN_WG) void bsc_bin_scatter_kernel(const bsc_template_dev *__restrict__ tpl, uint32_t nr,
-                                                                            uint64_t seq_bytes, uint32_t x, uint32_t y,
+                                                                            const acc_seq_bounds seq_bytes, uint32_t x, uint32_t y,
                                                                             const uint8_t *__restrict__ tflag,
                                                                             uint32_t *__restrict__ bin_cur,
                                                                             bsc_read_desc *__restrict__ rd,
@@ -402,7 +411,7 @@
 
 extern "C" uint32_t bsc_dev_n_bins(uint32_t n_sites) { return ((n_sites - 1u) >> ACC_BIN_SHIFT) + 1u; }
 
-static int launch_bin_reads(const void *tpl, uint32_t nr, const void *seq, uint64_t seq_bytes, uint32_t x, uint32_t y, uint32_t nb,
+static int launch_bin_reads(const void *tpl, uint32_t nr, const void *seq, const acc_seq_bounds seq_bytes, uint32_t x, uint32_t y, uint32_t nb,
                             const bsc_chain_mblock *blk, uint32_t n_blk, void *tflag, void *bin_cnt, void *bin_off, void *bin_cur,
                             void *scan_tmp, size_t scan_tmp_bytes, void *rd, void *counters, void *stream) {
   hipStream_t s = (hipStream_t)stream;
@@ -425,14 +434,24 @@
 extern "C" int bsc_dev_launch_bin_reads(const void *tpl, uint32_t nr, const void *seq, uint64_t seq_bytes, uint32_t x, uint32_t y,
                                         void *tflag, void *bin_cnt, void *bin_off, void *bin_cur, void *scan_tmp,
                                         size_t scan_tmp_bytes, void *rd, void *counters, void *stream) {
-  return launch_bin_reads(tpl, nr, seq, seq_bytes, x, y, bsc_dev_n_bins(y - x + 1), NULL, 0, tflag, bin_cnt, bin_off, bin_cur, scan_tmp,
+  const acc_seq_bounds sb = {seq_bytes, 0u, 0u};
+  return launch_bin_reads(tpl, nr, seq, sb, x, y, bsc_dev_n_bins(y - x + 1), NULL, 0, tflag, bin_cnt, bin_off, bin_cur, scan_tmp,
+                          scan_tmp_bytes, rd, counters, stream);
+}
+
+extern "C" int bsc_dev_launch_bin_reads_side(const void *tpl, uint32_t nr, const void *seq, uint64_t seq_bytes, uint64_t side_off,
+                                             uint64_t side_bytes, uint32_t x, uint32_t y, void *tflag, void *bin_cnt, void *bin_off,
+                                             void *bin_cur, void *scan_tmp, size_t scan_tmp_bytes, void *rd, void *counters, void *stream) {
+  const acc_seq_bounds sb = {seq_bytes, side_off, side_bytes};
+  return launch_bin_reads(tpl, nr, seq, sb, x, y, bsc_dev_n_bins(y - x + 1), NULL, 0, tflag, bin_cnt, bin_off, bin_cur, scan_tmp,
                           scan_tmp_bytes, rd, counters, stream);
 }
 
 extern "C" int bsc_dev_launch_bin_reads_multi(const void *tpl, uint32_t nr, const void *seq, uint64_t seq_bytes, const void *d_blk,
                                               uint32_t n_blk, uint32_t n_bins, void *tflag, void *bin_cnt, void *bin_off, void *bin_cur,
                                               void *scan_tmp, size_t scan_tmp_bytes, void *rd, void *counters, void *stream) {
-  return launch_bin_reads(tpl, nr, seq, seq_bytes, 0, 0, n_bins, (const bsc_chain_mblock *)d_blk, n_blk, tflag, bin_cnt, bin_off, bin_cur,
+  const acc_seq_bounds sb = {seq_bytes, 0u, 0u};
+  return launch_bin_reads(tpl, nr, seq, sb, 0, 0, n_bins, (const bsc_chain_mblock *)d_blk, n_blk, tflag, bin_cnt, bin_off, bin_cur,
                           scan_tmp, scan_tmp_bytes, rd, counters, stream);
 }
 
diff --git a/bs_call_amd/csrc/bscall_api.c b/bs_call_amd/csrc/bscall_api.c
--- a/bs_call_amd/csrc/bscall_api.c
+++ b/bs_call_amd/csrc/bscall_api.c
@@ -63,7 +63,7 @@
                         const bsc_prep_params *par, void *ms_work, void *plan, void *out_len, void *out_off, void *scan_tmp,
                         size_t scan_tmp_bytes, void *tpl_out, void *seq_out, uint64_t seq_out_cap, void *cnt, int num_cus, void *stream,
                         const void *prof_ref, uint32_t prof_x, uint32_t prof_n_ref, uint32_t prof_cap, uint32_t prof_used0, void *prof_table,
-                        void *max_pos1, void *used_scan, void *prof_mask);
+                        void *max_pos1, void *used_scan, void *prof_mask, int inplace);
 int bsc_dev_launch_bcf(const void *recs, const void *core, const void *aux, const void *n_recs, uint64_t max_recs, int32_t rid,
                        const bsc_bcf_ids *ids, const void *name_pos, const void *name_off, const void *name_bytes, uint32_t n_names,
                        void *tile_bytes, void *tile_off, void *scan_tmp, size_t scan_tmp_bytes, void *out, uint64_t out_cap, void *totals,
@@ -74,6 +74,9 @@
                             void *totals, int num_cus, void *stream);
 int bsc_dev_launch_fmt_g(const void *v, uint64_t n, void *out16, int num_cus, void *stream);
 int bsc_dev_launch_ref_pad(const void *packed, const void *d_blk, uint32_t n_blk, void *padded, uint32_t n_pos, int num_cus, void *stream);
+int bsc_dev_launch_bin_reads_side(const void *tpl, uint32_t nr, const void *seq, uint64_t seq_bytes, uint64_t side_off, uint64_t side_bytes,
+                                  uint32_t x, uint32_t y, void *tflag, void *bin_cnt, void *bin_off, void *bin_cur, void *scan_tmp,
+                                  size_t scan_tmp_bytes, void *rd, void *counters, void *stream);
 int bsc_dev_launch_bin_reads_multi(const void *tpl, uint32_t nr, const void *seq, uint64_t seq_bytes, const void *d_blk, uint32_t n_blk,
                                    uint32_t n_bins, void *tflag, void *bin_cnt, void *bin_off, void *bin_cur, void *scan_tmp,
                                    size_t scan_tmp_bytes, void *rd, void *counters, void *stream);
@@ -197,6 +200,8 @@
   int ev_rchain_valid;
   hipEvent_t ev_raw[2];
   int ev_raw_valid;
+  const void *win_seq;
+  uint64_t win_bytes, side_bytes;
   int ref_resident;
   hipEvent_t ev_acc[2];
   int ev_acc_valid;
@@ -712,8 +717,11 @@
   HIP_TRY(hipMemsetAsync(ctx->d_counters + BSC_CNT_SPAN, 0, 2 * sizeof(unsigned long long), s));
   HIP_TRY(hipMemsetAsync(ctx->d_counters + BSC_CNT_ERR, 0xff, sizeof(unsigned long long), s));
   HIP_TRY(hipMemsetAsync(ctx->d_counters + BSC_CNT_DEEP, 0, sizeof(unsigned long long), s));
-  int e = bsc_dev_launch_bin_reads(d_tpl, nr, d_seq, seq_bytes, x, y, ctx->d_tflag, ctx->d_bcnt, ctx->d_boff, ctx->d_bcur,
-                                   ctx->d_bscan, scan_bytes, ctx->d_rd, ctx->d_counters, s);
+  int e = ctx->win_seq ? bsc_dev_launch_bin_reads_side(d_tpl, nr, d_seq, seq_bytes, (uint64_t)(uintptr_t)ctx->d_seq - (uint64_t)(uintptr_t)d_seq,
+                                                       ctx->side_bytes, x, y, ctx->d_tflag, ctx->d_bcnt, ctx->d_boff, ctx->d_bcur, ctx->d_bscan,
+                                                       scan_bytes, ctx->d_rd, ctx->d_counters, s)
+                       : bsc_dev_launch_bin_reads(d_tpl, nr, d_seq, seq_bytes, x, y, ctx->d_tflag, ctx->d_bcnt, ctx->d_boff, ctx->d_bcur,
+                                                  ctx->d_bscan, scan_bytes, ctx->d_rd, ctx->d_counters, s);
   if (e) return bsc_fail(BSC_ERR_HIP, "read grouping launch failed: %s", hipGetErrorString((hipError_t)e));
   return BSC_OK;
 }
@@ -1509,7 +1517,8 @@
 }
 
 static int bsc_prep_queue(bsc_context *ctx, const void *d_raw, uint32_t nr, const void *d_seq, uint64_t seq_bytes, const void *d_misms, uint64_t n_misms,
-                          const bsc_prep_params *par, void *d_tpl_out, void *d_seq_out, uint64_t seq_out_cap, const bsc_read_profile *pf, hipStream_t s) {
+                          const bsc_prep_params *par, void *d_tpl_out, void *d_seq_out, uint64_t seq_out_cap, const bsc_read_profile *pf, hipStream_t s,
+                          int inplace) {
   int rc;
   size_t scan_bytes = 0;
   const uint32_t n2 = 2u * nr + 1u;
@@ -1542,7 +1551,7 @@
   int e = bsc_dev_launch_prep(d_raw, nr, d_seq, seq_bytes, d_misms, n_misms, par, ctx->d_pms, ctx->d_pplan, ctx->d_plen, ctx->d_poff,
                               ctx->d_pscan, scan_bytes, d_tpl_out, d_seq_out, seq_out_cap, ctx->d_pcnt, ctx->num_cus, s,
                               prof_bytes ? pf->ref : NULL, pf ? pf->x : 0u, pf ? pf->n_ref : 0u, pf ? pf->cap : 0u, pf ? pf->used : 0u,
-                              ctx->d_pprof, ctx->d_pmax, ctx->d_pused, ctx->d_pmask);
+                              ctx->d_pprof, ctx->d_pmax, ctx->d_pused, ctx->d_pmask, inplace);
   if (e) {
     (void)hipStreamSynchronize(s);
     return bsc_fail(BSC_ERR_HIP, "read pre-processing launch failed: %s", hipGetErrorString((hipError_t)e));
@@ -1612,7 +1621,7 @@
   if (stats) memset(stats, 0, sizeof *stats);
   BSC_ENTER(ctx);
   hipStream_t s = (hipStream_t)stream;
-  if ((rc = bsc_prep_queue(ctx, d_raw, nr, d_seq, seq_bytes, d_misms, n_misms, par, d_tpl_out, d_seq_out, seq_out_cap, pf, s))) return rc;
+  if ((rc = bsc_prep_queue(ctx, d_raw, nr, d_seq, seq_bytes, d_misms, n_misms, par, d_tpl_out, d_seq_out, seq_out_cap, pf, s, 0))) return rc;
   const hipError_t se = hipStreamSynchronize(s);
   if (se != hipSuccess) return bsc_fail(BSC_ERR_HIP, "bsc_prepare_templates_device: %s", hipGetErrorString(se));
   return bsc_prep_finish(ctx, d_raw, nr, d_seq, d_misms, par, seq_out_used, stats, pf);
@@ -1978,8 +1987,9 @@
     HIP_TRY(hipMemsetAsync(ctx->d_emit, 0, (size_t)sz + 64u, s));
     d_emit = ctx->d_emit;
   }
-  if ((rc = bsc_reads_chain_queue(ctx, ctx->d_tpl, nr, ctx->d_seq, seq_bytes, x, y, ctx->d_ref, d_db, params, with_stats, ctx->d_vout,
-                                  ctx->d_out, d_emit, s)))
+  const int windows = resident && ctx->win_seq;
+  if ((rc = bsc_reads_chain_queue(ctx, ctx->d_tpl, nr, windows ? ctx->win_seq : ctx->d_seq, windows ? ctx->win_bytes : seq_bytes, x, y, ctx->d_ref,
+                                  d_db, params, with_stats, ctx->d_vout, ctx->d_out, d_emit, s)))
     return rc;
   unsigned long long *d_total = ctx->d_counters + BSC_CNT_RECORDS;
   ctx->emit_hint = d_emit;
@@ -2199,7 +2209,7 @@
   }
   if ((rc = bsc_prep_args_check(ctx, d_raw, nr, d_rseq, seq_bytes, d_rms, n_misms, prep, ctx->d_tpl, ctx->d_seq, cap, profile ? &dp : NULL))) return rc;
   if (prep_stats) memset(prep_stats, 0, sizeof *prep_stats);
-  if ((rc = bsc_prep_queue(ctx, d_raw, nr, d_rseq, seq_bytes, d_rms, n_misms, prep, ctx->d_tpl, ctx->d_seq, cap, profile ? &dp : NULL, s))) {
+  if ((rc = bsc_prep_queue(ctx, d_raw, nr, d_rseq, seq_bytes, d_rms, n_misms, prep, ctx->d_tpl, ctx->d_seq, cap, profile ? &dp : NULL, s, d_rseq != NULL))) {
     (void)hipStreamSynchronize(s);
     return rc;
   }
@@ -2208,7 +2218,11 @@
     fprintf(stderr, "bsc stage: pre-processing queued %.1f us\n", (t1 - t0) * 1e6);
     t0 = t1;
   }
+  ctx->win_seq = d_rseq;
+  ctx->win_bytes = seq_bytes;
+  ctx->side_bytes = cap;
   rc = bsc_records_queue(ctx, NULL, nr, NULL, cap, x, y, ref, dbsnp, params, with_stats, out, out_cap, 2, bcf);
+  ctx->win_seq = NULL;
   ctx->ref_resident = 0;
   if (rc) {
     (void)hipStreamSynchronize(ctx->stream);
diff --git a/bs_call_amd/csrc/prepdev.hip b/bs_call_amd/csrc/prepdev.hip
--- a/bs_call_amd/csrc/prepdev.hip
+++ b/bs_call_amd/csrc/prepdev.hip
@@ -97,7 +97,7 @@
                                                             bsc_prep_plan *__restrict__ plan, bsc_prep_desc *__restrict__ desc,
                                                             unsigned long long *__restrict__ out_len,
                                                             bsc_template *__restrict__ tpl_out, unsigned long long *__restrict__ cnt,
-                                                            uint32_t *__restrict__ max_pos1) {
+                                                            uint32_t *__restrict__ max_pos1, uint32_t inplace) {
   const uint32_t ti = blockIdx.x * 256u + threadIdx.x;
   unsigned long long n_clip = 0, n_overlap = 0;
   uint32_t err = 0;
@@ -341,6 +341,7 @@
       d.pc = k ? (int32_t)(P[k].wl + P[k].trim_r) - 1 : (int32_t)P[k].trim_l;
       desc[2u * ti + (uint32_t)k] = d;
       if (slow) plan[2u * ti + (uint32_t)k] = P[k];
+      out_len[2u * ti + (uint32_t)k] = (inplace && !slow && ml == 0u) ? 0u : ol;
     }
     if (max_pos1) {
       int32_t max_pos = 0;
@@ -352,8 +353,6 @@
         }
       max_pos1[ti] = err ? 0u : (uint32_t)max_pos + 1u;
     }
-    out_len[2u * ti] = P[0].out_len;
-    out_len[2u * ti + 1u] = P[1].out_len;
     bsc_template o;
     o.pos[0] = pos[0];
     o.pos[1] = pos[1];
@@ -495,12 +494,15 @@
   return r;
 }
 
+#define PD_IN_PLACE(pk_) (!(((pk_) >> 28) & PD_SLOW) && (((pk_) >> 20) & 0xffu) == 0u)
+template <bool INPLACE>
 __global__ __launch_bounds__(64 * PREP_WAVES) void bsc_prep_copy_kernel(const bsc_prep_plan *__restrict__ plan,
                                                                         const bsc_prep_desc *__restrict__ desc, uint32_t nr,
                                                                         const uint8_t *__restrict__ seq, const bsc_misms *__restrict__ ms_work,
                                                                         const unsigned long long *__restrict__ out_off, int32_t min_qual,
                                                                         bsc_template *__restrict__ tpl_out, uint8_t *__restrict__ seq_out,
-                                                                        uint64_t seq_out_cap, unsigned long long *__restrict__ cnt) {
+                                                                        uint64_t seq_out_cap, unsigned long long *__restrict__ cnt,
+                                                                        uint64_t side_off) {
   const unsigned lane = threadIdx.x & 63u, lane4 = lane * 4u;
   const uint32_t wave = (uint32_t)__builtin_amdgcn_readfirstlane((int)(blockIdx.x * PREP_WAVES + (threadIdx.x >> 6)));
   const uint32_t n_waves = gridDim.x * PREP_WAVES;
@@ -521,8 +523,9 @@
         ol = plan[ri].out_len;
         wl = plan[ri].wl;
       }
-      tpl_out[my_ti].off[my_k] = l_off;
-      if (l_off > seq_out_cap || seq_out_cap - l_off < ol) {
+      const bool in_place = INPLACE && PD_IN_PLACE(L.pk);
+      tpl_out[my_ti].off[my_k] = INPLACE ? (in_place ? L.srcw : side_off + l_off) : l_off;
+      if (!in_place && (l_off > seq_out_cap || seq_out_cap - l_off < ol)) {
         atomicMin(&cnt[0], ((unsigned long long)my_ti << 8) | PE_CAP);
         L.pk &= 0xf0000000u;
       }
@@ -580,7 +583,7 @@
           any |= q1 & 0x3e3e3e3eu;
         }
         if (any) walk_bits |= 1u << l;
-        if (act) __builtin_memcpy(dp_w + ((a_ >> 8) + o), &v[i], 16);
+        if (!INPLACE && act) __builtin_memcpy(dp_w + ((a_ >> 8) + o), &v[i], 16);
       }
     };
     auto one = [&](const uint32_t l) {
@@ -612,7 +615,7 @@
         c63 += (uint32_t)__popc(q1 & 0x40404040u);
         cge += (uint32_t)__popc((qh - mq4) & 0x80808080u);
         if (k == 0) walked |= __any((q1 & 0x3e3e3e3eu) != 0u) != 0;
-        if (act) d_st32(dp + o, w);
+        if (act && (!INPLACE || ml != 0u)) d_st32(dp + o, w);
       }
       if (k == 0 && walked) walked_mask |= 1ull << l;
     };
@@ -674,12 +677,14 @@
   __builtin_memcpy(mask + i, &m, 4);
 }
 
+template <bool INPLACE>
 __global__ __launch_bounds__(64 * PREP_WAVES) void bsc_prep_profile_kernel(const bsc_prep_plan *__restrict__ plan, const bsc_prep_desc *__restrict__ desc,
                                                                            uint32_t nr, const bsc_misms *__restrict__ ms_work,
                                                                            const unsigned long long *__restrict__ out_off,
                                                                            const bsc_template *__restrict__ tpl_out, const uint8_t *__restrict__ seq_out,
                                                                            uint64_t seq_out_cap, unsigned long long *__restrict__ cnt,
-                                                                           const uint8_t *__restrict__ mask, const bsc_prep_prof F) {
+                                                                           const uint8_t *__restrict__ mask, const bsc_prep_prof F,
+                                                                           const uint8_t *__restrict__ seq, uint64_t seq_bytes) {
   __shared__ uint32_t s_prof[PROF_LDS * 4u];
   for (unsigned i = threadIdx.x; i < PROF_LDS * 4u; i += 64 * PREP_WAVES) s_prof[i] = 0;
   __syncthreads();
@@ -712,11 +717,13 @@
     const uint32_t us_prev = my_ti ? F.used_scan[my_ti - 1u] : 0u, us_mine = F.used_scan[my_ti];
     const uint32_t t_strand = tpl_out[my_ti].bs_strand, t_pos = tpl_out[my_ti].pos[my_k];
     uint32_t c1 = 0, kind = 0, l_used = 0, l_strand = 0, l_ol = 0, top = 0;
+    const bool in_place = INPLACE && PD_IN_PLACE(L.pk);
+    const unsigned long long l_loc = in_place ? L.srcw : l_off, l_room = in_place ? seq_bytes : seq_out_cap;
     if (lane < n) {
       const uint32_t fl = L.pk >> 28;
       uint32_t ol = L.pk & 0xfffffu;
       if (fl & PD_SLOW) ol = plan[ri].out_len;
-      const bool fits = !(l_off > seq_out_cap || seq_out_cap - l_off < ol);
+      const bool fits = in_place || !(l_off > seq_out_cap || seq_out_cap - l_off < ol);
       if ((fl & PD_PRESENT) && ol != 0 && fits) {
         const uint32_t before = my_ti ? (us_prev > F.used0 ? us_prev : F.used0) : F.used0;
         l_used = us_mine > before ? us_mine : before;
@@ -730,8 +737,8 @@
           const uint32_t lim = l_used < F.cap ? l_used : F.cap;
           const int32_t pc = L.pc;
           top = my_k ? (uint32_t)(pc < 0 ? 0 : pc) : (uint32_t)pc + ol - 1u;
-          const bool regs = !(fl & PD_SLOW) && l_strand != 0u && ol <= 256u && pc >= 0 && pc < 512 && top < 256u && top + 1u < lim && l_off >= 8u &&
-                            seq_out_cap - l_off - ol >= 8u;
+          const bool regs = !(fl & PD_SLOW) && l_strand != 0u && ol <= 256u && pc >= 0 && pc < 512 && top < 256u && top + 1u < lim && l_loc >= 8u &&
+                            l_room - l_loc - ol >= 8u;
           kind = regs ? 1u : 2u;
           c1 = pos > F.x ? pos - F.x + 1u : 0u;
         }
@@ -739,18 +746,20 @@
     }
     unsigned long long m_regs = __ballot(kind == 1u);
     if (m_regs) {
-      const uint32_t first = (uint32_t)__builtin_ctzll(m_regs);
-      const unsigned long long obase = d_bcast64(l_off, first);
-      const unsigned long long orel = l_off - obase;
+      const unsigned long long m_in = INPLACE ? __ballot(kind == 1u && in_place) : 0ull, m_out = m_regs & ~m_in;
+      const unsigned long long obase = m_out ? d_bcast64(l_loc, (uint32_t)__builtin_ctzll(m_out)) : 0ull;
+      const unsigned long long obase_in = m_in ? d_bcast64(l_loc, (uint32_t)__builtin_ctzll(m_in)) : 0ull;
+      const unsigned long long orel = l_loc - (in_place ? obase_in : obase);
       if (kind == 1u && orel >= (1ull << 15)) kind = 2u;
-      const uint32_t A1 = kind == 1u ? (c1 + 7u) | (l_strand == 2u ? 1u << 29 : 0u) | (1u << 31) : 0u;
+      const uint32_t A1 = kind == 1u ? (c1 + 7u) | (l_strand == 2u ? 1u << 29 : 0u) | (in_place ? 1u << 30 : 0u) | (1u << 31) : 0u;
       const uint32_t A2 = kind == 1u ? (l_ol - 1u) | ((uint32_t)L.pc << 8) | ((uint32_t)orel << 17) : 0u;
       const bool quarter = __ballot(kind == 1u && top >= 128u) == 0ull;
       if (quarter != acc_quarter) {
         flush();
         acc_quarter = quarter;
       }
-      const uint8_t *const sb = seq_out + obase - 8u;
+      const uint8_t *const sb_in = m_in ? seq + obase_in - 8u : seq_out + obase - 8u;
+      const uint8_t *const sb = m_out ? seq_out + obase - 8u : sb_in;
       const uint32_t h = quarter ? (lane & 15u) : (lane & 31u);
       const int32_t p0 = (int32_t)(8u * h);
       const uint32_t hsel = quarter ? (lane & 48u) : (lane & 32u), rounds = quarter ? 16u : 32u;
@@ -770,7 +779,8 @@
         const int32_t j0 = (i & 1u) ? pc - p0 - 7 : p0 - pc;
         const bool some = (int32_t)r.a1 < 0 && (uint32_t)(j0 + 7) < (uint32_t)(len + 7);
         r.jc = some ? j0 : 0;
-        __builtin_memcpy(&r.w, sb + ((a2 >> 17) + (uint32_t)(r.jc + 8)), 8);
+        const uint8_t *const sbr = INPLACE && ((r.a1 >> 30) & 1u) ? sb_in : sb;
+        __builtin_memcpy(&r.w, sbr + ((a2 >> 17) + (uint32_t)(r.jc + 8)), 8);
         __builtin_memcpy(&r.mw, mask + (some ? (r.a1 & 0x1fffffffu) + (uint32_t)j0 : 0u), 8);
       };
       auto count = [&](uint32_t i, const rnd &r) {
@@ -814,13 +824,14 @@
       }
     }
     unsigned long long m_long = __ballot(kind == 2u);
+    const unsigned long long m_place = INPLACE ? __ballot(in_place) : 0ull;
     while (m_long) {
       const uint32_t l = (uint32_t)__builtin_ctzll(m_long);
       m_long &= m_long - 1ull;
       const uint32_t ol = d_bcast(l_ol, l), k = l & 1u, strand = d_bcast(l_strand, l), used_t = d_bcast(l_used, l);
       const int32_t pc = (int32_t)d_bcast((uint32_t)L.pc, l);
       const int64_t v0 = (int64_t)d_bcast(c1, l) - 1;
-      const uint8_t *const dp = seq_out + d_bcast64(l_off, l);
+      const uint8_t *const dp = ((m_place >> l) & 1ull ? seq : seq_out) + d_bcast64(l_loc, l);
       const bool slow = (d_bcast(L.pk, l) >> 28) & PD_SLOW;
       bsc_prep_plan P;
       bool edited = false;
@@ -854,7 +865,7 @@
                                    const bsc_prep_params *par, void *ms_work, void *plan, void *out_len, void *out_off, void *scan_tmp,
                                    size_t scan_tmp_bytes, void *tpl_out, void *seq_out, uint64_t seq_out_cap, void *cnt, int num_cus,
                                    void *stream, const void *prof_ref, uint32_t prof_x, uint32_t prof_n_ref, uint32_t prof_cap,
-                                   uint32_t prof_used0, void *prof_table, void *max_pos1, void *used_scan, void *prof_mask) {
+                                   uint32_t prof_used0, void *prof_table, void *max_pos1, void *used_scan, void *prof_mask, int inplace) {
   hipStream_t s = (hipStream_t)stream;
   bsc_prep_desc *const desc = (bsc_prep_desc *)((bsc_prep_plan *)plan + 2ull * nr);
   if (!nr) return (int)hipMemsetAsync(out_off, 0, sizeof(unsigned long long), s);
@@ -862,7 +873,7 @@
   if (e != hipSuccess) return (int)e;
   hipLaunchKernelGGL(bsc_prep_plan_kernel, dim3((nr + 255u) / 256u), dim3(256), 0, s, (const bsc_raw_template *)raw, nr, (const uint8_t *)seq,
                      seq_bytes, (const bsc_misms *)misms, n_misms, *par, (bsc_misms *)ms_work, (bsc_prep_plan *)plan, desc,
-                     (unsigned long long *)out_len, (bsc_template *)tpl_out, (unsigned long long *)cnt, prof_ref ? (uint32_t *)max_pos1 : nullptr);
+                     (unsigned long long *)out_len, (bsc_template *)tpl_out, (unsigned long long *)cnt, prof_ref ? (uint32_t *)max_pos1 : nullptr, inplace ? 1u : 0u);
   if ((e = hipGetLastError()) != hipSuccess) return (int)e;
   int rc = bsc_dev_scan_u64(out_len, out_off, 2u * nr + 1u, scan_tmp, scan_tmp_bytes, stream);
   if (rc) return rc;
@@ -882,25 +893,28 @@
   for (int pv = 0; pv < (prof_ref ? 2 : 1); pv++)
     if (!per_cu[pv]) {
       int nb = 0;
-      const hipError_t eo = pv ? hipOccupancyMaxActiveBlocksPerMultiprocessor(&nb, bsc_prep_profile_kernel, 64 * PREP_WAVES, 0)
-                               : hipOccupancyMaxActiveBlocksPerMultiprocessor(&nb, bsc_prep_copy_kernel, 64 * PREP_WAVES, 0);
+      const hipError_t eo = pv ? hipOccupancyMaxActiveBlocksPerMultiprocessor(&nb, bsc_prep_profile_kernel<false>, 64 * PREP_WAVES, 0)
+                               : hipOccupancyMaxActiveBlocksPerMultiprocessor(&nb, bsc_prep_copy_kernel<false>, 64 * PREP_WAVES, 0);
       per_cu[pv] = (eo == hipSuccess && nb > 0) ? nb : 4;
       (void)hipGetLastError();
     }
   unsigned gc = g, gp = g;
   if (gc > (unsigned)num_cus * (unsigned)per_cu[0]) gc = (unsigned)num_cus * (unsigned)per_cu[0];
-  hipLaunchKernelGGL(bsc_prep_copy_kernel, dim3(gc), dim3(64 * PREP_WAVES), 0, s, (const bsc_prep_plan *)plan, (const bsc_prep_desc *)desc, nr,
-                     (const uint8_t *)seq, (const bsc_misms *)ms_work, (const unsigned long long *)out_off, par->min_qual, (bsc_template *)tpl_out,
-                     (uint8_t *)seq_out, seq_out_cap, (unsigned long long *)cnt);
+  const uint64_t side_off = inplace ? (uint64_t)(uintptr_t)seq_out - (uint64_t)(uintptr_t)seq : 0u;
+  hipLaunchKernelGGL(inplace ? bsc_prep_copy_kernel<true> : bsc_prep_copy_kernel<false>, dim3(gc), dim3(64 * PREP_WAVES), 0, s,
+                     (const bsc_prep_plan *)plan, (const bsc_prep_desc *)desc, nr, (const uint8_t *)seq, (const bsc_misms *)ms_work,
+                     (const unsigned long long *)out_off, par->min_qual, (bsc_template *)tpl_out, (uint8_t *)seq_out, seq_out_cap,
+                     (unsigned long long *)cnt, side_off);
   if ((e = hipGetLastError()) != hipSuccess) return (int)e;
   if (prof_ref) {
     hipLaunchKernelGGL(bsc_prep_refmask_kernel, dim3((unsigned)(((uint64_t)prof_n_ref + 24u + 1023u) / 1024u)), dim3(256), 0, s, (const uint8_t *)prof_ref,
                        prof_n_ref, (uint8_t *)prof_mask);
     if ((e = hipGetLastError()) != hipSuccess) return (int)e;
     if (gp > (unsigned)num_cus * (unsigned)per_cu[1]) gp = (unsigned)num_cus * (unsigned)per_cu[1];
-    hipLaunchKernelGGL(bsc_prep_profile_kernel, dim3(gp), dim3(64 * PREP_WAVES), 0, s, (const bsc_prep_plan *)plan, (const bsc_prep_desc *)desc, nr,
-                       (const bsc_misms *)ms_work, (const unsigned long long *)out_off, (const bsc_template *)tpl_out, (const uint8_t *)seq_out,
-                       seq_out_cap, (unsigned long long *)cnt, (const uint8_t *)prof_mask, F);
+    hipLaunchKernelGGL(inplace ? bsc_prep_profile_kernel<true> : bsc_prep_profile_kernel<false>, dim3(gp), dim3(64 * PREP_WAVES), 0, s,
+                       (const bsc_prep_plan *)plan, (const bsc_prep_desc *)desc, nr, (const bsc_misms *)ms_work, (const unsigned long long *)out_off,
+                       (const bsc_template *)tpl_out, (const uint8_t *)seq_out, seq_out_cap, (unsigned long long *)cnt, (const uint8_t *)prof_mask, F,
+                       (const uint8_t *)seq, seq_bytes);
   }
   return (int)hipGetLastError();
 }
```

New measurement: 18.03 billion, median of 4. About the same (+0.2%).
